# thimabru1010/ResUnet-a_mltsk_keras

Measured on AMD Instinct MI355X. Metric: training patches/sec (256×256, 6-ch, bs=8/GPU) at 1/2/4/8 MI355X, higher is better.
Workload: dtype bf16; 1 GPU; cfg3: ResUnet-a d6 multitask (seg+bound+dist+color) Tanimoto-dual, 256x256x6, 6 classes, Adam, full train step (fwd+loss+bwd+allreduce+update); global_batch=8, per_gpu_batch=8, parallelism=dp1

## Files before the change

include/rua_hip.h:

```cpp
#ifndef RUA_HIP_H
#define RUA_HIP_H
#include <stdint.h>
#ifdef __cplusplus
extern "C" {
#endif

#define RUA_F32 0
#define RUA_BF16 1
#define RUA_MAX_SEG 6
#define RUA_MAX_BRANCH 4
#define RUA_MAX_WGRAD_BATCH 32
#define RUA_MAX_WGRAD_GROUP 8

#define RUA_OK 0
#define RUA_ERR_ARG (-1)
#define RUA_ERR_LAUNCH (-2)

int rua_version(void);
const char* rua_last_error(void);
int rua_device_info(int* cu_count, int* lds_bytes, char* arch, int arch_len);

typedef struct rua_conv_seg {
  const void* x;
  const void* w;
  int32_t C, Hs, Ws;
  int32_t up_shift;
  int32_t dil;
  int32_t taps;
} rua_conv_seg;

typedef struct rua_bn_fold {
  const double* stats;
  int32_t replicas, pad;
  double count, bessel_n;
  float eps, momentum;
  const float* gamma; const float* beta;
  float* moving_mean; float* moving_var;
  float* scale; float* shift; float* mean; float* rstd;
} rua_bn_fold;

typedef struct rua_conv_desc {
  rua_conv_seg seg[RUA_MAX_SEG];
  int32_t nseg;
  int32_t N, H, W, Cout;
  int32_t stride;
  int32_t dtype;
  const float* bias;
  const void* aux;
  int32_t aux_mode;
  const float* mscale;
  const float* mshift;
  int32_t out_relu;
  int32_t accumulate;
  void* y;
  int32_t out_stride, OH, OW;
  double* stats;
  int32_t stats_mode;
  void* workspace;
  int64_t workspace_bytes;
  int32_t stats_replicas;
  const float* bias_more[3];
  const float* in_scale;
  const float* in_shift;
  int32_t in_relu;
  int32_t pad_fold;
  const struct rua_bn_fold* in_fold;
} rua_conv_desc;
int rua_conv_fwd(const rua_conv_desc* d, void* stream);
int rua_conv_fwd_group(const rua_conv_desc* d, int n, void* stream);
int rua_conv_group_last_grids(void);
int rua_conv_group_band_ok(const rua_conv_desc* d, int n);
int rua_conv_group_last_band(void);
int rua_conv_group_last_chain(void);
int rua_conv_fwd_sum(const rua_conv_desc* d, int n, void* stream);
int rua_conv_sum_last_kernel(void);
int rua_conv_sum_kernel(const rua_conv_desc* d, int n);
int rua_conv_smem_bytes(const rua_conv_desc* d);
int64_t rua_conv_workspace_bytes(const rua_conv_desc* d);
void* rua_prof_event_create(void);
int rua_prof_event_record(void* ev, void* hip_stream);
int rua_prof_event_elapsed_us(void* start, void* stop, double* us);
void rua_prof_event_destroy(void* ev);
void rua_profile_mid_event(void* hip_event);
int rua_profile_mid_event_fired(void);
int rua_conv_last_ksplit(void);
int rua_conv_tile_bn(const rua_conv_desc* d);
int rua_conv_kernel_id(const rua_conv_desc* d);
int rua_conv_fused_input_ok(const rua_conv_desc* d);
int rua_conv_tile_bm(const rua_conv_desc* d);
typedef struct rua_conv_launch_info {
  int32_t kernel_id;
  int32_t form;
  int32_t grid_x, grid_y, block, lds_bytes;
  int32_t bm, bn;
  int32_t ksplit;
  int32_t finisher;
  int32_t members;
  int32_t band, chain;
} rua_conv_launch_info;
int rua_conv_plan(const rua_conv_desc* d, rua_conv_launch_info* out);
int rua_conv_group_plan(const rua_conv_desc* d, int n, rua_conv_launch_info* out, int* n_out);

typedef struct rua_wgrad_desc {
  const void* a;  int32_t C, Hs, Ws;
  const void* dy; int32_t Cout, H, W;
  int32_t N, stride, dil, taps, dtype;
  float* dw;
  void* workspace;
  int64_t workspace_bytes;
  const float* in_scale;
  const float* in_shift;
  int32_t in_relu;
  int32_t defer;
  int32_t group_members;
  int32_t batch;
  const int32_t* overwrite_dev;
} rua_wgrad_desc;
typedef struct rua_wgrad_pending {
  int32_t kind;
  int32_t parts;
  int64_t n;
  const float* partials;
  float* dw;
  int32_t CC;
  int32_t blocks;
  int32_t block_begin, pad;
  const int32_t* overwrite_dev;
} rua_wgrad_pending;
int rua_wgrad_plan(const rua_wgrad_desc* d, rua_wgrad_pending* out);
int rua_wgrad_reduce_batch(const rua_wgrad_pending* items_dev, int n_items, int total_blocks, void* stream);
int rua_conv_wgrad(const rua_wgrad_desc* d, void* stream);
int rua_conv_wgrad_group(const rua_wgrad_desc* d, int n, void* stream);
int rua_wgrad_group_last_grids(void);
int rua_wgrad_group_plan(const rua_wgrad_desc* d, int n, rua_wgrad_pending* out);
int64_t rua_wgrad_workspace_bytes(const rua_wgrad_desc* d);
int rua_wgrad_kind(const rua_wgrad_desc* d);
int rua_wgrad_img_kind(const rua_wgrad_desc* d);

typedef struct rua_wprep_item { int64_t src_off, dst_off; int32_t taps, Cout, C, pad; } rua_wprep_item;
int rua_weight_prep(const float* master, void* w_fwd, void* w_dgrad, const rua_wprep_item* items_dev,
                    int n_items, int max_elems, int dtype, void* stream);
int rua_weight_prep_dgrad(const void* w_fwd, void* w_dgrad, const rua_wprep_item* items_dev, int n_items, int max_elems, const int32_t* blockmap_dev,
                          int n_blocks, int dtype, void* stream);
int rua_wprep_blocks(int taps, int Cout, int C);

int rua_stem_fwd(const float* x, const float* w, const float* b, void* y, int64_t M, int Cin, int Cout, int dtype, void* stream);
int rua_stem_fwd_stats(const float* x, const float* w, const float* b, void* y, int64_t M, int Cin, int Cout, int dtype, double* stats, int replicas, void* stream);
int rua_stem_bwd(const float* x, const void* dy, float* dw, float* db, int64_t M, int Cin, int Cout, int dtype, void* stream);
int rua_stem_fwd_pack(const float* x, const float* w, const float* b, void* y, int64_t M, int Cin, int Cout, int dtype, double* stats, int replicas,
                      void* xpack, void* stream);
int rua_stem_bwd_fold(float* tmp, float* dw, float* db, int Cin, int Cout, void* stream);
int rua_head_fwd(const void* x, const float* w, const float* b, float* z, float* p, int64_t M, int Cin, int Cout, int act, int dtype, void* stream);
int rua_head_fwd_loss(const void* x, const float* w, const float* b, float* z, float* p, const float* y, double* tanimoto_sums,
                      double* metrics, int B, int64_t HW, int Cin, int Cout, int act, int dtype, void* stream);
int rua_head_fwd_loss_rep(const void* x, const float* w, const float* b, float* z, float* p, const float* y, double* tanimoto_sums,
                          int sums_replicas, double* metrics, int B, int64_t HW, int Cin, int Cout, int act, int dtype, void* stream);
int rua_head_bwd(const void* x, const float* dz, const float* w, void* dx, int accumulate_dx, float* dw, float* db,
                 float* scratch, int64_t scratch_bytes, int64_t M, int Cin, int Cout, int dtype, int mask_dx, void* stream);
int rua_head_bwd_sums(const void* x, const float* dz, const float* w, void* dx, int accumulate_dx, float* dw, float* db, float* dxsum,
                      float* scratch, int64_t scratch_bytes, int64_t M, int Cin, int Cout, int dtype, int mask_dx, void* stream);

int rua_col_stats(const void* x, int64_t M, int C, double* stats, int replicas, int dtype, void* stream);
int rua_stats_replicas(int64_t blocks);
int rua_col_stats2(const void* g, const void* x, const float* mscale, const float* mshift, int masked,
                   int64_t M, int C, double* stats, int replicas, int dtype, void* stream);
int rua_bn_finalize(const double* stats, int replicas, double count, double bessel_n, const float* gamma, const float* beta,
                    float* moving_mean, float* moving_var, float momentum, float eps, int training,
                    float* scale, float* shift, float* mean, float* rstd, int C, void* stream);
int rua_stats_to_f32(const double* stats, int replicas, int C, float* const* dst, int n, void* stream);
int rua_bn_apply(const void* x, int nb, const float* const* scale, const float* const* shift, int relu,
                 void* const* out, int64_t M, int C, int dtype, void* stream);
int rua_bn_bwd_finalize(const double* stats2, int replicas, double count, const float* gamma, const float* mean, const float* rstd,
                        float* dgamma, float* dbeta, float* coefA, float* coefB, float* coefC, int C, void* stream);
int rua_bn_bwd_apply(int nb, const void* const* g, const float* const* coefA, const float* const* coefB,
                     const float* const* coefC, const float* const* mscale, const float* const* mshift, int masked,
                     const void* x, const void* dskip, void* dx, int accumulate, int64_t M, int C, int dtype, void* stream);

typedef struct rua_bn_branch {
  const float* gamma; const float* beta; float* moving_mean; float* moving_var;
  float* scale; float* shift; float* mean; float* rstd;
  void* out;
  const double* stats; int32_t replicas, pad;
  double* out_stats;
} rua_bn_branch;
typedef struct rua_bn_fwd_desc {
  const void* x; int64_t M; int32_t C, dtype, nb, relu, training, replicas;
  const double* stats;
  double count, bessel_n; float momentum, eps;
  rua_bn_branch br[RUA_MAX_BRANCH];
} rua_bn_fwd_desc;
int rua_bn_fwd(const rua_bn_fwd_desc* d, void* stream);
int rua_bn_fwd_group(const rua_bn_fwd_desc* d, int n, void* stream);
int rua_bn_fwd_group_last_grids(void);
typedef struct rua_bn_bwd_branch {
  const void* g; const double* stats2; int32_t replicas;
  int32_t stats2_out;
  const float* gamma; const float* mean; const float* rstd; const float* scale; const float* shift;
  float* dgamma; float* dbeta;
} rua_bn_bwd_branch;
typedef struct rua_bn_bwd_desc {
  const void* x; const void* dskip; void* dx; int64_t M; int32_t C, dtype, nb, masked, accumulate, pad; double count;
  rua_bn_bwd_branch br[RUA_MAX_BRANCH];
  double* skip_stats;
  int32_t skip_replicas, pad2;
  double* dx_stats;
  int32_t dx_replicas, pad3;
} rua_bn_bwd_desc;
int rua_bn_bwd(const rua_bn_bwd_desc* d, void* stream);
int rua_bn_bwd_group(const rua_bn_bwd_desc* d, int n, void* stream);
int rua_bn_bwd_group_last_grids(void);

int rua_maxpool_fwd(const void* x, void* y, uint8_t* idx, int N, int H, int W, int C, int k, int dtype, void* stream);
int rua_maxpool_bwd(const void* dy, const uint8_t* idx, void* dx, int accumulate, int N, int H, int W, int C, int k, int dtype, void* stream);
int rua_sumpool(const void* x, void* y, int N, int H, int W, int C, int k, int dtype, void* stream);
int rua_maxpool_derive(const void* y_half, const uint8_t* idx_half, void* y, uint8_t* idx, int N, int H_half, int W_half, int C,
                       int k_half, int dtype, void* stream);
int rua_maxpool_bwd_multi(int n, const void* const* dy, const uint8_t* const* idx, const int* ks, void* dx, int accumulate,
                          int N, int H, int W, int C, int dtype, void* stream);
int rua_sumpool_pyramid(const void* x, void* y2, void* y4, void* y8, int N, int H, int W, int C, int dtype, void* stream);
int rua_upsample_nearest(const void* x, void* y, int N, int H, int W, int C, int k, int dtype, void* stream);

int rua_add_n(int n, const void* const* in, void* out, int accumulate, int64_t elems, int dtype, void* stream);
int rua_relu_mask(void* dy, const void* y, int64_t elems, int dtype, void* stream);
int rua_relu(const void* x, void* y, int64_t elems, int dtype, void* stream);
int rua_cast_f32_to(const float* x, void* y, int64_t elems, int dtype, void* stream);
int rua_cast_to_f32(const void* x, float* y, int64_t elems, int dtype, void* stream);
int rua_fill_zero(void* p, int64_t bytes, void* stream);

#define RUA_LOSS_TANIMOTO 0
#define RUA_LOSS_WCE 1
#define RUA_LOSS_CE_LOGITS 2
#define RUA_LOSS_BCE_LOGITS 3
#define RUA_LOSS_MSE 4
#define RUA_ACT_NONE 0
#define RUA_ACT_SOFTMAX 1
#define RUA_ACT_SIGMOID 2
int rua_tanimoto_sums(const float* p, const float* y, int B, int64_t HW, int C, double* sums, void* stream);
int rua_tanimoto_finalize(const double* sums, int B, int64_t HW, int C, float grad_scale, double* loss_out, float* coef,
                          float* per_sample, void* stream);
#define RUA_MAX_HEADS 8
typedef struct rua_tani_head {
  double* sums; int32_t replicas, B, C; float grad_scale; double* loss_out; float* coef; float* per_sample;
} rua_tani_head;
int rua_tanimoto_finalize_multi(const rua_tani_head* heads, int n, void* stream);
typedef struct rua_dz_head {
  int32_t kind, act; const float* p; const float* y; const float* coef; const float* class_w; float grad_scale; int32_t B; int64_t HW; int32_t C, pad; float* dz;
} rua_dz_head;
int rua_head_dz_multi(const rua_dz_head* heads, int n, void* stream);
int rua_tanimoto_finalize_rep(double* sums, int replicas, int B, int64_t HW, int C, float grad_scale, double* loss_out, float* coef,
                              float* per_sample, void* stream);
int rua_tanimoto_ratio(const double* sums, int B, int C, double* mean_out, float* per_sample, void* stream);
int rua_pixel_loss(int kind, const float* p, const float* z, const float* y, const float* class_w,
                   int64_t M, int C, double* loss_out, float* per_pixel, void* stream);
int rua_head_dz(int kind, int act, const float* p, const float* y, const float* coef, const float* class_w,
                float grad_scale, int B, int64_t HW, int C, float* dz, void* stream);
int rua_seg_metrics(const float* p, const float* y, int64_t M, int C, double* out, void* stream);

int rua_tanimoto_sums_void(const float* p, const float* y, const uint8_t* void_mask, int B, int64_t HW, int C, double* sums, void* stream);
int rua_head_fwd_loss_void(const void* x, const float* w, const float* b, float* z, float* p, const float* y, double* tanimoto_sums,
                           int sums_replicas, double* metrics, int B, int64_t HW, int Cin, int Cout, int act, int dtype,
                           const uint8_t* void_mask, void* stream);
int rua_pixel_loss_void(int kind, const float* p, const float* z, const float* y, const float* class_w, const uint8_t* void_mask,
                        int64_t M, int C, double* loss_out, float* per_pixel, void* stream);
int rua_head_dz_void(int kind, int act, const float* p, const float* y, const float* coef, const float* class_w,
                     float grad_scale, int B, int64_t HW, int C, const uint8_t* void_mask, float* dz, void* stream);
int rua_head_dz_multi_void(const rua_dz_head* heads, int n, const uint8_t* void_mask, void* stream);
int rua_seg_metrics_void(const float* p, const float* y, const uint8_t* void_mask, int64_t M, int C, double* out, void* stream);

#define RUA_LOSS_FOCAL_CE 5
#define RUA_LOSS_FOCAL_BCE 6
typedef struct rua_loss_opts { float gamma, label_smoothing, alpha; int32_t class_balance; } rua_loss_opts;
int rua_pixel_loss_opts(int kind, const float* p, const float* z, const float* y, const float* class_w, const uint8_t* void_mask,
                        const rua_loss_opts* opts, int64_t M, int C, double* loss_out, float* per_pixel, void* stream);
int rua_head_dz_opts(int kind, int act, const float* p, const float* y, const float* coef, const float* class_w, float grad_scale,
                     int B, int64_t HW, int C, const uint8_t* void_mask, const rua_loss_opts* opts, float* dz, void* stream);
int rua_head_dz_multi_opts(const rua_dz_head* heads, const rua_loss_opts* opts, int n, const uint8_t* void_mask, void* stream);

typedef struct rua_ohem_opts { int64_t min_kept; int32_t keep_q16, warmup; float thresh; int32_t has_thresh; } rua_ohem_opts;
typedef struct rua_ohem_result { uint32_t tau_key; float tau; int64_t n_valid, n_kept, K; double kept_sum; float scale; int32_t q16_used; } rua_ohem_result;
int64_t rua_ohem_workspace_bytes(int64_t M);
int rua_ohem_select(const float* per_pixel, const uint8_t* void_mask, int64_t M, const rua_ohem_opts* opts, const double* step_state,
                    float loss_weight, void* workspace, int64_t workspace_bytes, uint8_t* drop_mask, double* loss_out,
                    rua_ohem_result* result_dev, void* stream);
typedef struct rua_dz_sel { const uint8_t* drop_mask; const float* scale_dev; } rua_dz_sel;
int rua_head_dz_sel(int kind, int act, const float* p, const float* y, const float* coef, const float* class_w, int B, int64_t HW, int C,
                    const rua_loss_opts* opts, const uint8_t* drop_mask, const float* scale_dev, float* dz, void* stream);
int rua_head_dz_multi_sel(const rua_dz_head* heads, const rua_loss_opts* opts, const rua_dz_sel* sel, int n, const uint8_t* void_mask, void* stream);

int rua_lr_step(double* state, float* lr_out, int adam, double beta1, double beta2, void* stream);
int rua_adam_step(float* theta, float* g, float* m, float* v, int64_t n, float lr_t, const float* lr_t_dev, float beta1, float beta2,
                  float eps, float grad_scale, int zero_grad, void* stream);
int rua_sgd_step(float* theta, float* g, float* vel, int64_t n, float lr, const float* lr_dev, float momentum, float grad_scale,
                 int zero_grad, void* stream);
int rua_adam_step_w(float* theta, float* g, float* m, float* v, int64_t n, float lr_t, const float* lr_t_dev, float beta1, float beta2,
                    float eps, float grad_scale, int zero_grad, void* wcopy_bf16, void* stream);
int rua_sgd_step_w(float* theta, float* g, float* vel, int64_t n, float lr, const float* lr_dev, float momentum, float grad_scale,
                   int zero_grad, void* wcopy_bf16, void* stream);

#define RUA_OPT_CHUNK 8192
typedef struct rua_opt_chunk { int64_t off; int32_t len; int32_t var; } rua_opt_chunk;
typedef struct rua_opt_var { int32_t chunk_begin, chunk_end, decay, pad; } rua_opt_var;
#define RUA_CLIP_NONE 0
#define RUA_CLIP_GLOBAL_NORM 1
#define RUA_CLIP_NORM 2
#define RUA_CLIP_VALUE 3
int rua_grad_sumsq(const float* g, const rua_opt_chunk* chunks, int n_chunks, double* partials, void* stream);
int rua_clip_finish(const double* partials, int n_chunks, const rua_opt_var* vars, int n_vars, int mode, double c, double grad_scale,
                    int skip_nonfinite, double* var_sumsq, float* coef, int32_t* flag, double* report, void* stream);
int rua_adam_step_seg(float* theta, float* g, float* m, float* v, const rua_opt_chunk* chunks, int n_chunks, const rua_opt_var* vars,
                      const float* coef, const int32_t* flag, const float* lr_dev, const double* lr_state, float beta1, float beta2, float eps,
                      float grad_scale, float clipvalue, double weight_decay, int zero_grad, void* wcopy_bf16, void* stream);
int rua_sgd_step_seg(float* theta, float* g, float* vel, const rua_opt_chunk* chunks, int n_chunks, const rua_opt_var* vars,
                     const float* coef, const int32_t* flag, const float* lr_dev, const double* lr_state, float momentum,
                     float grad_scale, float clipvalue, double weight_decay, int zero_grad, void* wcopy_bf16, void* stream);
int rua_state_copy(float* dst, const float* src, int64_t n, const int32_t* flag, void* stream);

#define RUA_SCHED_CONSTANT 0
#define RUA_SCHED_COSINE 1
#define RUA_SCHED_EXPONENTIAL 2
#define RUA_SCHED_POLYNOMIAL 3
#define RUA_SCHED_PIECEWISE 4
#define RUA_SCHED_INVERSE_TIME 5
#define RUA_SCHED_MAX_BOUNDARIES 16
typedef struct rua_lr_schedule {
  int32_t kind, staircase, cycle, warmup, n_boundaries, pad;
  double initial, decay_steps, decay_rate, alpha, end, power, warmup_target, warmup_steps;
  double boundaries[RUA_SCHED_MAX_BOUNDARIES];
  double values[RUA_SCHED_MAX_BOUNDARIES + 1];
} rua_lr_schedule;
int rua_lr_schedule_step(double* state, float* lr_out, rua_lr_schedule sched, int adam, double beta1, double beta2, void* stream);
int rua_ema_step(float* ema, float* theta, void* wcopy_bf16, int64_t n, float momentum, const double* lr_state, int overwrite_every,
                 const int32_t* flag, void* stream);

int rua_accum_gate(int32_t* acc_state, int k, int32_t* hold, void* stream);
int rua_accum_step(float* g, float* a, int64_t n, int k, const int32_t* hold, void* stream);
int rua_lr_step_gated(double* state, float* lr_out, int adam, double beta1, double beta2, const int32_t* hold, void* stream);
int rua_lr_schedule_step_gated(double* state, float* lr_out, rua_lr_schedule sched, int adam, double beta1, double beta2, const int32_t* hold,
                               void* stream);
int rua_grad_sumsq_gated(const float* g, const rua_opt_chunk* chunks, int n_chunks, double* partials, const int32_t* hold, void* stream);
int rua_clip_finish_gated(const double* partials, int n_chunks, const rua_opt_var* vars, int n_vars, int mode, double c, double grad_scale,
                          int skip_nonfinite, double* var_sumsq, float* coef, int32_t* flag2, double* report, const int32_t* hold, void* stream);

int rua_lamb_moments(const float* theta, float* g, float* m, float* v, const rua_opt_chunk* chunks, int n_chunks, const rua_opt_var* vars,
                     const float* coef, const int32_t* flag, const double* lr_state, float beta1, float beta2, float eps, float grad_scale,
                     float clipvalue, double weight_decay, double* pw, double* pu, void* stream);
int rua_lamb_finish(const double* pw, const double* pu, int n_chunks, const rua_opt_var* vars, int n_vars, const int32_t* flag, double* var_wu,
                    float* ratio, double* report, void* stream);
int rua_lamb_apply(float* theta, float* g, const rua_opt_chunk* chunks, int n_chunks, const rua_opt_var* vars, const float* ratio,
                   const int32_t* flag, const float* lr_dev, const double* lr_state, double weight_decay, int zero_grad, void* wcopy_bf16,
                   void* stream);

int64_t rua_targets_scratch_bytes(int N, int num_classes);
int rua_multitask_targets(const uint8_t* img, const uint8_t* cls, int N, int H, int W, int Cin, int num_classes, int norm_type,
                          float* x, float* seg, float* bound, float* dist, float* color, void* scratch, int64_t scratch_bytes, void* stream);
int rua_void_mask(const uint8_t* cls, int N, int H, int W, int num_classes, int margin, uint8_t* mask, void* stream);

int rua_scene_windows(const uint8_t* const* scene_img, const uint8_t* const* scene_cls, const int32_t* scene_h, const int32_t* scene_w,
                      int nscenes, const int32_t* windows, int N, int PH, int PW, int Cin,
                      uint8_t* img_out, uint8_t* cls_out, void* stream);

int rua_scene_windows_affine(const uint8_t* const* scene_img, const uint8_t* const* scene_cls, const int32_t* scene_h, const int32_t* scene_w,
                             int nscenes, const int32_t* windows , int N, int PH, int PW, int Cin,
                             uint8_t* img_out, uint8_t* cls_out, void* stream);

int rua_window_photometric(const uint8_t* img_in, uint8_t* img_out, int N, int PH, int PW, int Cin,
                           const int32_t* photo , void* stream);

int rua_scene_stitch(const float* p, int N, int PH, int PW, int C, const int32_t* windows, const int32_t* own,
                     uint8_t* const* scene_pred, const uint8_t* const* scene_cls, const int32_t* scene_h, const int32_t* scene_w,
                     int nscenes, int64_t* confusion, void* stream);

int rua_scene_stitch_views(const float* p, int G, int K, int PH, int PW, int C, const int32_t* windows ,
                           const int32_t* own , uint8_t* const* scene_pred, const uint8_t* const* scene_cls,
                           const int32_t* scene_h, const int32_t* scene_w, int nscenes, int64_t* confusion, void* stream);

int rua_scene_stitch_maps(const float* p, int G, int K, int PH, int PW, int Ch, const int32_t* windows ,
                          const int32_t* own , uint8_t* const* scene_out, const int32_t* scene_h,
                          const int32_t* scene_w, int nscenes, int mode , void* stream);

int rua_scene_accumulate(const float* p, int G, int K, int PH, int PW, int C, const int32_t* windows7 ,
                         const int32_t* own , int32_t* const* scene_acc, const int32_t* scene_h,
                         const int32_t* scene_w, int nscenes, void* stream);

int rua_scene_accumulate_blend(const float* p, int G, int K, int PH, int PW, int C, const int32_t* windows7 ,
                               const int32_t* foot , int32_t* const* scene_acc, const int32_t* scene_h,
                               const int32_t* scene_w, int nscenes, void* stream);

int rua_scene_argmax(const int32_t* const* scene_acc, uint8_t* const* scene_pred, const uint8_t* const* scene_cls,
                     const int32_t* scene_h, const int32_t* scene_w, int nscenes, int C, int64_t* confusion, void* stream);

int rua_scene_class_counts(const uint8_t* const* scene_cls, const int32_t* scene_h, const int32_t* scene_w, int nscenes,
                           const int32_t* windows, int N, int PH, int PW, int C, int32_t* counts, void* stream);

int rua_scene_erode(const uint8_t* const* scene_cls, const int32_t* scene_h, const int32_t* scene_w, int nscenes, int radius,
                    uint8_t* const* scene_out, const uint8_t* const* scene_pred, int C, int64_t* confusion, void* stream);

int rua_scene_boundary(const uint8_t* const* scene_cls, const uint8_t* const* scene_pred, const int32_t* scene_h, const int32_t* scene_w,
                       int nscenes, int radius, int C, uint8_t* const* bound_cls, uint8_t* const* bound_pred, int64_t* counts,
                       void* stream);

int rua_scene_regions(const uint8_t* const* scene_map, const int32_t* scene_h, const int32_t* scene_w, int nscenes, int connectivity,
                      int32_t* const* labels, int32_t* const* areas, int64_t min_area, int C, int64_t* counts, void* stream);

#define RUA_SIEVE_VOID 0
#define RUA_SIEVE_FILL 1
int rua_scene_sieve(const uint8_t* const* scene_map, const int32_t* scene_h, const int32_t* scene_w, int nscenes, int connectivity,
                    int64_t min_area, int C, uint64_t class_mask, int mode, const int32_t* const* labels, const int32_t* const* areas,
                    uint8_t* const* scene_out, void* work, int64_t work_bytes, int64_t* changed, void* stream);
int64_t rua_scene_sieve_work_bytes(int H, int W, int C);

int rua_scene_area_open(const uint8_t* const* scene_prob, const int32_t* scene_h, const int32_t* scene_w, int nscenes, int pix_stride,
                        const uint8_t* levels, int T, int64_t min_area, int connectivity, uint8_t* const* scene_open,
                        int32_t* const* labels, int32_t* const* areas, void* stream);
int rua_scene_sweep_hist(const uint8_t* const* scene_prob, const uint8_t* const* scene_open, const uint8_t* const* scene_cls,
                         const int32_t* scene_h, const int32_t* scene_w, int nscenes, int pix_stride, int positive, int C,
                         int64_t* hist, void* stream);


int rua_graph_kernel_nodes(void* graph, int* kernels, int* total);

int rua_set_tuning(const char* key, int64_t value);
int rua_get_tuning(const char* key, int64_t* value);
const char* rua_tuning_key(int index);

#ifdef __cplusplus
}
#endif
#endif
```

resunet_a_mltsk_keras_amd/_lib.py:

```python
from __future__ import annotations

import ctypes as C
import os

HERE = os.path.dirname(os.path.abspath(__file__))
LIB_PATH = os.environ.get("RUA_LIB_PATH") or os.path.join(HERE, "librua_hip.so")

RUA_F32, RUA_BF16 = 0, 1
RUA_MAX_SEG, RUA_MAX_BRANCH, RUA_MAX_WGRAD_GROUP, RUA_MAX_WGRAD_BATCH = 6, 4, 8, 32
LOSS_TANIMOTO, LOSS_WCE, LOSS_CE_LOGITS, LOSS_BCE_LOGITS, LOSS_MSE, LOSS_FOCAL_CE, LOSS_FOCAL_BCE = 0, 1, 2, 3, 4, 5, 6
ACT_NONE, ACT_SOFTMAX, ACT_SIGMOID = 0, 1, 2

vp, i32, i64, f32, f64 = C.c_void_p, C.c_int32, C.c_int64, C.c_float, C.c_double


class ConvSeg(C.Structure):
    _fields_ = [("x", vp), ("w", vp), ("C", i32), ("Hs", i32), ("Ws", i32), ("up_shift", i32), ("dil", i32), ("taps", i32)]


class ConvDesc(C.Structure):
    _fields_ = [("seg", ConvSeg * RUA_MAX_SEG), ("nseg", i32), ("N", i32), ("H", i32), ("W", i32), ("Cout", i32),
                ("stride", i32), ("dtype", i32), ("bias", vp), ("aux", vp), ("aux_mode", i32), ("mscale", vp),
                ("mshift", vp), ("out_relu", i32), ("accumulate", i32), ("y", vp), ("out_stride", i32), ("OH", i32),
                ("OW", i32), ("stats", vp), ("stats_mode", i32), ("workspace", vp), ("workspace_bytes", i64), ("stats_replicas", i32),
                ("bias_more", vp * 3), ("in_scale", vp), ("in_shift", vp), ("in_relu", i32), ("pad_fold", i32), ("in_fold", vp)]


class ConvLaunchInfo(C.Structure):
    _fields_ = [(k, i32) for k in ("kernel_id", "form", "grid_x", "grid_y", "block", "lds_bytes", "bm", "bn", "ksplit", "finisher", "members", "band", "chain")]


class BnFold(C.Structure):
    _fields_ = [("stats", vp), ("replicas", i32), ("pad", i32), ("count", f64), ("bessel_n", f64), ("eps", f32), ("momentum", f32),
                ("gamma", vp), ("beta", vp), ("moving_mean", vp), ("moving_var", vp), ("scale", vp), ("shift", vp), ("mean", vp), ("rstd", vp)]


class WgradDesc(C.Structure):
    _fields_ = [("a", vp), ("C", i32), ("Hs", i32), ("Ws", i32), ("dy", vp), ("Cout", i32), ("H", i32), ("W", i32),
                ("N", i32), ("stride", i32), ("dil", i32), ("taps", i32), ("dtype", i32), ("dw", vp), ("workspace", vp), ("workspace_bytes", i64),
                ("in_scale", vp), ("in_shift", vp), ("in_relu", i32), ("defer", i32), ("group_members", i32), ("batch", i32), ("overwrite_dev", vp)]


class WgradPending(C.Structure):
    _fields_ = [("kind", i32), ("parts", i32), ("n", i64), ("partials", vp), ("dw", vp), ("CC", i32), ("blocks", i32),
                ("block_begin", i32), ("pad", i32), ("overwrite_dev", vp)]


class LrSchedule(C.Structure):
    _fields_ = [("kind", i32), ("staircase", i32), ("cycle", i32), ("warmup", i32), ("n_boundaries", i32), ("pad", i32), ("initial", f64),
                ("decay_steps", f64), ("decay_rate", f64), ("alpha", f64), ("end", f64), ("power", f64), ("warmup_target", f64),
                ("warmup_steps", f64), ("boundaries", f64 * 16), ("values", f64 * 17)]


class TaniHead(C.Structure):
    _fields_ = [("sums", vp), ("replicas", i32), ("B", i32), ("C", i32), ("grad_scale", f32), ("loss_out", vp), ("coef", vp), ("per_sample", vp)]


class DzHead(C.Structure):
    _fields_ = [("kind", i32), ("act", i32), ("p", vp), ("y", vp), ("coef", vp), ("class_w", vp), ("grad_scale", f32), ("B", i32), ("HW", i64),
                ("C", i32), ("pad", i32), ("dz", vp)]


class LossOpts(C.Structure):
    _fields_ = [("gamma", f32), ("label_smoothing", f32), ("alpha", f32), ("class_balance", i32)]


class OhemOpts(C.Structure):
    _fields_ = [("min_kept", i64), ("keep_q16", i32), ("warmup", i32), ("thresh", f32), ("has_thresh", i32)]


class OhemResult(C.Structure):
    _fields_ = [("tau_key", C.c_uint32), ("tau", f32), ("n_valid", i64), ("n_kept", i64), ("K", i64), ("kept_sum", f64), ("scale", f32), ("q16_used", i32)]


class DzSel(C.Structure):
    _fields_ = [("drop_mask", vp), ("scale_dev", vp)]


class BnBranch(C.Structure):
    _fields_ = [("gamma", vp), ("beta", vp), ("moving_mean", vp), ("moving_var", vp), ("scale", vp), ("shift", vp),
                ("mean", vp), ("rstd", vp), ("out", vp), ("stats", vp), ("replicas", i32), ("pad", i32), ("out_stats", vp)]


class BnFwdDesc(C.Structure):
    _fields_ = [("x", vp), ("M", i64), ("C", i32), ("dtype", i32), ("nb", i32), ("relu", i32), ("training", i32), ("replicas", i32),
                ("stats", vp), ("count", f64), ("bessel_n", f64), ("momentum", f32), ("eps", f32), ("br", BnBranch * RUA_MAX_BRANCH)]


class BnBwdBranch(C.Structure):
    _fields_ = [("g", vp), ("stats2", vp), ("replicas", i32), ("stats2_out", i32), ("gamma", vp), ("mean", vp), ("rstd", vp),
                ("scale", vp), ("shift", vp), ("dgamma", vp), ("dbeta", vp)]


class BnBwdDesc(C.Structure):
    _fields_ = [("x", vp), ("dskip", vp), ("dx", vp), ("M", i64), ("C", i32), ("dtype", i32), ("nb", i32), ("masked", i32),
                ("accumulate", i32), ("pad", i32), ("count", f64), ("br", BnBwdBranch * RUA_MAX_BRANCH),
                ("skip_stats", vp), ("skip_replicas", i32), ("pad2", i32), ("dx_stats", vp), ("dx_replicas", i32), ("pad3", i32)]


class WprepItem(C.Structure):
    _fields_ = [("src_off", i64), ("dst_off", i64), ("taps", i32), ("Cout", i32), ("C", i32), ("pad", i32)]


PP = C.POINTER(vp)

_SIGS = {
    "rua_version": ([], i32),
    "rua_device_info": ([C.POINTER(i32), C.POINTER(i32), C.c_char_p, i32], i32),
    "rua_conv_fwd": ([C.POINTER(ConvDesc), vp], i32),
    "rua_conv_fwd_group": ([C.POINTER(ConvDesc), i32, vp], i32),
    "rua_conv_smem_bytes": ([C.POINTER(ConvDesc)], i32),
    "rua_conv_tile_bn": ([C.POINTER(ConvDesc)], i32),
    "rua_conv_tile_bm": ([C.POINTER(ConvDesc)], i32),
    "rua_conv_kernel_id": ([C.POINTER(ConvDesc)], i32),
    "rua_conv_fused_input_ok": ([C.POINTER(ConvDesc)], i32),
    "rua_conv_plan": ([C.POINTER(ConvDesc), C.POINTER(ConvLaunchInfo)], i32),
    "rua_conv_group_plan": ([C.POINTER(ConvDesc), i32, C.POINTER(ConvLaunchInfo), C.POINTER(i32)], i32),
    "rua_conv_last_ksplit": ([], i32),
    "rua_conv_group_last_grids": ([], i32),
    "rua_conv_group_band_ok": ([C.POINTER(ConvDesc), i32], i32),
    "rua_conv_group_last_band": ([], i32),
    "rua_conv_group_last_chain": ([], i32),
    "rua_conv_fwd_sum": ([C.POINTER(ConvDesc), i32, vp], i32),
    "rua_conv_sum_last_kernel": ([], i32),
    "rua_conv_sum_kernel": ([C.POINTER(ConvDesc), i32], i32),
    "rua_conv_wgrad_group": ([C.POINTER(WgradDesc), i32, vp], i32),
    "rua_wgrad_group_last_grids": ([], i32),
    "rua_wgrad_group_plan": ([C.POINTER(WgradDesc), i32, C.POINTER(WgradPending)], i32),
    "rua_profile_mid_event": ([vp], None),
    "rua_profile_mid_event_fired": ([], i32),
    "rua_prof_event_create": ([], vp),
    "rua_prof_event_record": ([vp, vp], i32),
    "rua_prof_event_elapsed_us": ([vp, vp, C.POINTER(f64)], i32),
    "rua_prof_event_destroy": ([vp], None),
    "rua_graph_kernel_nodes": ([vp, C.POINTER(i32), C.POINTER(i32)], i32),
    "rua_conv_workspace_bytes": ([C.POINTER(ConvDesc)], i64),
    "rua_conv_wgrad": ([C.POINTER(WgradDesc), vp], i32),
    "rua_wgrad_workspace_bytes": ([C.POINTER(WgradDesc)], i64),
    "rua_wgrad_kind": ([C.POINTER(WgradDesc)], i32),
    "rua_wgrad_img_kind": ([C.POINTER(WgradDesc)], i32),
    "rua_wgrad_plan": ([C.POINTER(WgradDesc), C.POINTER(WgradPending)], i32),
    "rua_wgrad_reduce_batch": ([vp, i32, i32, vp], i32),
    "rua_weight_prep": ([vp, vp, vp, vp, i32, i32, i32, vp], i32),
    "rua_weight_prep_dgrad": ([vp, vp, vp, i32, i32, vp, i32, i32, vp], i32),
    "rua_wprep_blocks": ([i32, i32, i32], i32),
    "rua_stem_fwd": ([vp, vp, vp, vp, i64, i32, i32, i32, vp], i32),
    "rua_stem_fwd_stats": ([vp, vp, vp, vp, i64, i32, i32, i32, vp, i32, vp], i32),
    "rua_stem_bwd": ([vp, vp, vp, vp, i64, i32, i32, i32, vp], i32),
    "rua_stem_fwd_pack": ([vp, vp, vp, vp, i64, i32, i32, i32, vp, i32, vp, vp], i32),
    "rua_stem_bwd_fold": ([vp, vp, vp, i32, i32, vp], i32),
    "rua_head_fwd": ([vp, vp, vp, vp, vp, i64, i32, i32, i32, i32, vp], i32),
    "rua_head_fwd_loss": ([vp, vp, vp, vp, vp, vp, vp, vp, i32, i64, i32, i32, i32, i32, vp], i32),
    "rua_head_fwd_loss_rep": ([vp, vp, vp, vp, vp, vp, vp, i32, vp, i32, i64, i32, i32, i32, i32, vp], i32),
    "rua_head_bwd": ([vp, vp, vp, vp, i32, vp, vp, vp, i64, i64, i32, i32, i32, i32, vp], i32),
    "rua_head_bwd_sums": ([vp, vp, vp, vp, i32, vp, vp, vp, vp, i64, i64, i32, i32, i32, i32, vp], i32),
    "rua_col_stats": ([vp, i64, i32, vp, i32, i32, vp], i32),
    "rua_col_stats2": ([vp, vp, vp, vp, i32, i64, i32, vp, i32, i32, vp], i32),
    "rua_stats_replicas": ([i64], i32),
    "rua_bn_finalize": ([vp, i32, f64, f64, vp, vp, vp, vp, f32, f32, i32, vp, vp, vp, vp, i32, vp], i32),
    "rua_bn_apply": ([vp, i32, PP, PP, i32, PP, i64, i32, i32, vp], i32),
    "rua_bn_bwd_finalize": ([vp, i32, f64, vp, vp, vp, vp, vp, vp, vp, vp, i32, vp], i32),
    "rua_bn_bwd_apply": ([i32, PP, PP, PP, PP, PP, PP, i32, vp, vp, vp, i32, i64, i32, i32, vp], i32),
    "rua_stats_to_f32": ([vp, i32, i32, PP, i32, vp], i32),
    "rua_bn_fwd": ([C.POINTER(BnFwdDesc), vp], i32),
    "rua_bn_fwd_group": ([C.POINTER(BnFwdDesc), i32, vp], i32),
    "rua_bn_fwd_group_last_grids": ([], i32),
    "rua_bn_bwd": ([C.POINTER(BnBwdDesc), vp], i32),
    "rua_bn_bwd_group": ([C.POINTER(BnBwdDesc), i32, vp], i32),
    "rua_bn_bwd_group_last_grids": ([], i32),
    "rua_maxpool_fwd": ([vp, vp, vp, i32, i32, i32, i32, i32, i32, vp], i32),
    "rua_maxpool_bwd": ([vp, vp, vp, i32, i32, i32, i32, i32, i32, i32, vp], i32),
    "rua_sumpool": ([vp, vp, i32, i32, i32, i32, i32, i32, vp], i32),
    "rua_maxpool_derive": ([vp, vp, vp, vp, i32, i32, i32, i32, i32, i32, vp], i32),
    "rua_maxpool_bwd_multi": ([i32, vp, vp, vp, vp, i32, i32, i32, i32, i32, i32, vp], i32),
    "rua_sumpool_pyramid": ([vp, vp, vp, vp, i32, i32, i32, i32, i32, vp], i32),
    "rua_upsample_nearest": ([vp, vp, i32, i32, i32, i32, i32, i32, vp], i32),
    "rua_add_n": ([i32, PP, vp, i32, i64, i32, vp], i32),
    "rua_relu_mask": ([vp, vp, i64, i32, vp], i32),
    "rua_relu": ([vp, vp, i64, i32, vp], i32),
    "rua_cast_f32_to": ([vp, vp, i64, i32, vp], i32),
    "rua_cast_to_f32": ([vp, vp, i64, i32, vp], i32),
    "rua_fill_zero": ([vp, i64, vp], i32),
    "rua_tanimoto_sums": ([vp, vp, i32, i64, i32, vp, vp], i32),
    "rua_tanimoto_finalize": ([vp, i32, i64, i32, f32, vp, vp, vp, vp], i32),
    "rua_tanimoto_finalize_rep": ([vp, i32, i32, i64, i32, f32, vp, vp, vp, vp], i32),
    "rua_tanimoto_finalize_multi": ([vp, i32, vp], i32),
    "rua_head_dz_multi": ([vp, i32, vp], i32),
    "rua_tanimoto_ratio": ([vp, i32, i32, vp, vp, vp], i32),
    "rua_pixel_loss": ([i32, vp, vp, vp, vp, i64, i32, vp, vp, vp], i32),
    "rua_head_dz": ([i32, i32, vp, vp, vp, vp, f32, i32, i64, i32, vp, vp], i32),
    "rua_seg_metrics": ([vp, vp, i64, i32, vp, vp], i32),
    "rua_lr_step": ([vp, vp, i32, f64, f64, vp], i32),
    "rua_adam_step": ([vp, vp, vp, vp, i64, f32, vp, f32, f32, f32, f32, i32, vp], i32),
    "rua_sgd_step": ([vp, vp, vp, i64, f32, vp, f32, f32, i32, vp], i32),
    "rua_adam_step_w": ([vp, vp, vp, vp, i64, f32, vp, f32, f32, f32, f32, i32, vp, vp], i32),
    "rua_sgd_step_w": ([vp, vp, vp, i64, f32, vp, f32, f32, i32, vp, vp], i32),
    "rua_grad_sumsq": ([vp, vp, i32, vp, vp], i32),
    "rua_clip_finish": ([vp, i32, vp, i32, i32, f64, f64, i32, vp, vp, vp, vp, vp], i32),
    "rua_adam_step_seg": ([vp, vp, vp, vp, vp, i32, vp, vp, vp, vp, vp, f32, f32, f32, f32, f32, f64, i32, vp, vp], i32),
    "rua_sgd_step_seg": ([vp, vp, vp, vp, i32, vp, vp, vp, vp, vp, f32, f32, f32, f64, i32, vp, vp], i32),
    "rua_state_copy": ([vp, vp, i64, vp, vp], i32),
    "rua_lr_schedule_step": ([vp, vp, LrSchedule, i32, f64, f64, vp], i32),
    "rua_ema_step": ([vp, vp, vp, i64, f32, vp, i32, vp, vp], i32),
    "rua_accum_gate": ([vp, i32, vp, vp], i32),
    "rua_accum_step": ([vp, vp, i64, i32, vp, vp], i32),
    "rua_lr_step_gated": ([vp, vp, i32, f64, f64, vp, vp], i32),
    "rua_lr_schedule_step_gated": ([vp, vp, LrSchedule, i32, f64, f64, vp, vp], i32),
    "rua_grad_sumsq_gated": ([vp, vp, i32, vp, vp, vp], i32),
    "rua_clip_finish_gated": ([vp, i32, vp, i32, i32, f64, f64, i32, vp, vp, vp, vp, vp, vp], i32),
    "rua_lamb_moments": ([vp, vp, vp, vp, vp, i32, vp, vp, vp, vp, f32, f32, f32, f32, f32, f64, vp, vp, vp], i32),
    "rua_lamb_finish": ([vp, vp, i32, vp, i32, vp, vp, vp, vp, vp], i32),
    "rua_lamb_apply": ([vp, vp, vp, i32, vp, vp, vp, vp, vp, f64, i32, vp, vp], i32),
    "rua_tanimoto_sums_void": ([vp, vp, vp, i32, i64, i32, vp, vp], i32),
    "rua_head_fwd_loss_void": ([vp, vp, vp, vp, vp, vp, vp, i32, vp, i32, i64, i32, i32, i32, i32, vp, vp], i32),
    "rua_pixel_loss_void": ([i32, vp, vp, vp, vp, vp, i64, i32, vp, vp, vp], i32),
    "rua_head_dz_void": ([i32, i32, vp, vp, vp, vp, f32, i32, i64, i32, vp, vp, vp], i32),
    "rua_head_dz_multi_void": ([vp, i32, vp, vp], i32),
    "rua_seg_metrics_void": ([vp, vp, vp, i64, i32, vp, vp], i32),
    "rua_pixel_loss_opts": ([i32, vp, vp, vp, vp, vp, C.POINTER(LossOpts), i64, i32, vp, vp, vp], i32),
    "rua_head_dz_opts": ([i32, i32, vp, vp, vp, vp, f32, i32, i64, i32, vp, C.POINTER(LossOpts), vp, vp], i32),
    "rua_head_dz_multi_opts": ([vp, vp, i32, vp, vp], i32),
    "rua_ohem_workspace_bytes": ([i64], i64),
    "rua_ohem_select": ([vp, vp, i64, C.POINTER(OhemOpts), vp, f32, vp, i64, vp, vp, vp, vp], i32),
    "rua_head_dz_sel": ([i32, i32, vp, vp, vp, vp, i32, i64, i32, C.POINTER(LossOpts), vp, vp, vp, vp], i32),
    "rua_head_dz_multi_sel": ([vp, vp, vp, i32, vp, vp], i32),
    "rua_void_mask": ([vp, i32, i32, i32, i32, i32, vp, vp], i32),
    "rua_targets_scratch_bytes": ([i32, i32], i64),
    "rua_multitask_targets": ([vp, vp, i32, i32, i32, i32, i32, i32, vp, vp, vp, vp, vp, vp, i64, vp], i32),
    "rua_scene_windows": ([vp, vp, vp, vp, i32, vp, i32, i32, i32, i32, vp, vp, vp], i32),
    "rua_scene_windows_affine": ([vp, vp, vp, vp, i32, vp, i32, i32, i32, i32, vp, vp, vp], i32),
    "rua_window_photometric": ([vp, vp, i32, i32, i32, i32, vp, vp], i32),
    "rua_scene_stitch": ([vp, i32, i32, i32, i32, vp, vp, vp, vp, vp, vp, i32, vp, vp], i32),
    "rua_scene_stitch_views": ([vp, i32, i32, i32, i32, i32, vp, vp, vp, vp, vp, vp, i32, vp, vp], i32),
    "rua_scene_stitch_maps": ([vp, i32, i32, i32, i32, i32, vp, vp, vp, vp, vp, i32, i32, vp], i32),
    "rua_scene_accumulate": ([vp, i32, i32, i32, i32, i32, vp, vp, vp, vp, vp, i32, vp], i32),
    "rua_scene_accumulate_blend": ([vp, i32, i32, i32, i32, i32, vp, vp, vp, vp, vp, i32, vp], i32),
    "rua_scene_argmax": ([vp, vp, vp, vp, vp, i32, i32, vp, vp], i32),
    "rua_scene_class_counts": ([vp, vp, vp, i32, vp, i32, i32, i32, i32, vp, vp], i32),
    "rua_scene_erode": ([vp, vp, vp, i32, i32, vp, vp, i32, vp, vp], i32),
    "rua_scene_boundary": ([vp, vp, vp, vp, i32, i32, i32, vp, vp, vp, vp], i32),
    "rua_scene_regions": ([vp, vp, vp, i32, i32, vp, vp, i64, i32, vp, vp], i32),
    "rua_scene_sieve": ([vp, vp, vp, i32, i32, i64, i32, C.c_uint64, i32, vp, vp, vp, vp, i64, vp, vp], i32),
    "rua_scene_sieve_work_bytes": ([i32, i32, i32], i64),
    "rua_scene_area_open": ([vp, vp, vp, i32, i32, vp, i32, i64, i32, vp, vp, vp, vp], i32),
    "rua_scene_sweep_hist": ([vp, vp, vp, vp, vp, i32, i32, i32, i32, vp, vp], i32),
    "rua_set_tuning": ([C.c_char_p, i64], i32),
    "rua_get_tuning": ([C.c_char_p, C.POINTER(i64)], i32),
    "rua_tuning_key": ([i32], C.c_char_p),
}

EXPORTED_SYMBOLS = sorted(list(_SIGS) + ["rua_last_error"])


class RuaError(RuntimeError):
    pass


class _Lib:
    def __init__(self):
        if not os.path.exists(LIB_PATH):
            raise RuaError(
                f"{LIB_PATH} is missing: the HIP extension has not been built. Run "
                "`python -m resunet_a_mltsk_keras_amd.build` (needs hipcc). There is no CPU fallback.")
        self.dll = C.CDLL(LIB_PATH)
        self.dll.rua_last_error.restype = C.c_char_p
        self.dll.rua_last_error.argtypes = []
        for name, (args, res) in _SIGS.items():
            fn = getattr(self.dll, name)
            fn.argtypes = args
            fn.restype = res
            setattr(self, "_" + name, fn)

        i = 0
        while True:
            key = self.dll.rua_tuning_key(i) if hasattr(self.dll, "rua_tuning_key") else None
            if not key:
                break
            v = os.environ.get("RUA_TUNE_" + key.decode().upper())
            if v is not None:
                self.check(self.dll.rua_set_tuning(key, int(v)), "rua_set_tuning")
            i += 1

    def set_tuning(self, **kv):
        for k, v in kv.items():
            self.check(self.dll.rua_set_tuning(k.encode(), int(v)), "rua_set_tuning")

    def get_tuning(self, key: str) -> int:
        v = i64()
        self.check(self.dll.rua_get_tuning(key.encode(), C.byref(v)), "rua_get_tuning")
        return int(v.value)

    def raw(self, name):
        return getattr(self, "_" + name)

    def check(self, rc, name):
        if rc != 0:
            raise RuaError(f"{name} failed ({rc}): {self.dll.rua_last_error().decode()}")

    def call(self, name, *args):
        self.check(getattr(self, "_" + name)(*args), name)


_lib = None


def lib() -> _Lib:
    global _lib
    if _lib is None:
        _lib = _Lib()
    return _lib


def ptr_array(ptrs):
    arr = (vp * len(ptrs))(*[vp(p) for p in ptrs])
    return arr
```

resunet_a_mltsk_keras_amd/csrc/capi.cpp:

```cpp
#include <hip/hip_runtime.h>
#include <stdarg.h>
#include <stdio.h>
#include <string.h>
#include <stdint.h>
#include "common.h"

static thread_local char g_err[512] = "";
RuaTuning g_tune;

void rua_set_error(const char* fmt, ...) {
  va_list ap;
  va_start(ap, fmt);
  vsnprintf(g_err, sizeof(g_err), fmt, ap);
  va_end(ap);
}

extern "C" const char* rua_last_error(void) { return g_err; }
extern "C" int rua_version(void) { return 200; }

extern "C" int rua_device_info(int* cu_count, int* lds_bytes, char* arch, int arch_len) {
  hipDeviceProp_t prop;
  int dev = 0;
  if (hipGetDevice(&dev) != hipSuccess || hipGetDeviceProperties(&prop, dev) != hipSuccess) {
    rua_set_error("rua_device_info: no HIP device");
    return RUA_ERR_LAUNCH;
  }
  if (cu_count) *cu_count = prop.multiProcessorCount;
  if (lds_bytes) *lds_bytes = (int)prop.sharedMemPerBlock;
  if (arch && arch_len > 0) { strncpy(arch, prop.gcnArchName, arch_len - 1); arch[arch_len - 1] = 0; }
  return RUA_OK;
}

extern "C" void* rua_prof_event_create(void) {
  hipEvent_t e = nullptr;
  if (hipEventCreateWithFlags(&e, hipEventDisableSystemFence | hipEventReleaseToDevice) != hipSuccess) {
    (void)hipGetLastError();
    if (hipEventCreate(&e) != hipSuccess) { rua_set_error("rua_prof_event_create: hipEventCreate failed"); return nullptr; }
  }
  return e;
}
extern "C" int rua_prof_event_record(void* ev, void* stream) {
  return hipEventRecord((hipEvent_t)ev, (hipStream_t)stream) == hipSuccess ? RUA_OK : RUA_ERR_LAUNCH;
}
extern "C" int rua_prof_event_elapsed_us(void* start, void* stop, double* us) {
  float ms = 0.f;
  if (hipEventSynchronize((hipEvent_t)stop) != hipSuccess || hipEventElapsedTime(&ms, (hipEvent_t)start, (hipEvent_t)stop) != hipSuccess) {
    rua_set_error("rua_prof_event_elapsed_us: %s", hipGetErrorString(hipGetLastError()));
    return RUA_ERR_LAUNCH;
  }
  *us = 1e3 * (double)ms;
  return RUA_OK;
}
extern "C" void rua_prof_event_destroy(void* ev) { (void)hipEventDestroy((hipEvent_t)ev); }
static thread_local hipEvent_t g_mid_event = nullptr;
static thread_local int g_mid_fired = 0;
extern "C" void rua_profile_mid_event(void* ev) { g_mid_event = (hipEvent_t)ev; if (ev) g_mid_fired = 0; }
extern "C" int rua_profile_mid_event_fired(void) { return g_mid_fired; }
void rua_record_mid_event(hipStream_t st) {
  if (g_mid_event) { (void)hipEventRecord(g_mid_event, st); g_mid_event = nullptr; g_mid_fired = 1; }
}

extern "C" int rua_graph_kernel_nodes(void* graph, int* kernels, int* total) {
  size_t n = 0;
  if (!graph || hipGraphGetNodes((hipGraph_t)graph, nullptr, &n) != hipSuccess) { (void)hipGetLastError(); rua_set_error("rua_graph_kernel_nodes: hipGraphGetNodes failed"); return RUA_ERR_ARG; }
  hipGraphNode_t* nodes = n ? new hipGraphNode_t[n] : nullptr;
  int k = 0;
  if (n && hipGraphGetNodes((hipGraph_t)graph, nodes, &n) == hipSuccess)
    for (size_t i = 0; i < n; ++i) {
      hipGraphNodeType t;
      if (hipGraphNodeGetType(nodes[i], &t) == hipSuccess && t == hipGraphNodeTypeKernel) ++k;
    }
  delete[] nodes;
  if (kernels) *kernels = k;
  if (total) *total = (int)n;
  return RUA_OK;
}

int rua_device_index() {
  int dev = 0;
  if (hipGetDevice(&dev) != hipSuccess || dev < 0) { (void)hipGetLastError(); dev = 0; }
  return dev;
}

int rua_cu_count() {
  static int cached[64] = {0};
  const int dev = rua_device_index();
  if (dev >= 64) return 256;
  if (cached[dev] == 0) {
    int n = 0;
    if (hipDeviceGetAttribute(&n, hipDeviceAttributeMultiprocessorCount, dev) != hipSuccess || n <= 0) { (void)hipGetLastError(); n = 256; }
    cached[dev] = n;
  }
  int n = cached[dev] - (g_tune.cu_reserve > 0 ? g_tune.cu_reserve : 0);
  return n < 16 ? 16 : n;
}

struct TuneKey { const char* name; int* i; long long* ll; };
static const TuneKey* tune_table(int* n) {
  static const TuneKey t[] = {
    {"conv_force_bn", &g_tune.conv_force_bn, nullptr}, {"conv_force_bm", &g_tune.conv_force_bm, nullptr}, {"conv_dma", &g_tune.conv_dma, nullptr},
    {"conv_pw", &g_tune.conv_pw, nullptr}, {"conv_pw_minm", nullptr, &g_tune.conv_pw_minm}, {"conv_pw_blocks", &g_tune.conv_pw_blocks, nullptr},
    {"conv_halo", &g_tune.conv_halo, nullptr}, {"conv_dmap", &g_tune.conv_dmap, nullptr}, {"dmap_target", &g_tune.dmap_target, nullptr},
    {"dmap_fused_finish", &g_tune.dmap_fused_finish, nullptr}, {"dmap_rowb", &g_tune.dmap_rowb, nullptr}, {"dmap_bm64", &g_tune.dmap_bm64, nullptr},
    {"wgrad_pw", &g_tune.wgrad_pw, nullptr}, {"wgpw_blocks", &g_tune.wgpw_blocks, nullptr}, {"wgpw_r", &g_tune.wgpw_r, nullptr},
    {"wgd_blocks", &g_tune.wgd_blocks, nullptr}, {"wgrad_dmap", &g_tune.wgrad_dmap, nullptr}, {"wgd_mintiles", &g_tune.wgd_mintiles, nullptr},
    {"wgrad_blocks", &g_tune.wgrad_blocks, nullptr}, {"bn_grid", &g_tune.bn_grid, nullptr}, {"tani_vec", &g_tune.tani_vec, nullptr},
    {"metrics_blocks", &g_tune.metrics_blocks, nullptr}, {"stem_blocks", &g_tune.stem_blocks, nullptr}, {"head_blocks", &g_tune.head_blocks, nullptr},
    {"conv_img", &g_tune.conv_img, nullptr}, {"conv_strip", &g_tune.conv_strip, nullptr}, {"wgrad_slabs", &g_tune.wgrad_slabs, nullptr},
    {"strip_narrow_maxd", &g_tune.strip_narrow_maxd, nullptr}, {"conv_group", &g_tune.conv_group, nullptr}, {"wgrad_group", &g_tune.wgrad_group, nullptr},
    {"wgrad_batch_blocks", &g_tune.wgrad_batch_blocks, nullptr}, {"wgd_ks_slow", &g_tune.wgd_ks_slow, nullptr}, {"head_fwd2", &g_tune.head_fwd2, nullptr},
    {"head_fwd3", &g_tune.head_fwd3, nullptr}, {"head_fwd3_bpc", &g_tune.head_fwd3_bpc, nullptr}, {"stem_reg", &g_tune.stem_reg, nullptr},
    {"stats_blocks", &g_tune.stats_blocks, nullptr}, {"conv_band", &g_tune.conv_band, nullptr}, {"conv_band64", &g_tune.conv_band64, nullptr},
    {"conv_band64m", &g_tune.conv_band64m, nullptr}, {"strip_group_share", &g_tune.strip_group_share, nullptr}, {"band_dbg", &g_tune.band_dbg, nullptr},
    {"fill_kernel", &g_tune.fill_kernel, nullptr}, {"bn_regs", &g_tune.bn_regs, nullptr}, {"wgrad_taps_share", &g_tune.wgrad_taps_share, nullptr},
    {"dmap_chain", &g_tune.dmap_chain, nullptr}, {"epi_fast", &g_tune.epi_fast, nullptr}, {"dmap_spread", &g_tune.dmap_spread, nullptr},
    {"bn_bwd_group", &g_tune.bn_bwd_group, nullptr}, {"conv_small", &g_tune.conv_small, nullptr}, {"strip_stag", &g_tune.strip_stag, nullptr},
    {"cu_reserve", &g_tune.cu_reserve, nullptr}, {"wgrad_rows", &g_tune.wgrad_rows, nullptr}, {"strip_seglen", &g_tune.strip_seglen, nullptr},
    {"band_stag", &g_tune.band_stag, nullptr}, {"conv_band128m", &g_tune.conv_band128m, nullptr}, {"conv_img2", &g_tune.conv_img2, nullptr},
    {"dbg_ptr", nullptr, &g_tune.dbg_ptr},
  };
  *n = (int)(sizeof(t) / sizeof(t[0]));
  return t;
}
extern "C" int rua_set_tuning(const char* key, int64_t value) {
  int n; const TuneKey* t = tune_table(&n);
  for (int i = 0; key && i < n; ++i)
    if (strcmp(t[i].name, key) == 0) { if (t[i].i) *t[i].i = (int)value; else *t[i].ll = (long long)value; return RUA_OK; }
  rua_set_error("rua_set_tuning: unknown key '%s'", key ? key : "(null)");
  return RUA_ERR_ARG;
}
extern "C" int rua_get_tuning(const char* key, int64_t* value) {
  int n; const TuneKey* t = tune_table(&n);
  for (int i = 0; key && value && i < n; ++i)
    if (strcmp(t[i].name, key) == 0) { *value = t[i].i ? (int64_t)*t[i].i : (int64_t)*t[i].ll; return RUA_OK; }
  rua_set_error("rua_get_tuning: unknown key '%s'", key ? key : "(null)");
  return RUA_ERR_ARG;
}
extern "C" const char* rua_tuning_key(int index) {
  int n; const TuneKey* t = tune_table(&n);
  return (index >= 0 && index < n) ? t[index].name : nullptr;
}
```

resunet_a_mltsk_keras_amd/csrc/common.h:

```cpp
#pragma once
#include <hip/hip_runtime.h>
#include <stdint.h>
#include <stdio.h>
#include <string.h>
#include "../../include/rua_hip.h"

typedef __bf16 bf16_t;
typedef __attribute__((ext_vector_type(16))) float f32x16;
typedef __attribute__((ext_vector_type(4))) float f32x4;
typedef __attribute__((ext_vector_type(8))) __bf16 bf16x8;
typedef __attribute__((ext_vector_type(4))) short s16x4;

void rua_set_error(const char* fmt, ...);
#define RUA_CHECK_ARG(cond, ...) do { if (!(cond)) { rua_set_error(__VA_ARGS__); return RUA_ERR_ARG; } } while (0)
#define RUA_LAUNCH_CHECK(name) do { hipError_t e_ = hipGetLastError(); if (e_ != hipSuccess) { \
    rua_set_error("%s: %s", name, hipGetErrorString(e_)); return RUA_ERR_LAUNCH; } } while (0)

template <typename T> struct ET;
template <> struct ET<float> {
  static constexpr int VEC = 4;
  static __device__ __forceinline__ void unpack(const uint4& v, float* f) {
    f[0] = __uint_as_float(v.x); f[1] = __uint_as_float(v.y); f[2] = __uint_as_float(v.z); f[3] = __uint_as_float(v.w);
  }
  static __device__ __forceinline__ uint4 pack(const float* f) {
    return make_uint4(__float_as_uint(f[0]), __float_as_uint(f[1]), __float_as_uint(f[2]), __float_as_uint(f[3]));
  }
};
template <> struct ET<bf16_t> {
  static constexpr int VEC = 8;
  static __device__ __forceinline__ void unpack(const uint4& v, float* f) {
    f[0] = __uint_as_float(v.x << 16); f[1] = __uint_as_float(v.x & 0xffff0000u);
    f[2] = __uint_as_float(v.y << 16); f[3] = __uint_as_float(v.y & 0xffff0000u);
    f[4] = __uint_as_float(v.z << 16); f[5] = __uint_as_float(v.z & 0xffff0000u);
    f[6] = __uint_as_float(v.w << 16); f[7] = __uint_as_float(v.w & 0xffff0000u);
  }
  static __device__ __forceinline__ uint32_t pk(float a, float b) {
    typedef __attribute__((ext_vector_type(2))) __bf16 bf2;
    bf2 r; r[0] = (__bf16)a; r[1] = (__bf16)b;
    return __builtin_bit_cast(uint32_t, r);
  }
  static __device__ __forceinline__ uint4 pack(const float* f) {
    return make_uint4(pk(f[0], f[1]), pk(f[2], f[3]), pk(f[4], f[5]), pk(f[6], f[7]));
  }
};

__device__ __forceinline__ uint4 ldg16(const void* p) { return *reinterpret_cast<const uint4*>(p); }

typedef __attribute__((ext_vector_type(4))) unsigned int u32x4_t;
#define RUA_OOB 0xFFFFFFF0u
__device__ __forceinline__ __amdgpu_buffer_rsrc_t make_rsrc(const void* p, unsigned bytes) {
  return __builtin_amdgcn_make_buffer_rsrc(const_cast<void*>(p), 0, bytes, 0x00020000);
}
__device__ __forceinline__ uint4 bufload16(__amdgpu_buffer_rsrc_t r, unsigned byte_off) {
  const u32x4_t v = __builtin_amdgcn_raw_buffer_load_b128(r, byte_off, 0, 0);
  return make_uint4(v[0], v[1], v[2], v[3]);
}
__device__ __forceinline__ void stg16(void* p, const uint4& v) { *reinterpret_cast<uint4*>(p) = v; }

__device__ __forceinline__ float wave_sum(float v) {
#pragma unroll
  for (int o = 32; o > 0; o >>= 1) v += __shfl_xor(v, o, 64);
  return v;
}

struct RuaTuning {
  int conv_force_bn = 0, conv_force_bm = 0, conv_dma = -1, conv_pw = 1;
  long long conv_pw_minm = 65536;
  int conv_pw_blocks = 0, conv_halo = 1, conv_dmap = 1, dmap_target = 0, dmap_fused_finish = 0, dmap_rowb = 64, dmap_bm64 = 1;
  int wgrad_pw = 3 , wgpw_blocks = 0, wgpw_r = 0, wgd_blocks = 0, wgrad_dmap = 1, wgd_mintiles = 10 , wgrad_blocks = 0;
  int bn_grid = 0, tani_vec = 1, metrics_blocks = 0, stem_blocks = 0, head_blocks = 0;
  int conv_strip = 1, wgrad_slabs = 1, strip_narrow_maxd = 0, strip_group_share = 1;
  int conv_group = 63;
  int stats_blocks = 0;
  int stem_reg = 1;
  int head_fwd3 = 1;
  int head_fwd3_bpc = 0;
  int head_fwd2 = 1;
  int conv_img2 = 1;
  int conv_img = 0;
  int conv_small = 4096;
  int bn_bwd_group = 1;
  int dmap_spread = 1;
  int epi_fast = 1;
  int dmap_chain = 0;
  int wgrad_taps_share = 1;
  int bn_regs = 1;
  int fill_kernel = 1;
  int band_dbg = 0;
  int conv_band64m = 1;
  int conv_band64 = 1;
  long long dbg_ptr = 0;
  int conv_band128m = 13;
  int conv_band = 1;
  int wgd_ks_slow = 1;
  int wgrad_rows = 127;
  int cu_reserve = 0;
  int strip_seglen = 0;
  int band_stag = 1;
  int strip_stag = 1;
  int wgrad_group = 23;
  int wgrad_batch_blocks = 0;
};
extern RuaTuning g_tune;
int rua_cu_count();
int rua_device_index();
void rua_record_mid_event(hipStream_t st);
struct RuaPerDevFlag { bool f[64] = {}; bool& get() { return f[rua_device_index() & 63]; } };

__device__ __forceinline__ void replica_sum(const double* __restrict__ stats, int R, int C, int c, double& s1, double& s2) {
  double a1 = 0, a2 = 0, b1 = 0, b2 = 0;
  int r = 0;
  for (; r + 8 <= R; r += 8) {
    double x[8], y[8];
#pragma unroll
    for (int u = 0; u < 8; ++u) { x[u] = stats[(size_t)(r + u) * 2 * C + c]; y[u] = stats[(size_t)(r + u) * 2 * C + C + c]; }
    a1 += (x[0] + x[1]) + (x[2] + x[3]); b1 += (x[4] + x[5]) + (x[6] + x[7]);
    a2 += (y[0] + y[1]) + (y[2] + y[3]); b2 += (y[4] + y[5]) + (y[6] + y[7]);
  }
  for (; r + 4 <= R; r += 4) {
    const double x0 = stats[(size_t)(r + 0) * 2 * C + c], y0 = stats[(size_t)(r + 0) * 2 * C + C + c];
    const double x1 = stats[(size_t)(r + 1) * 2 * C + c], y1 = stats[(size_t)(r + 1) * 2 * C + C + c];
    const double x2 = stats[(size_t)(r + 2) * 2 * C + c], y2 = stats[(size_t)(r + 2) * 2 * C + C + c];
    const double x3 = stats[(size_t)(r + 3) * 2 * C + c], y3 = stats[(size_t)(r + 3) * 2 * C + C + c];
    a1 += x0 + x1; b1 += x2 + x3; a2 += y0 + y1; b2 += y2 + y3;
  }
  for (; r < R; ++r) { a1 += stats[(size_t)r * 2 * C + c]; a2 += stats[(size_t)r * 2 * C + C + c]; }
  s1 = a1 + b1; s2 = a2 + b2;
}

__device__ __forceinline__ float ld_f32_or_zero(const float* p, int c, int n) {
  return __builtin_bit_cast(float, __builtin_amdgcn_raw_buffer_load_b32(make_rsrc(p, p ? (unsigned)(n * 4) : 0u), (unsigned)(c * 4), 0, 0));
}

template <int NT, int CH, typename GetF, typename Has, typename Store>
__device__ __forceinline__ void rua_fold_members(GetF&& getf, Has&& has, int nmem, bool publish, double* red, int tid, Store&& store) {
  typedef __attribute__((ext_vector_type(2))) unsigned u32x2_t;
  constexpr int NG = NT / CH, gpm = NG / RUA_MAX_BRANCH;
  static_assert(gpm >= 1, "thread groups per member");
  constexpr int KMAX = (32 + gpm - 1) / gpm;
  constexpr int GPW = 64 / CH;
  static_assert(CH <= 64 && gpm % GPW == 0, "a wave must not straddle two members");
  const int c = tid % CH, grp = tid / CH;
  const int m = __builtin_amdgcn_readfirstlane(tid >> 6) / (gpm / GPW), gi = grp - m * gpm;
  const int mc = m < nmem ? m : 0;
  const bool act = m < nmem && has(mc);
  const rua_bn_fold& f = getf(mc);
  float gam = 0.f, bet = 0.f;
  if (act) {
    const __amdgpu_buffer_rsrc_t rs = make_rsrc(f.stats, (unsigned)(f.replicas * 2 * CH * 8));
    u32x2_t x[KMAX], y[KMAX];
#pragma unroll
    for (int k = 0; k < KMAX; ++k) {
      const unsigned off = (unsigned)(((gi + k * gpm) * 2 * CH + c) * 8);
      x[k] = __builtin_amdgcn_raw_buffer_load_b64(rs, off, 0, 0);
      y[k] = __builtin_amdgcn_raw_buffer_load_b64(rs, off + (unsigned)(CH * 8), 0, 0);
    }
    if (gi == 0) { gam = f.gamma[c]; bet = f.beta[c]; }
    double a1 = 0, a2 = 0;
#pragma unroll
    for (int k = 0; k < KMAX; ++k) { a1 += __builtin_bit_cast(double, x[k]); a2 += __builtin_bit_cast(double, y[k]); }
    for (int r = gi + KMAX * gpm; r < f.replicas; r += gpm) { a1 += f.stats[(size_t)r * 2 * CH + c]; a2 += f.stats[(size_t)r * 2 * CH + CH + c]; }
    red[(grp * 2) * CH + c] = a1; red[(grp * 2 + 1) * CH + c] = a2;
  }
  __syncthreads();
  if (act && gi == 0) {
    double s1 = 0, s2 = 0;
    for (int g = 0; g < gpm; ++g) { s1 += red[((grp + g) * 2) * CH + c]; s2 += red[((grp + g) * 2 + 1) * CH + c]; }
    const double mean = s1 / f.count;
    double v = s2 / f.count - mean * mean;
    if (v < 0) v = 0;
    const double r = 1.0 / sqrt(v + (double)f.eps);
    const double sc = (double)gam * r;
    const float scf = (float)sc, shf = (float)((double)bet - mean * sc);
    store(m, c, scf, shf);
    if (publish) {
      f.scale[c] = scf; f.shift[c] = shf;
      if (f.mean) f.mean[c] = (float)mean;
      if (f.rstd) f.rstd[c] = (float)r;
      if (f.moving_mean) {
        const double unb = f.bessel_n > 1 ? v * (f.bessel_n / (f.bessel_n - 1)) : v;
        f.moving_mean[c] = (float)((double)f.moving_mean[c] * f.momentum + mean * (1.0 - f.momentum));
        f.moving_var[c] = (float)((double)f.moving_var[c] * f.momentum + unb * (1.0 - f.momentum));
      }
    }
  }
  __syncthreads();
}

struct SegK { const unsigned char* x; const unsigned char* w; int C, Hs, Ws, up, dil, taps, nchunk, ubegin; unsigned xbytes, wbytes; };
struct ConvK {
  SegK seg[RUA_MAX_SEG];
  int nseg, nunits;
  int N, H, W, Cout, stride;
  long long M;
  const float* bias; const float* bias_more[3]; const unsigned char* aux; int aux_mode; const float* mscale; const float* mshift;
  int out_relu, accumulate; unsigned char* y; int out_stride, OH, OW; double* stats; int stats_mode; int stats_R;
  int nbn, nbm, ksplit, stages_per_split; float* ws;
  int* cnt;
  const float* in_scale; const float* in_shift; int in_relu;
  int epi_fast;
};
typedef __attribute__((address_space(3))) void* lds_void_p;
struct ConvKG { ConvK k[RUA_MAX_BRANCH]; };
static_assert(sizeof(ConvKG) <= 4096, "grouped launch: kernel arguments are limited to 4 KiB");
struct HaloK {
  ConvK c;
  int d, TH, TW, PT, NS, HPW, HP, nty, ntx, total_sub, rows;
  unsigned mHP, mHPW, mPT, mTW;
};
struct PwStep { const unsigned char* x; const unsigned char* w; unsigned xbytes, wbytes; int C, kofs, up, Hs, Ws, dense; };
template <int KS> struct PwK { ConvK c; PwStep st[KS]; int px_per_wave, wsh, hsh, nblk; };
struct StripK {
  ConvK c;
  const unsigned char* ep;
  unsigned epbytes;
  int d, strips, spc, seglen, njobs, nchains;
  int slot_bytes, SWH;
  int dbg;
  int has_fold; rua_bn_fold f;
};
struct StripKG { StripK k[RUA_MAX_BRANCH]; };
static_assert(sizeof(StripKG) <= 4096, "a grouped launch passes its members by value: HIP kernel arguments are limited to 4 KiB");
struct Img2K {
  const unsigned char* x; const unsigned char* w; float* ws;
  int C, Cout, H, M, ngrp, nco, ksplit, cpb;
  unsigned xbytes, wbytes;
};

enum ConvKernel {
  CK_IGEMM_BF16 = 0,
  CK_IGEMM_F32 = 5,
  CK_DMA = 10,
  CK_DMAP128 = 15, CK_DMAP128_R128, CK_DMAP64, CK_DMAP_S,
  CK_HALO2, CK_HALO3,
  CK_PW2, CK_PW2_DENSE, CK_PW4, CK_PW4_DENSE, CK_PW6, CK_PW6_DENSE,
  CK_SMALL,
  CK_IMG8_24, CK_IMG8_12, CK_IMG16, CK_IMG16_K2,
  CK_MFMA_KERNELS,
  CK_IMG2_8 = CK_MFMA_KERNELS, CK_IMG2_16,
  CK_STRIP,
  CK_STRIPS = CK_STRIP + 4,
  CK_KERNELS = CK_STRIPS + 16
};
enum ConvArgs { CA_CONV, CA_HALO, CA_PW2, CA_PW4, CA_PW6, CA_STRIP, CA_STRIPS, CA_IMG2 };
enum ConvRoute { CONV_LAUNCH = 0, CONV_ROUTE_BAND128_SUM };
struct ConvKernelRow { const char* name; const void* one; const void* many; const void* chain; int args; int lds; int lds_chain; };
#define RUA_KERNEL_FN(...) reinterpret_cast<const void*>(&__VA_ARGS__)
extern const ConvKernelRow RUA_STRIP_ROWS[CK_KERNELS - CK_STRIP];
extern const ConvKernelRow RUA_IMG2_ROWS[2];
struct ConvLaunch {
  int kernel;
  int route;
  int kid;
  unsigned gx, block; int smem;
  int bm, bn;
  int ksplit, finisher;
  bool groupable;
  int per_cu;
  union { ConvK c; HaloK h; PwK<2> p2; PwK<4> p4; PwK<6> p6; StripK s; } a;
  Img2K i2;
};
int rua_plan_conv_strip(const rua_conv_desc* d, int members, bool in_group, ConvLaunch* L);
int rua_strip_s_pack(const ConvLaunch* const* L, int m, void* sg, unsigned* gx, int* smem);
bool rua_band64_ok(const rua_conv_desc* d, int n);
int rua_launch_band64(const rua_conv_desc* d, int n, hipStream_t st);
bool rua_band64m_ok(const rua_conv_desc* d, int n);
int rua_launch_band64m(const rua_conv_desc* d, int n, hipStream_t st);
bool rua_band128m_ok(const rua_conv_desc* d, int n);
int rua_launch_band128m(const rua_conv_desc* d, int n, hipStream_t st);
bool rua_band128_sum_ok(const rua_conv_desc* d);
int rua_launch_band128_sum(const rua_conv_desc* d, hipStream_t st);
int rua_pick_img2(const rua_conv_desc* d, bool in_group);
void rua_plan_conv_img2(const rua_conv_desc* d, int KS, ConvLaunch* L);
bool rua_pick_strip(const rua_conv_desc* d);

static inline int rua_div_up(int64_t a, int64_t b) { return (int)((a + b - 1) / b); }
```

resunet_a_mltsk_keras_amd/csrc/elementwise.hip:

```cpp
#include "common.h"
#include <stdlib.h>

static inline int grid_for(int64_t pieces) {
  int64_t g = (pieces + 255) / 256;
  if (g > 2048) g = 2048;
  if (g < 1) g = 1;
  return (int)g;
}

struct StatsK { const unsigned char* x; const unsigned char* g; const float* ms; const float* mt; int masked;
                long long M; int C, CG, TX, TY, rows_per_block; double* stats; int R; };

template <typename T, int MODE>
__global__ __launch_bounds__(256) void col_stats_kernel(const StatsK p) {
  constexpr int VEC = ET<T>::VEC;
  __shared__ float sred[256 * (2 * VEC + 1)];
  const int tid = threadIdx.x;
  const int CGA = p.CG;
  const int CG = CGA < 256 ? CGA : 256;
  const int cp0 = blockIdx.y * CG;
  const int cp = cp0 + (tid & (CG - 1));
  const int rpb = 256 / CG;
  float s1[VEC], s2[VEC], ms[VEC], mt[VEC];
#pragma unroll
  for (int j = 0; j < VEC; ++j) { s1[j] = 0.f; s2[j] = 0.f; ms[j] = 1.f; mt[j] = 0.f; }
  if (MODE == 2 && p.masked) {
#pragma unroll
    for (int j = 0; j < VEC; ++j) { if (p.ms) ms[j] = p.ms[cp * VEC + j]; if (p.mt) mt[j] = p.mt[cp * VEC + j]; }
  }
  const long long rstep = (long long)gridDim.x * rpb;
  long long r = (long long)blockIdx.x * rpb + tid / CG;
  constexpr int UN = (MODE == 1) ? 8 : 4;
  for (; r + (UN - 1) * rstep < p.M; r += UN * rstep) {
    uint4 q[UN], qg[UN];
#pragma unroll
    for (int u = 0; u < UN; ++u) {
      q[u] = ldg16(p.x + ((size_t)(r + u * rstep) * CGA + cp) * 16);
      if (MODE == 2) qg[u] = ldg16(p.g + ((size_t)(r + u * rstep) * CGA + cp) * 16);
    }
#pragma unroll
    for (int u = 0; u < UN; ++u) {
      float xv[VEC];
      ET<T>::unpack(q[u], xv);
      if (MODE == 1) {
#pragma unroll
        for (int j = 0; j < VEC; ++j) { s1[j] += xv[j]; s2[j] = fmaf(xv[j], xv[j], s2[j]); }
      } else {
        float gv[VEC];
        ET<T>::unpack(qg[u], gv);
#pragma unroll
        for (int j = 0; j < VEC; ++j) {
          const float m = (!p.masked || fmaf(ms[j], xv[j], mt[j]) > 0.f) ? gv[j] : 0.f;
          s1[j] += m; s2[j] = fmaf(m, xv[j], s2[j]);
        }
      }
    }
  }
  for (; r < p.M; r += rstep) {
    float xv[VEC];
    ET<T>::unpack(ldg16(p.x + ((size_t)r * CGA + cp) * 16), xv);
    if (MODE == 1) {
#pragma unroll
      for (int j = 0; j < VEC; ++j) { s1[j] += xv[j]; s2[j] = fmaf(xv[j], xv[j], s2[j]); }
    } else {
      float gv[VEC];
      ET<T>::unpack(ldg16(p.g + ((size_t)r * CGA + cp) * 16), gv);
#pragma unroll
      for (int j = 0; j < VEC; ++j) {
        const float m = (!p.masked || fmaf(ms[j], xv[j], mt[j]) > 0.f) ? gv[j] : 0.f;
        s1[j] += m; s2[j] = fmaf(m, xv[j], s2[j]);
      }
    }
  }
  constexpr int TW = 2 * VEC + 1;
  float* mine = sred + tid * TW;
#pragma unroll
  for (int j = 0; j < VEC; ++j) { mine[j] = s1[j]; mine[VEC + j] = s2[j]; }
  __syncthreads();
  double* st = p.stats + (size_t)(blockIdx.x & (p.R - 1)) * 2 * p.C;
  for (int t = tid; t < CG * 2 * VEC; t += 256) {
    const int cpi = t / (2 * VEC), k = t % (2 * VEC);
    float a0 = 0.f, a1 = 0.f;
    int rr = cpi;
    for (; rr + CG < 256; rr += 2 * CG) { a0 += sred[rr * TW + k]; a1 += sred[(rr + CG) * TW + k]; }
    if (rr < 256) a0 += sred[rr * TW + k];
    unsafeAtomicAdd(&st[(k / VEC) * p.C + (cp0 + cpi) * VEC + (k % VEC)], (double)(a0 + a1));
  }
}

extern "C" int rua_stats_replicas(int64_t blocks) {
  int r = 1;
  while (r < 32 && (int64_t)r * 8 < blocks) r *= 2;
  return r;
}

template <int MODE>
static int launch_stats(const void* g, const void* x, const float* ms, const float* mt, int masked,
                        int64_t M, int C, double* stats, int replicas, int dtype, void* stream, const char* name) {
  RUA_CHECK_ARG(replicas >= 1 && (replicas & (replicas - 1)) == 0, "%s: replicas must be a power of two", name);
  RUA_CHECK_ARG(x && stats && M > 0, "%s: bad arguments", name);
  RUA_CHECK_ARG(dtype == RUA_F32 || dtype == RUA_BF16, "%s: bad dtype", name);
  const int vec = dtype == RUA_BF16 ? 8 : 4;
  RUA_CHECK_ARG(C % vec == 0, "%s: C=%d not a multiple of %d", name, C, vec);
  StatsK k;
  k.x = (const unsigned char*)x; k.g = (const unsigned char*)g; k.ms = ms; k.mt = mt; k.masked = masked;
  k.M = M; k.C = C; k.CG = C / vec;
  RUA_CHECK_ARG((k.CG & (k.CG - 1)) == 0, "%s: C/%d = %d must be a power of two", name, vec, k.CG);
  const int gy = k.CG > 256 ? k.CG / 256 : 1;
  k.TX = k.CG; k.TY = 256 / k.CG; k.rows_per_block = 0;
  k.stats = stats; k.R = replicas;
  const int64_t pieces = M * k.CG;
  int64_t gx = pieces / (256 * 8) / gy;
  const int64_t scap = g_tune.stats_blocks > 0 ? g_tune.stats_blocks : 1024;
  if (gx > scap / gy) gx = scap / gy;
  if (gx < 1) gx = 1;
  hipStream_t st = (hipStream_t)stream;
  if (dtype == RUA_BF16) hipLaunchKernelGGL((col_stats_kernel<bf16_t, MODE>), dim3((unsigned)gx, gy), dim3(256), 0, st, k);
  else hipLaunchKernelGGL((col_stats_kernel<float, MODE>), dim3((unsigned)gx, gy), dim3(256), 0, st, k);
  RUA_LAUNCH_CHECK(name);
  return RUA_OK;
}

extern "C" int rua_col_stats(const void* x, int64_t M, int C, double* stats, int replicas, int dtype, void* stream) {
  return launch_stats<1>(nullptr, x, nullptr, nullptr, 0, M, C, stats, replicas, dtype, stream, "rua_col_stats");
}
extern "C" int rua_col_stats2(const void* g, const void* x, const float* mscale, const float* mshift, int masked,
                              int64_t M, int C, double* stats, int replicas, int dtype, void* stream) {
  RUA_CHECK_ARG(g != nullptr, "rua_col_stats2: null g");
  return launch_stats<2>(g, x, mscale, mshift, masked, M, C, stats, replicas, dtype, stream, "rua_col_stats2");
}


__global__ void bn_finalize_kernel(const double* stats, int R, double count, double bessel_n, const float* gamma, const float* beta,
                                   float* mmean, float* mvar, float momentum, float eps, int training,
                                   float* scale, float* shift, float* mean_o, float* rstd_o, int C) {
  const int c = blockIdx.x * blockDim.x + threadIdx.x;
  if (c >= C) return;
  double mean, var;
  if (training) {
    double s1, s2;
    replica_sum(stats, R, C, c, s1, s2);
    mean = s1 / count;
    var = s2 / count - mean * mean;
    if (var < 0) var = 0;
    if (mmean) {
      const double unb = bessel_n > 1 ? var * (bessel_n / (bessel_n - 1)) : var;
      mmean[c] = (float)((double)mmean[c] * momentum + mean * (1.0 - momentum));
      mvar[c] = (float)((double)mvar[c] * momentum + unb * (1.0 - momentum));
    }
  } else {
    mean = mmean[c]; var = mvar[c];
  }
  const double r = 1.0 / sqrt(var + (double)eps);
  const double s = (double)gamma[c] * r;
  scale[c] = (float)s;
  shift[c] = (float)((double)beta[c] - mean * s);
  if (mean_o) mean_o[c] = (float)mean;
  if (rstd_o) rstd_o[c] = (float)r;
}

extern "C" int rua_bn_finalize(const double* stats, int replicas, double count, double bessel_n, const float* gamma, const float* beta,
                               float* moving_mean, float* moving_var, float momentum, float eps, int training,
                               float* scale, float* shift, float* mean, float* rstd, int C, void* stream) {
  RUA_CHECK_ARG(gamma && beta && scale && shift && C > 0, "rua_bn_finalize: bad arguments");
  RUA_CHECK_ARG(training ? (stats != nullptr && count > 0) : (moving_mean && moving_var), "rua_bn_finalize: missing statistics");
  hipLaunchKernelGGL(bn_finalize_kernel, dim3(rua_div_up(C, 64)), dim3(64), 0, (hipStream_t)stream,
                     stats, replicas < 1 ? 1 : replicas, count, bessel_n, gamma, beta, moving_mean, moving_var, momentum, eps, training, scale, shift, mean, rstd, C);
  RUA_LAUNCH_CHECK("rua_bn_finalize");
  return RUA_OK;
}

__global__ void bn_bwd_finalize_kernel(const double* st2, int R, double count, const float* gamma, const float* mean, const float* rstd,
                                       float* dgamma, float* dbeta, float* cA, float* cB, float* cC, int C) {
  const int c = blockIdx.x * blockDim.x + threadIdx.x;
  if (c >= C) return;
  double sg, sgx;
  replica_sum(st2, R, C, c, sg, sgx);
  const double mu = mean[c], r = rstd[c], gm = gamma[c];
  const double dbe = sg;
  const double dga = r * (sgx - mu * sg);
  const double s = gm * r;
  if (dgamma) dgamma[c] += (float)dga;
  if (dbeta) dbeta[c] += (float)dbe;
  cA[c] = (float)s;
  cB[c] = (float)(-s * r * dga / count);
  cC[c] = (float)(-s * dbe / count + s * r * mu * dga / count);
}

extern "C" int rua_bn_bwd_finalize(const double* stats2, int replicas, double count, const float* gamma, const float* mean, const float* rstd,
                                   float* dgamma, float* dbeta, float* coefA, float* coefB, float* coefC, int C, void* stream) {
  RUA_CHECK_ARG(stats2 && gamma && mean && rstd && coefA && coefB && coefC && C > 0 && count > 0, "rua_bn_bwd_finalize: bad arguments");
  hipLaunchKernelGGL(bn_bwd_finalize_kernel, dim3(rua_div_up(C, 64)), dim3(64), 0, (hipStream_t)stream,
                     stats2, replicas < 1 ? 1 : replicas, count, gamma, mean, rstd, dgamma, dbeta, coefA, coefB, coefC, C);
  RUA_LAUNCH_CHECK("rua_bn_bwd_finalize");
  return RUA_OK;
}

__global__ void stats_to_f32_kernel(const double* stats, int R, int C, float* d0, float* d1, float* d2, float* d3, int n) {
  const int c = blockIdx.x * blockDim.x + threadIdx.x;
  if (c >= C) return;
  double a, unused;
  replica_sum(stats, R, C, c, a, unused);
  const float v = (float)a;
  d0[c] += v; if (n > 1) d1[c] += v; if (n > 2) d2[c] += v; if (n > 3) d3[c] += v;
}
extern "C" int rua_stats_to_f32(const double* stats, int replicas, int C, float* const* dst, int n, void* stream) {
  RUA_CHECK_ARG(stats && dst && n >= 1 && n <= 4 && C > 0, "rua_stats_to_f32: bad arguments");
  for (int i = 0; i < n; ++i) RUA_CHECK_ARG(dst[i], "rua_stats_to_f32: null destination");
  hipLaunchKernelGGL(stats_to_f32_kernel, dim3(rua_div_up(C, 64)), dim3(64), 0, (hipStream_t)stream, stats, replicas < 1 ? 1 : replicas, C,
                     dst[0], n > 1 ? dst[1] : nullptr, n > 2 ? dst[2] : nullptr, n > 3 ? dst[3] : nullptr, n);
  RUA_LAUNCH_CHECK("rua_stats_to_f32");
  return RUA_OK;
}

struct ApplyK { const unsigned char* x; int nb; const float* scale[RUA_MAX_BRANCH]; const float* shift[RUA_MAX_BRANCH];
                unsigned char* out[RUA_MAX_BRANCH]; int relu; long long pieces; int C, CG; };

template <typename T>
__global__ __launch_bounds__(256) void bn_apply_kernel(const ApplyK p) {
  constexpr int VEC = ET<T>::VEC;
  extern __shared__ float tab[];
  for (int i = threadIdx.x; i < p.nb * p.C; i += 256) {
    const int b = i / p.C, c = i - b * p.C;
    tab[(b * 2) * p.C + c] = p.scale[b][c];
    tab[(b * 2 + 1) * p.C + c] = p.shift[b][c];
  }
  __syncthreads();
  const long long stride = (long long)gridDim.x * 256;
  for (long long i = (long long)blockIdx.x * 256 + threadIdx.x; i < p.pieces; i += stride) {
    const int c = (int)(i % p.CG) * VEC;
    float xv[VEC];
    ET<T>::unpack(ldg16(p.x + i * 16), xv);
    for (int b = 0; b < p.nb; ++b) {
      float o[VEC];
#pragma unroll
      for (int j = 0; j < VEC; ++j) {
        o[j] = fmaf(tab[(b * 2) * p.C + c + j], xv[j], tab[(b * 2 + 1) * p.C + c + j]);
        if (p.relu) o[j] = fmaxf(o[j], 0.f);
      }
      stg16(p.out[b] + i * 16, ET<T>::pack(o));
    }
  }
}

extern "C" int rua_bn_apply(const void* x, int nb, const float* const* scale, const float* const* shift, int relu,
                            void* const* out, int64_t M, int C, int dtype, void* stream) {
  RUA_CHECK_ARG(x && scale && shift && out && nb >= 1 && nb <= RUA_MAX_BRANCH && M > 0, "rua_bn_apply: bad arguments");
  RUA_CHECK_ARG(dtype == RUA_F32 || dtype == RUA_BF16, "rua_bn_apply: bad dtype");
  const int vec = dtype == RUA_BF16 ? 8 : 4;
  RUA_CHECK_ARG(C % vec == 0, "rua_bn_apply: C=%d not a multiple of %d", C, vec);
  ApplyK k;
  k.x = (const unsigned char*)x; k.nb = nb; k.relu = relu; k.C = C; k.CG = C / vec; k.pieces = M * k.CG;
  for (int b = 0; b < nb; ++b) { k.scale[b] = scale[b]; k.shift[b] = shift[b]; k.out[b] = (unsigned char*)out[b];
    RUA_CHECK_ARG(scale[b] && shift[b] && out[b], "rua_bn_apply: null branch pointer"); }
  const size_t smem = (size_t)nb * 2 * C * 4;
  RUA_CHECK_ARG(smem <= 64 * 1024, "rua_bn_apply: coefficient table too large");
  hipStream_t st = (hipStream_t)stream;
  if (dtype == RUA_BF16) hipLaunchKernelGGL((bn_apply_kernel<bf16_t>), dim3(grid_for(k.pieces)), dim3(256), smem, st, k);
  else hipLaunchKernelGGL((bn_apply_kernel<float>), dim3(grid_for(k.pieces)), dim3(256), smem, st, k);
  RUA_LAUNCH_CHECK("rua_bn_apply");
  return RUA_OK;
}

struct BwdApplyK { int nb; const unsigned char* g[RUA_MAX_BRANCH]; const float* cA[RUA_MAX_BRANCH]; const float* cB[RUA_MAX_BRANCH];
                   const float* cC[RUA_MAX_BRANCH]; const float* ms[RUA_MAX_BRANCH]; const float* mt[RUA_MAX_BRANCH]; int masked;
                   const unsigned char* x; const unsigned char* dskip; unsigned char* dx; int accumulate; long long pieces; int C, CG; };

template <typename T>
__global__ __launch_bounds__(256) void bn_bwd_apply_kernel(const BwdApplyK p) {
  constexpr int VEC = ET<T>::VEC;
  extern __shared__ float tab[];
  float* tB = tab + p.nb * 3 * p.C;
  for (int c = threadIdx.x; c < p.C; c += 256) {
    float sb = 0.f, sc = 0.f;
    for (int b = 0; b < p.nb; ++b) {
      tab[(b * 3) * p.C + c] = p.cA[b][c];
      tab[(b * 3 + 1) * p.C + c] = (p.masked && p.ms[b]) ? p.ms[b][c] : 1.f;
      tab[(b * 3 + 2) * p.C + c] = (p.masked && p.mt[b]) ? p.mt[b][c] : 0.f;
      sb += p.cB[b][c]; sc += p.cC[b][c];
    }
    tB[c] = sb; tB[p.C + c] = sc;
  }
  __syncthreads();
  const long long stride = (long long)gridDim.x * 256;
  for (long long i = (long long)blockIdx.x * 256 + threadIdx.x; i < p.pieces; i += stride) {
    const int c = (int)(i % p.CG) * VEC;
    float xv[VEC], acc[VEC];
    ET<T>::unpack(ldg16(p.x + i * 16), xv);
#pragma unroll
    for (int j = 0; j < VEC; ++j) acc[j] = fmaf(tB[c + j], xv[j], tB[p.C + c + j]);
    if (p.dskip) {
      float d[VEC];
      ET<T>::unpack(ldg16(p.dskip + i * 16), d);
#pragma unroll
      for (int j = 0; j < VEC; ++j) acc[j] += d[j];
    }
    if (p.accumulate) {
      float d[VEC];
      ET<T>::unpack(ldg16(p.dx + i * 16), d);
#pragma unroll
      for (int j = 0; j < VEC; ++j) acc[j] += d[j];
    }
    for (int b = 0; b < p.nb; ++b) {
      float gv[VEC];
      ET<T>::unpack(ldg16(p.g[b] + i * 16), gv);
#pragma unroll
      for (int j = 0; j < VEC; ++j) {
        const bool on = !p.masked || fmaf(tab[(b * 3 + 1) * p.C + c + j], xv[j], tab[(b * 3 + 2) * p.C + c + j]) > 0.f;
        acc[j] = fmaf(tab[(b * 3) * p.C + c + j], on ? gv[j] : 0.f, acc[j]);
      }
    }
    stg16(p.dx + i * 16, ET<T>::pack(acc));
  }
}

extern "C" int rua_bn_bwd_apply(int nb, const void* const* g, const float* const* coefA, const float* const* coefB,
                                const float* const* coefC, const float* const* mscale, const float* const* mshift, int masked,
                                const void* x, const void* dskip, void* dx, int accumulate, int64_t M, int C, int dtype, void* stream) {
  RUA_CHECK_ARG(nb >= 1 && nb <= RUA_MAX_BRANCH && g && coefA && coefB && coefC && x && dx && M > 0, "rua_bn_bwd_apply: bad arguments");
  RUA_CHECK_ARG(dtype == RUA_F32 || dtype == RUA_BF16, "rua_bn_bwd_apply: bad dtype");
  const int vec = dtype == RUA_BF16 ? 8 : 4;
  RUA_CHECK_ARG(C % vec == 0, "rua_bn_bwd_apply: C=%d not a multiple of %d", C, vec);
  BwdApplyK k;
  k.nb = nb; k.masked = masked; k.x = (const unsigned char*)x; k.dskip = (const unsigned char*)dskip; k.dx = (unsigned char*)dx;
  k.accumulate = accumulate; k.C = C; k.CG = C / vec; k.pieces = M * k.CG;
  for (int b = 0; b < nb; ++b) {
    RUA_CHECK_ARG(g[b] && coefA[b] && coefB[b] && coefC[b], "rua_bn_bwd_apply: null branch pointer");
    k.g[b] = (const unsigned char*)g[b]; k.cA[b] = coefA[b]; k.cB[b] = coefB[b]; k.cC[b] = coefC[b];
    k.ms[b] = mscale ? mscale[b] : nullptr; k.mt[b] = mshift ? mshift[b] : nullptr;
  }
  const size_t smem = (size_t)(nb * 3 + 2) * C * 4;
  RUA_CHECK_ARG(smem <= 64 * 1024, "rua_bn_bwd_apply: coefficient table too large");
  hipStream_t st = (hipStream_t)stream;
  if (dtype == RUA_BF16) hipLaunchKernelGGL((bn_bwd_apply_kernel<bf16_t>), dim3(grid_for(k.pieces)), dim3(256), smem, st, k);
  else hipLaunchKernelGGL((bn_bwd_apply_kernel<float>), dim3(grid_for(k.pieces)), dim3(256), smem, st, k);
  RUA_LAUNCH_CHECK("rua_bn_bwd_apply");
  return RUA_OK;
}

template <typename T, int NB>
__device__ __forceinline__ void bn_fwd_body(const rua_bn_fwd_desc& p, long long pieces, int CG) {
  constexpr int VEC = ET<T>::VEC;
  extern __shared__ float tab[];
  const int C = p.C;
  float* mr = tab + p.nb * 2 * C;
  for (int c = threadIdx.x; c < C; c += 256) {
    double mean, var;
    if (p.training && p.stats) {
      double s1, s2;
      replica_sum(p.stats, p.replicas, C, c, s1, s2);
      mean = s1 / p.count;
      var = s2 / p.count - mean * mean;
      if (var < 0) var = 0;
    } else { mean = 0; var = 1; }
    for (int b = 0; b < p.nb; ++b) {
      const rua_bn_branch& br = p.br[b];
      double m = mean, v = var;
      if (p.training && br.stats) {
        double s1, s2;
        replica_sum(br.stats, br.replicas, C, c, s1, s2);
        m = s1 / p.count;
        v = s2 / p.count - m * m;
        if (v < 0) v = 0;
      }
      if (!p.training) { m = br.moving_mean[c]; v = br.moving_var[c]; }
      const double r = 1.0 / sqrt(v + (double)p.eps);
      const double sc = (double)br.gamma[c] * r;
      tab[(b * 2) * C + c] = (float)sc;
      tab[(b * 2 + 1) * C + c] = (float)((double)br.beta[c] - m * sc);
      if (blockIdx.x == 0) {
        br.scale[c] = (float)sc; br.shift[c] = (float)((double)br.beta[c] - m * sc);
        if (br.mean) br.mean[c] = (float)m;
        if (br.rstd) br.rstd[c] = (float)r;
        if (p.training && br.out_stats) {
          const double be = (double)br.beta[c];
          br.out_stats[c] = p.count * be;
          br.out_stats[C + c] = p.count * (be * be + sc * sc * v);
        }
        if (p.training && br.moving_mean) {
          const double unb = p.bessel_n > 1 ? v * (p.bessel_n / (p.bessel_n - 1)) : v;
          br.moving_mean[c] = (float)((double)br.moving_mean[c] * p.momentum + m * (1.0 - p.momentum));
          br.moving_var[c] = (float)((double)br.moving_var[c] * p.momentum + unb * (1.0 - p.momentum));
        }
      }
    }
    (void)mr;
  }
  __syncthreads();
  if (p.br[0].out == nullptr) return;
  const unsigned char* x = (const unsigned char*)p.x;
  const long long stride = (long long)gridDim.x * 256;
  if constexpr (NB > 0) {
    const int c = (int)(threadIdx.x % CG) * VEC;
    float sc[NB][VEC], sh[NB][VEC];
#pragma unroll
    for (int b = 0; b < NB; ++b)
#pragma unroll
      for (int j = 0; j < VEC; ++j) { sc[b][j] = tab[(b * 2) * C + c + j]; sh[b][j] = tab[(b * 2 + 1) * C + c + j]; }
    unsigned char* outs[NB];
#pragma unroll
    for (int b = 0; b < NB; ++b) outs[b] = (unsigned char*)p.br[b].out;
    const bool relu = p.relu != 0;
    for (long long i = (long long)blockIdx.x * 256 + threadIdx.x; i < pieces; i += stride) {
      float xv[VEC];
      ET<T>::unpack(ldg16(x + i * 16), xv);
#pragma unroll
      for (int b = 0; b < NB; ++b) {
        float o[VEC];
#pragma unroll
        for (int j = 0; j < VEC; ++j) {
          o[j] = fmaf(sc[b][j], xv[j], sh[b][j]);
          if (relu) o[j] = fmaxf(o[j], 0.f);
        }
        stg16(outs[b] + i * 16, ET<T>::pack(o));
      }
    }
  } else {
    for (long long i = (long long)blockIdx.x * 256 + threadIdx.x; i < pieces; i += stride) {
      const int c = (int)(i % CG) * VEC;
      float xv[VEC];
      ET<T>::unpack(ldg16(x + i * 16), xv);
      for (int b = 0; b < p.nb; ++b) {
        float o[VEC];
#pragma unroll
        for (int j = 0; j < VEC; ++j) {
          o[j] = fmaf(tab[(b * 2) * C + c + j], xv[j], tab[(b * 2 + 1) * C + c + j]);
          if (p.relu) o[j] = fmaxf(o[j], 0.f);
        }
        stg16((unsigned char*)p.br[b].out + i * 16, ET<T>::pack(o));
      }
    }
  }
}

template <typename T, int NB>
__global__ __launch_bounds__(256) void bn_fwd_kernel(const rua_bn_fwd_desc p, long long pieces, int CG) { bn_fwd_body<T, NB>(p, pieces, CG); }
struct BnFwdG { rua_bn_fwd_desc k[RUA_MAX_BRANCH]; long long pieces[RUA_MAX_BRANCH]; };
static_assert(sizeof(BnFwdG) <= 4096, "grouped launch: kernel arguments are limited to 4 KiB");
template <typename T>
__global__ __launch_bounds__(256) void bn_fwd_kernel_g(const BnFwdG g, int CG) { bn_fwd_body<T, 1>(g.k[blockIdx.y], g.pieces[blockIdx.y], CG); }

extern "C" int rua_bn_fwd(const rua_bn_fwd_desc* d, void* stream);
static thread_local int g_bn_fwd_group_last = 0;
extern "C" int rua_bn_fwd_group_last_grids(void) { return g_bn_fwd_group_last; }
extern "C" int rua_bn_fwd_group(const rua_bn_fwd_desc* d, int n, void* stream) {
  RUA_CHECK_ARG(d && n >= 1 && n <= RUA_MAX_BRANCH, "rua_bn_fwd_group: 1..%d members", RUA_MAX_BRANCH);
  const int vec = d[0].dtype == RUA_BF16 ? 8 : 4;
  bool one = n > 1 && g_tune.bn_bwd_group && d[0].C % vec == 0 && d[0].C / vec <= 256 && 256 % (d[0].C / vec) == 0 && g_tune.bn_regs &&
             (d[0].dtype == RUA_F32 || d[0].dtype == RUA_BF16) && (size_t)4 * d[0].C * 4 <= 64 * 1024;
  for (int i = 0; i < n && one; ++i) {
    const rua_bn_fwd_desc& m = d[i];
    const rua_bn_branch& br = m.br[0];
    one = m.x && m.nb == 1 && m.M > 0 && m.C == d[0].C && m.dtype == d[0].dtype && m.training == d[0].training && m.relu == d[0].relu && br.out &&
          br.gamma && br.beta && br.scale && br.shift && (!m.training || (m.count > 0 && (br.stats ? br.replicas >= 1 : (m.stats && m.replicas >= 1)))) &&
          (m.training || (br.moving_mean && br.moving_var)) && (br.out_stats == nullptr || (m.relu == 0 && m.training));
  }
  g_bn_fwd_group_last = n;
  if (!one) {
    for (int i = 0; i < n; ++i) { const int rc = rua_bn_fwd(d + i, stream); if (rc != RUA_OK) return rc; }
    return RUA_OK;
  }
  const int CG = d[0].C / vec;
  const size_t smem = (size_t)(1 * 2 + 2) * d[0].C * 4;
  BnFwdG a;
  long long pieces = 0;
  for (int i = 0; i < n; ++i) { a.k[i] = d[i]; a.pieces[i] = d[i].M * CG; if (a.pieces[i] > pieces) pieces = a.pieces[i]; }
  int g = grid_for(pieces);
  const int cap = 2 * rua_cu_count() / (n > 2 ? 2 : 1);
  if (g > cap) g = cap;
  hipStream_t st = (hipStream_t)stream;
  if (d[0].dtype == RUA_BF16) hipLaunchKernelGGL((bn_fwd_kernel_g<bf16_t>), dim3(g, n), dim3(256), smem, st, a, CG);
  else hipLaunchKernelGGL((bn_fwd_kernel_g<float>), dim3(g, n), dim3(256), smem, st, a, CG);
  RUA_LAUNCH_CHECK("rua_bn_fwd_group");
  g_bn_fwd_group_last = 1;
  return RUA_OK;
}

extern "C" int rua_bn_fwd(const rua_bn_fwd_desc* d, void* stream) {
  RUA_CHECK_ARG(d && d->nb >= 1 && d->nb <= RUA_MAX_BRANCH && d->M > 0 && d->C > 0, "rua_bn_fwd: bad arguments");
  const bool coef_only = d->br[0].out == nullptr;
  RUA_CHECK_ARG(coef_only || d->x, "rua_bn_fwd: null input");
  RUA_CHECK_ARG(d->dtype == RUA_F32 || d->dtype == RUA_BF16, "rua_bn_fwd: bad dtype");
  const int vec = d->dtype == RUA_BF16 ? 8 : 4;
  RUA_CHECK_ARG(d->C % vec == 0, "rua_bn_fwd: C=%d not a multiple of %d", d->C, vec);
  RUA_CHECK_ARG(!d->training || d->count > 0, "rua_bn_fwd: training needs the element count");
  for (int b = 0; b < d->nb; ++b) {
    const rua_bn_branch& br = d->br[b];
    RUA_CHECK_ARG(br.gamma && br.beta && br.scale && br.shift, "rua_bn_fwd: null branch pointer");
    RUA_CHECK_ARG((br.out == nullptr) == coef_only, "rua_bn_fwd: either every branch has an output or none (coefficients only)");
    RUA_CHECK_ARG(!d->training || (br.stats ? br.replicas >= 1 : (d->stats && d->replicas >= 1)), "rua_bn_fwd: training needs statistics");
    RUA_CHECK_ARG(d->training || (br.moving_mean && br.moving_var), "rua_bn_fwd: inference needs moving statistics");
    RUA_CHECK_ARG(br.out_stats == nullptr || (d->relu == 0 && d->training), "rua_bn_fwd: out_stats is the statistics of a training-mode BatchNorm WITHOUT ReLU");
  }
  const size_t smem = (size_t)(d->nb * 2 + 2) * d->C * 4;
  RUA_CHECK_ARG(smem <= 64 * 1024, "rua_bn_fwd: coefficient table too large");
  const int CG = d->C / vec;
  const long long pieces = d->M * CG;
  int g = grid_for(pieces);
  const int cap = g_tune.bn_grid > 0 ? g_tune.bn_grid : 2 * rua_cu_count();
  if ((long long)d->replicas * d->C >= 512 && g > cap) g = cap;
  if (coef_only) g = 1;
  hipStream_t st = (hipStream_t)stream;
  const int nbk = (!coef_only && CG <= 256 && 256 % CG == 0 && g_tune.bn_regs) ? d->nb : 0;
#define RUA_BN_FWD_GO(T_, NB_) hipLaunchKernelGGL((bn_fwd_kernel<T_, NB_>), dim3(g), dim3(256), smem, st, *d, pieces, CG)
  if (d->dtype == RUA_BF16) {
    switch (nbk) { case 1: RUA_BN_FWD_GO(bf16_t, 1); break; case 2: RUA_BN_FWD_GO(bf16_t, 2); break; case 3: RUA_BN_FWD_GO(bf16_t, 3); break;
                   case 4: RUA_BN_FWD_GO(bf16_t, 4); break; default: RUA_BN_FWD_GO(bf16_t, 0); }
  } else {
    switch (nbk) { case 1: RUA_BN_FWD_GO(float, 1); break; case 2: RUA_BN_FWD_GO(float, 2); break; case 3: RUA_BN_FWD_GO(float, 3); break;
                   case 4: RUA_BN_FWD_GO(float, 4); break; default: RUA_BN_FWD_GO(float, 0); }
  }
#undef RUA_BN_FWD_GO
  RUA_LAUNCH_CHECK("rua_bn_fwd");
  return RUA_OK;
}

template <typename T, int NB, bool MASKED, bool DXS = false>
__device__ __forceinline__ void bn_bwd_body(const rua_bn_bwd_desc& p, long long pieces, int CG) {
  constexpr int VEC = ET<T>::VEC;
  extern __shared__ float tab[];
  const int C = p.C;
  float* tB = tab + p.nb * 3 * C;
  float* tT = tB + 2 * C;
  for (int it = threadIdx.x; it < p.nb * C; it += 256) {
    const int b = it / C, c = it - b * C;
    const rua_bn_bwd_branch& br = p.br[b];
    double sg, sgx;
    replica_sum(br.stats2, br.replicas, C, c, sg, sgx);
    const double mu = br.mean[c], r = br.rstd[c], gm = br.gamma[c];
    if (br.stats2_out) {
      const double sc = br.scale[c], sh = br.shift[c];
      sgx = sc != 0.0 ? (sgx - sh * sg) / sc : mu * sg;
    }
    const double dga = r * (sgx - mu * sg);
    const double s = gm * r;
    tab[(b * 3) * C + c] = (float)s;
    tab[(b * 3 + 1) * C + c] = (p.masked && br.scale) ? br.scale[c] : 1.f;
    tab[(b * 3 + 2) * C + c] = (p.masked && br.shift) ? br.shift[c] : 0.f;
    tT[(b * 2) * C + c] = (float)(-s * r * dga / p.count);
    tT[(b * 2 + 1) * C + c] = (float)(-s * sg / p.count + s * r * mu * dga / p.count);
    if (blockIdx.x == 0) {
      if (br.dgamma) br.dgamma[c] += (float)dga;
      if (br.dbeta) br.dbeta[c] += (float)sg;
    }
  }
  __syncthreads();
  for (int c = threadIdx.x; c < C; c += 256) {
    float sb = 0.f, sc_ = 0.f;
    for (int b = 0; b < p.nb; ++b) { sb += tT[(b * 2) * C + c]; sc_ += tT[(b * 2 + 1) * C + c]; }
    tB[c] = sb; tB[C + c] = sc_;
  }
  __syncthreads();
  const unsigned char* x = (const unsigned char*)p.x;
  const unsigned char* dskip = (const unsigned char*)p.dskip;
  unsigned char* dx = (unsigned char*)p.dx;
  const long long stride = (long long)gridDim.x * 256;
  float sk[VEC], so[VEC], so2[VEC];
#pragma unroll
  for (int j = 0; j < VEC; ++j) { sk[j] = 0.f; so[j] = 0.f; so2[j] = 0.f; }
  if constexpr (NB > 0) {
    const int c = (int)(threadIdx.x % CG) * VEC;
    float cA[NB][VEC], cS[MASKED ? NB : 1][VEC], cT[MASKED ? NB : 1][VEC], cB[VEC], cC[VEC];
#pragma unroll
    for (int j = 0; j < VEC; ++j) { cB[j] = tB[c + j]; cC[j] = tB[C + c + j]; }
#pragma unroll
    for (int b = 0; b < NB; ++b)
#pragma unroll
      for (int j = 0; j < VEC; ++j) {
        cA[b][j] = tab[(b * 3) * C + c + j];
        if constexpr (MASKED) { cS[b][j] = tab[(b * 3 + 1) * C + c + j]; cT[b][j] = tab[(b * 3 + 2) * C + c + j]; }
      }
    const unsigned char* gp[NB];
#pragma unroll
    for (int b = 0; b < NB; ++b) gp[b] = (const unsigned char*)p.br[b].g;
    const bool accum = p.accumulate != 0;
    for (long long i = (long long)blockIdx.x * 256 + threadIdx.x; i < pieces; i += stride) {
      const uint4 xr = ldg16(x + i * 16);
      uint4 gr[NB];
#pragma unroll
      for (int b = 0; b < NB; ++b) gr[b] = ldg16(gp[b] + i * 16);
      uint4 dr = make_uint4(0, 0, 0, 0), ar = make_uint4(0, 0, 0, 0);
      if (dskip) dr = ldg16(dskip + i * 16);
      if (accum) ar = ldg16(dx + i * 16);
      float xv[VEC], acc[VEC];
      ET<T>::unpack(xr, xv);
#pragma unroll
      for (int j = 0; j < VEC; ++j) acc[j] = fmaf(cB[j], xv[j], cC[j]);
      if (dskip) {
        float dd[VEC];
        ET<T>::unpack(dr, dd);
#pragma unroll
        for (int j = 0; j < VEC; ++j) { acc[j] += dd[j]; sk[j] += dd[j]; }
      }
      if (accum) {
        float dd[VEC];
        ET<T>::unpack(ar, dd);
#pragma unroll
        for (int j = 0; j < VEC; ++j) acc[j] += dd[j];
      }
#pragma unroll
      for (int b = 0; b < NB; ++b) {
        float gv[VEC];
        ET<T>::unpack(gr[b], gv);
#pragma unroll
        for (int j = 0; j < VEC; ++j) {
          bool on = true;
          if constexpr (MASKED) on = fmaf(cS[b][j], xv[j], cT[b][j]) > 0.f;
          acc[j] = fmaf(cA[b][j], on ? gv[j] : 0.f, acc[j]);
        }
      }
#pragma unroll
      for (int j = 0; j < VEC; ++j) if constexpr (DXS) { so[j] += acc[j]; so2[j] = fmaf(acc[j], xv[j], so2[j]); }
      stg16(dx + i * 16, ET<T>::pack(acc));
    }
  } else {
  for (long long i = (long long)blockIdx.x * 256 + threadIdx.x; i < pieces; i += stride) {
    const int c = (int)(i % CG) * VEC;
    float xv[VEC], acc[VEC];
    ET<T>::unpack(ldg16(x + i * 16), xv);
#pragma unroll
    for (int j = 0; j < VEC; ++j) acc[j] = fmaf(tB[c + j], xv[j], tB[C + c + j]);
    if (dskip) {
      float dd[VEC];
      ET<T>::unpack(ldg16(dskip + i * 16), dd);
#pragma unroll
      for (int j = 0; j < VEC; ++j) { acc[j] += dd[j]; sk[j] += dd[j]; }
    }
    if (p.accumulate) {
      float dd[VEC];
      ET<T>::unpack(ldg16(dx + i * 16), dd);
#pragma unroll
      for (int j = 0; j < VEC; ++j) acc[j] += dd[j];
    }
    for (int b = 0; b < p.nb; ++b) {
      float gv[VEC];
      ET<T>::unpack(ldg16((const unsigned char*)p.br[b].g + i * 16), gv);
#pragma unroll
      for (int j = 0; j < VEC; ++j) {
        const bool on = !p.masked || fmaf(tab[(b * 3 + 1) * C + c + j], xv[j], tab[(b * 3 + 2) * C + c + j]) > 0.f;
        acc[j] = fmaf(tab[(b * 3) * C + c + j], on ? gv[j] : 0.f, acc[j]);
      }
    }
#pragma unroll
    for (int j = 0; j < VEC; ++j) if constexpr (DXS) { so[j] += acc[j]; so2[j] = fmaf(acc[j], xv[j], so2[j]); }
    stg16(dx + i * 16, ET<T>::pack(acc));
  }
  }
  auto fold = [&](float* v, double* dst, int replicas, int slot) {
    float* red = tab;
    __syncthreads();
    if (CG <= 32) {
#pragma unroll
      for (int j = 0; j < VEC; ++j)
        for (int o = CG; o < 64; o <<= 1) v[j] += __shfl_xor(v[j], o, 64);
      const int lane = threadIdx.x & 63, wv = threadIdx.x >> 6;
      if (lane < CG) {
#pragma unroll
        for (int j = 0; j < VEC; ++j) red[(wv * CG + lane) * VEC + j] = v[j];
      }
      __syncthreads();
      for (int ch = threadIdx.x; ch < C; ch += 256) {
        const float t = (red[ch] + red[C + ch]) + (red[2 * C + ch] + red[3 * C + ch]);
        unsafeAtomicAdd(&dst[(size_t)(blockIdx.x & (replicas - 1)) * 2 * C + slot * C + ch], (double)t);
      }
    } else {
#pragma unroll
      for (int j = 0; j < VEC; ++j) red[threadIdx.x * VEC + j] = v[j];
      __syncthreads();
      const int per = 256 / CG;
      for (int ch = threadIdx.x; ch < C; ch += 256) {
        const int cg = ch / VEC, j = ch - cg * VEC;
        float t = 0.f;
        for (int k = 0; k < per; ++k) t += red[(k * CG + cg) * VEC + j];
        unsafeAtomicAdd(&dst[(size_t)(blockIdx.x & (replicas - 1)) * 2 * C + slot * C + ch], (double)t);
      }
    }
  };
  if (p.skip_stats && dskip) fold(sk, p.skip_stats, p.skip_replicas, 0);
  if constexpr (DXS) { fold(so, p.dx_stats, p.dx_replicas, 0); fold(so2, p.dx_stats, p.dx_replicas, 1); }
}

template <typename T, int NB, bool MASKED, bool DXS = false>
__global__ __launch_bounds__(256) void bn_bwd_kernel(const rua_bn_bwd_desc p, long long pieces, int CG) { bn_bwd_body<T, NB, MASKED, DXS>(p, pieces, CG); }
struct BnBwdG { rua_bn_bwd_desc k[RUA_MAX_BRANCH]; long long pieces[RUA_MAX_BRANCH]; };
static_assert(sizeof(BnBwdG) <= 4096, "grouped launch: kernel arguments are limited to 4 KiB");
template <typename T, bool MASKED>
__global__ __launch_bounds__(256) void bn_bwd_kernel_g(const BnBwdG g, int CG) { bn_bwd_body<T, 1, MASKED>(g.k[blockIdx.y], g.pieces[blockIdx.y], CG); }

extern "C" int rua_bn_bwd(const rua_bn_bwd_desc* d, void* stream);
static thread_local int g_bn_bwd_group_last = 0;
extern "C" int rua_bn_bwd_group_last_grids(void) { return g_bn_bwd_group_last; }
extern "C" int rua_bn_bwd_group(const rua_bn_bwd_desc* d, int n, void* stream) {
  RUA_CHECK_ARG(d && n >= 1 && n <= RUA_MAX_BRANCH, "rua_bn_bwd_group: 1..%d members", RUA_MAX_BRANCH);
  const int vec = d[0].dtype == RUA_BF16 ? 8 : 4;
  bool one = n > 1 && g_tune.bn_bwd_group && d[0].C % vec == 0 && d[0].C / vec <= 256 && 256 % (d[0].C / vec) == 0 && g_tune.bn_regs;
  for (int i = 0; i < n && one; ++i) {
    const rua_bn_bwd_desc& m = d[i];
    one = m.x && m.dx && m.nb == 1 && m.M > 0 && m.C == d[0].C && m.dtype == d[0].dtype && m.masked == d[0].masked && !m.skip_stats && !m.dx_stats && m.count > 0 &&
          m.br[0].g && m.br[0].stats2 && m.br[0].replicas >= 1 && m.br[0].gamma && m.br[0].mean && m.br[0].rstd &&
          (d[0].dtype == RUA_F32 || d[0].dtype == RUA_BF16);
  }
  g_bn_bwd_group_last = n;
  if (!one) {
    for (int i = 0; i < n; ++i) { const int rc = rua_bn_bwd(d + i, stream); if (rc != RUA_OK) return rc; }
    return RUA_OK;
  }
  const int CG = d[0].C / vec;
  const size_t smem = (size_t)(1 * 5 + 2) * d[0].C * 4;
  BnBwdG a;
  long long pieces = 0;
  for (int i = 0; i < n; ++i) { a.k[i] = d[i]; a.pieces[i] = d[i].M * CG; if (a.pieces[i] > pieces) pieces = a.pieces[i]; }
  int g = grid_for(pieces);
  const int cap = (pieces >= (1ll << 20) ? 4 : 2) * rua_cu_count() / (n > 2 ? 2 : 1);
  if (g > cap) g = cap;
  hipStream_t st = (hipStream_t)stream;
  const bool mk = d[0].masked != 0;
  if (d[0].dtype == RUA_BF16) {
    if (mk) hipLaunchKernelGGL((bn_bwd_kernel_g<bf16_t, true>), dim3(g, n), dim3(256), smem, st, a, CG);
    else hipLaunchKernelGGL((bn_bwd_kernel_g<bf16_t, false>), dim3(g, n), dim3(256), smem, st, a, CG);
  } else {
    if (mk) hipLaunchKernelGGL((bn_bwd_kernel_g<float, true>), dim3(g, n), dim3(256), smem, st, a, CG);
    else hipLaunchKernelGGL((bn_bwd_kernel_g<float, false>), dim3(g, n), dim3(256), smem, st, a, CG);
  }
  RUA_LAUNCH_CHECK("rua_bn_bwd_group");
  g_bn_bwd_group_last = 1;
  return RUA_OK;
}

extern "C" int rua_bn_bwd(const rua_bn_bwd_desc* d, void* stream) {
  RUA_CHECK_ARG(d && d->x && d->dx && d->nb >= 1 && d->nb <= RUA_MAX_BRANCH && d->M > 0 && d->C > 0 && d->count > 0, "rua_bn_bwd: bad arguments");
  RUA_CHECK_ARG(d->dtype == RUA_F32 || d->dtype == RUA_BF16, "rua_bn_bwd: bad dtype");
  const int vec = d->dtype == RUA_BF16 ? 8 : 4;
  RUA_CHECK_ARG(d->C % vec == 0, "rua_bn_bwd: C=%d not a multiple of %d", d->C, vec);
  int rmax = 1;
  for (int b = 0; b < d->nb; ++b) {
    const rua_bn_bwd_branch& br = d->br[b];
    RUA_CHECK_ARG(br.g && br.stats2 && br.replicas >= 1 && br.gamma && br.mean && br.rstd, "rua_bn_bwd: null branch pointer");
    if (br.replicas > rmax) rmax = br.replicas;
  }
  size_t smem = (size_t)(d->nb * 5 + 2) * d->C * 4;
  RUA_CHECK_ARG(smem <= 160 * 1024, "rua_bn_bwd: coefficient table too large");
  const int CG = d->C / vec;
  if (d->skip_stats) {
    RUA_CHECK_ARG(d->dskip && d->skip_replicas >= 1 && (d->skip_replicas & (d->skip_replicas - 1)) == 0 && CG <= 256 && 256 % CG == 0,
                  "rua_bn_bwd: skip_stats needs dskip, a power-of-two replica count and C / %d dividing 256", vec);
    if (smem < (size_t)256 * vec * 4) smem = (size_t)256 * vec * 4;
  }
  if (d->dx_stats) {
    RUA_CHECK_ARG(d->dx_replicas >= 1 && (d->dx_replicas & (d->dx_replicas - 1)) == 0 && CG <= 256 && 256 % CG == 0,
                  "rua_bn_bwd: dx_stats needs a power-of-two replica count and C / %d dividing 256", vec);
    if (smem < (size_t)256 * vec * 4) smem = (size_t)256 * vec * 4;
  }
  const long long pieces = d->M * CG;
  int g = grid_for(pieces);
  const int cap_env = g_tune.bn_grid;
  const int cap = cap_env > 0 ? cap_env : (pieces >= (1ll << 20) ? 4 : 2) * rua_cu_count();
  if ((long long)rmax * d->C * d->nb >= 512 && g > cap) g = cap;
  hipStream_t st = (hipStream_t)stream;
  const int nbk = (CG <= 256 && 256 % CG == 0 && g_tune.bn_regs) ? d->nb : 0;
  const bool mk = d->masked != 0;
#define RUA_BN_BWD_GO1(T_, NB_, MK_, DX_) do { if (smem > 64 * 1024) (void)hipFuncSetAttribute((const void*)bn_bwd_kernel<T_, NB_, MK_, DX_>, hipFuncAttributeMaxDynamicSharedMemorySize, (int)smem); \
                                               hipLaunchKernelGGL((bn_bwd_kernel<T_, NB_, MK_, DX_>), dim3(g), dim3(256), smem, st, *d, pieces, CG); } while (0)
#define RUA_BN_BWD_GO(T_, NB_, MK_) do { if (d->dx_stats) RUA_BN_BWD_GO1(T_, NB_, MK_, true); else RUA_BN_BWD_GO1(T_, NB_, MK_, false); } while (0)
#define RUA_BN_BWD_SW(T_) switch (nbk * 2 + (mk ? 1 : 0)) { \
    case 2: RUA_BN_BWD_GO(T_, 1, false); break; case 3: RUA_BN_BWD_GO(T_, 1, true); break; \
    case 4: RUA_BN_BWD_GO(T_, 2, false); break; case 5: RUA_BN_BWD_GO(T_, 2, true); break; \
    case 6: RUA_BN_BWD_GO(T_, 3, false); break; case 7: RUA_BN_BWD_GO(T_, 3, true); break; \
    case 8: RUA_BN_BWD_GO(T_, 4, false); break; case 9: RUA_BN_BWD_GO(T_, 4, true); break; \
    default: RUA_BN_BWD_GO(T_, 0, false); }
  if (d->dtype == RUA_BF16) { RUA_BN_BWD_SW(bf16_t) } else { RUA_BN_BWD_SW(float) }
#undef RUA_BN_BWD_SW
#undef RUA_BN_BWD_GO
#undef RUA_BN_BWD_GO1
  RUA_LAUNCH_CHECK("rua_bn_bwd");
  return RUA_OK;
}

template <int VEC> __device__ __forceinline__ void idx_load(const uint8_t* p, int* out) {
  if constexpr (VEC == 8) { const uint2 q = *reinterpret_cast<const uint2*>(p);
#pragma unroll
    for (int j = 0; j < 4; ++j) { out[j] = (q.x >> (8 * j)) & 255; out[4 + j] = (q.y >> (8 * j)) & 255; } }
  else { const unsigned q = *reinterpret_cast<const unsigned*>(p);
#pragma unroll
    for (int j = 0; j < 4; ++j) out[j] = (q >> (8 * j)) & 255; }
}
template <int VEC> __device__ __forceinline__ void idx_store(uint8_t* p, const int* v) {
  if constexpr (VEC == 8) { uint2 q; q.x = (unsigned)v[0] | ((unsigned)v[1] << 8) | ((unsigned)v[2] << 16) | ((unsigned)v[3] << 24);
    q.y = (unsigned)v[4] | ((unsigned)v[5] << 8) | ((unsigned)v[6] << 16) | ((unsigned)v[7] << 24);
    *reinterpret_cast<uint2*>(p) = q; }
  else *reinterpret_cast<unsigned*>(p) = (unsigned)v[0] | ((unsigned)v[1] << 8) | ((unsigned)v[2] << 16) | ((unsigned)v[3] << 24);
}

template <typename T, int K>
__global__ void maxpool_fwd_kernel(const unsigned char* x, unsigned char* y, uint8_t* idx, int N, int H, int W, int CG, int k_rt) {
  constexpr int VEC = ET<T>::VEC;
  const int k = K > 0 ? K : k_rt;
  const int Ho = H / k, Wo = W / k;
  const long long total = (long long)N * Ho * Wo * CG;
  for (long long i = (long long)blockIdx.x * blockDim.x + threadIdx.x; i < total; i += (long long)gridDim.x * blockDim.x) {
    const int cp = (int)(i % CG); long long r = i / CG;
    const int wo = (int)(r % Wo); r /= Wo;
    const int ho = (int)(r % Ho); const int n = (int)(r / Ho);
    float best[VEC]; int bi[VEC];
#pragma unroll
    for (int j = 0; j < VEC; ++j) { best[j] = -INFINITY; bi[j] = 0; }
    if constexpr (K > 0) {
      for (int a = 0; a < K; ++a) {
        uint4 q[K];
#pragma unroll
        for (int b = 0; b < K; ++b) q[b] = ldg16(x + ((((size_t)n * H + ho * K + a) * W + wo * K + b) * CG + cp) * 16);
#pragma unroll
        for (int b = 0; b < K; ++b) {
          float v[VEC];
          ET<T>::unpack(q[b], v);
#pragma unroll
          for (int j = 0; j < VEC; ++j) if (v[j] > best[j]) { best[j] = v[j]; bi[j] = a * K + b; }
        }
      }
    } else {
      for (int a = 0; a < k; ++a)
        for (int b = 0; b < k; ++b) {
          float v[VEC];
          ET<T>::unpack(ldg16(x + ((((size_t)n * H + ho * k + a) * W + wo * k + b) * CG + cp) * 16), v);
#pragma unroll
          for (int j = 0; j < VEC; ++j) if (v[j] > best[j]) { best[j] = v[j]; bi[j] = a * k + b; }
        }
    }
    stg16(y + i * 16, ET<T>::pack(best));
    idx_store<VEC>(idx + i * VEC, bi);
  }
}

template <typename T>
__global__ void maxpool_bwd_kernel(const unsigned char* dy, const uint8_t* idx, unsigned char* dx, int accumulate,
                                   int N, int H, int W, int CG, int k) {
  constexpr int VEC = ET<T>::VEC;
  const int Ho = H / k, Wo = W / k;
  const long long total = (long long)N * H * W * CG;
  for (long long i = (long long)blockIdx.x * blockDim.x + threadIdx.x; i < total; i += (long long)gridDim.x * blockDim.x) {
    const int cp = (int)(i % CG); long long r = i / CG;
    const int w = (int)(r % W); r /= W;
    const int h = (int)(r % H); const int n = (int)(r / H);
    float o[VEC];
#pragma unroll
    for (int j = 0; j < VEC; ++j) o[j] = 0.f;
    if (accumulate) ET<T>::unpack(ldg16(dx + i * 16), o);
    if (h / k < Ho && w / k < Wo) {
      const size_t pi = (((size_t)n * Ho + h / k) * Wo + w / k) * CG + cp;
      float g[VEC];
      ET<T>::unpack(ldg16(dy + pi * 16), g);
      const int pos = (h % k) * k + (w % k);
      int ib[VEC];
      idx_load<VEC>(idx + pi * VEC, ib);
#pragma unroll
      for (int j = 0; j < VEC; ++j) if (ib[j] == pos) o[j] += g[j];
    }
    stg16(dx + i * 16, ET<T>::pack(o));
  }
}

template <typename T, int K>
__global__ void sumpool_kernel(const unsigned char* x, unsigned char* y, int N, int H, int W, int CG, int k_rt) {
  constexpr int VEC = ET<T>::VEC;
  const int k = K > 0 ? K : k_rt;
  const int Ho = H / k, Wo = W / k;
  const long long total = (long long)N * Ho * Wo * CG;
  for (long long i = (long long)blockIdx.x * blockDim.x + threadIdx.x; i < total; i += (long long)gridDim.x * blockDim.x) {
    const int cp = (int)(i % CG); long long r = i / CG;
    const int wo = (int)(r % Wo); r /= Wo;
    const int ho = (int)(r % Ho); const int n = (int)(r / Ho);
    float s[VEC];
#pragma unroll
    for (int j = 0; j < VEC; ++j) s[j] = 0.f;
    if constexpr (K > 0) {
      for (int a = 0; a < K; ++a) {
        uint4 q[K];
#pragma unroll
        for (int b = 0; b < K; ++b) q[b] = ldg16(x + ((((size_t)n * H + ho * K + a) * W + wo * K + b) * CG + cp) * 16);
#pragma unroll
        for (int b = 0; b < K; ++b) {
          float v[VEC];
          ET<T>::unpack(q[b], v);
#pragma unroll
          for (int j = 0; j < VEC; ++j) s[j] += v[j];
        }
      }
    } else {
      for (int a = 0; a < k; ++a)
        for (int b = 0; b < k; ++b) {
          float v[VEC];
          ET<T>::unpack(ldg16(x + ((((size_t)n * H + ho * k + a) * W + wo * k + b) * CG + cp) * 16), v);
#pragma unroll
          for (int j = 0; j < VEC; ++j) s[j] += v[j];
        }
    }
    stg16(y + i * 16, ET<T>::pack(s));
  }
}

template <typename T>
__global__ void upsample_kernel(const unsigned char* x, unsigned char* y, int N, int H, int W, int CG, int k) {
  const int Ho = H * k, Wo = W * k;
  const long long total = (long long)N * Ho * Wo * CG;
  for (long long i = (long long)blockIdx.x * blockDim.x + threadIdx.x; i < total; i += (long long)gridDim.x * blockDim.x) {
    const int cp = (int)(i % CG); long long r = i / CG;
    const int wo = (int)(r % Wo); r /= Wo;
    const int ho = (int)(r % Ho); const int n = (int)(r / Ho);
    stg16(y + i * 16, ldg16(x + ((((size_t)n * H + ho / k) * W + wo / k) * CG + cp) * 16));
  }
}

template <typename T>
__global__ __launch_bounds__(256) void maxpool_derive_kernel(const unsigned char* yp, const uint8_t* ip, unsigned char* y, uint8_t* idx,
                                                             int N, int Hp, int Wp, int CG, int kp) {
  constexpr int VEC = ET<T>::VEC;
  const int Ho = Hp / 2, Wo = Wp / 2, k = 2 * kp;
  const long long total = (long long)N * Ho * Wo * CG;
  for (long long i = (long long)blockIdx.x * blockDim.x + threadIdx.x; i < total; i += (long long)gridDim.x * blockDim.x) {
    const int cp = (int)(i % CG); long long r = i / CG;
    const int wo = (int)(r % Wo); r /= Wo;
    const int ho = (int)(r % Ho); const int n = (int)(r / Ho);
    uint4 q[4]; size_t o[4];
#pragma unroll
    for (int u = 0; u < 4; ++u) {
      o[u] = (((size_t)n * Hp + ho * 2 + (u >> 1)) * Wp + wo * 2 + (u & 1)) * CG + cp;
      q[u] = ldg16(yp + o[u] * 16);
    }
    float best[VEC]; int bi[VEC];
#pragma unroll
    for (int j = 0; j < VEC; ++j) { best[j] = -INFINITY; bi[j] = k * k; }
#pragma unroll
    for (int u = 0; u < 4; ++u) {
      float v[VEC];
      ET<T>::unpack(q[u], v);
      int ib[VEC];
      idx_load<VEC>(ip + o[u] * VEC, ib);
#pragma unroll
      for (int j = 0; j < VEC; ++j) {
        const int pp = ib[j];
        const int pos = ((u >> 1) * kp + pp / kp) * k + (u & 1) * kp + pp % kp;
        if (v[j] > best[j] || (v[j] == best[j] && pos < bi[j])) { best[j] = v[j]; bi[j] = pos; }
      }
    }
    stg16(y + i * 16, ET<T>::pack(best));
    idx_store<VEC>(idx + i * VEC, bi);
  }
}

struct PoolPyr { const unsigned char* dy[3]; const uint8_t* idx[3]; int k[3]; int n; };
template <typename T, bool POW2>
__global__ __launch_bounds__(256) void maxpool_bwd_multi_kernel(const PoolPyr q, unsigned char* dx, int accumulate, int N, int H, int W, int CG, int cgs, int ws, int hs) {
  constexpr int VEC = ET<T>::VEC;
  const long long total = (long long)N * H * W * CG;
  for (long long i = (long long)blockIdx.x * blockDim.x + threadIdx.x; i < total; i += (long long)gridDim.x * blockDim.x) {
    int cp, w, h, n;
    if constexpr (POW2) {
      const unsigned ii = (unsigned)i;
      cp = (int)(ii & (unsigned)(CG - 1)); const unsigned r = ii >> cgs;
      w = (int)(r & (unsigned)(W - 1)); h = (int)((r >> ws) & (unsigned)(H - 1)); n = (int)(r >> (ws + hs));
    } else {
      cp = (int)(i % CG); long long r = i / CG;
      w = (int)(r % W); r /= W;
      h = (int)(r % H); n = (int)(r / H);
    }
    float o[VEC];
#pragma unroll
    for (int j = 0; j < VEC; ++j) o[j] = 0.f;
    if (accumulate) ET<T>::unpack(ldg16(dx + i * 16), o);
#pragma unroll
    for (int u = 0; u < 3; ++u) {
      if (u >= q.n) break;
      const int k = q.k[u];
      size_t pi; int pos;
      if constexpr (POW2) {
        const int ks = 31 - __clz(k);
        pi = ((((size_t)n << (hs - ks)) + (h >> ks)) << (ws - ks)) + (w >> ks); pi = (pi << cgs) + cp;
        pos = ((h & (k - 1)) << ks) + (w & (k - 1));
      } else {
        const int Ho = H / k, Wo = W / k;
        pi = (((size_t)n * Ho + h / k) * Wo + w / k) * CG + cp;
        pos = (h % k) * k + (w % k);
      }
      float g[VEC];
      ET<T>::unpack(ldg16(q.dy[u] + pi * 16), g);
      int ib[VEC];
      idx_load<VEC>(q.idx[u] + pi * VEC, ib);
#pragma unroll
      for (int j = 0; j < VEC; ++j) if (ib[j] == pos) o[j] += g[j];
    }
    stg16(dx + i * 16, ET<T>::pack(o));
  }
}

template <typename T>
__global__ __launch_bounds__(256) void sumpool_pyramid_kernel(const unsigned char* x, unsigned char* y2, unsigned char* y4, unsigned char* y8,
                                                              int N, int H, int W, int CG) {
  constexpr int VEC = ET<T>::VEC;
  const int H8 = H / 8, W8 = W / 8;
  const long long total = (long long)N * H8 * W8 * CG;
  for (long long i = (long long)blockIdx.x * blockDim.x + threadIdx.x; i < total; i += (long long)gridDim.x * blockDim.x) {
    const int cp = (int)(i % CG); long long r = i / CG;
    const int w8 = (int)(r % W8); r /= W8;
    const int h8 = (int)(r % H8); const int n = (int)(r / H8);
    float s8[VEC], s4[2][VEC], s2[4][VEC];
#pragma unroll
    for (int j = 0; j < VEC; ++j) s8[j] = 0.f;
#pragma unroll
    for (int a = 0; a < 8; ++a) {
      uint4 q[8];
#pragma unroll
      for (int b = 0; b < 8; ++b) q[b] = ldg16(x + ((((size_t)n * H + h8 * 8 + a) * W + w8 * 8 + b) * CG + cp) * 16);
      if ((a & 1) == 0) {
#pragma unroll
        for (int u = 0; u < 4; ++u)
#pragma unroll
          for (int j = 0; j < VEC; ++j) s2[u][j] = 0.f;
      }
      if ((a & 3) == 0) {
#pragma unroll
        for (int u = 0; u < 2; ++u)
#pragma unroll
          for (int j = 0; j < VEC; ++j) s4[u][j] = 0.f;
      }
#pragma unroll
      for (int b = 0; b < 8; ++b) {
        float v[VEC];
        ET<T>::unpack(q[b], v);
#pragma unroll
        for (int j = 0; j < VEC; ++j) s2[b >> 1][j] += v[j];
      }
      if (a & 1) {
#pragma unroll
        for (int u = 0; u < 4; ++u) {
          const size_t o = (((size_t)n * (H / 2) + h8 * 4 + (a >> 1)) * (W / 2) + w8 * 4 + u) * CG + cp;
          stg16(y2 + o * 16, ET<T>::pack(s2[u]));
#pragma unroll
          for (int j = 0; j < VEC; ++j) s4[u >> 1][j] += s2[u][j];
        }
      }
      if ((a & 3) == 3) {
#pragma unroll
        for (int u = 0; u < 2; ++u) {
          const size_t o = (((size_t)n * (H / 4) + h8 * 2 + (a >> 2)) * (W / 4) + w8 * 2 + u) * CG + cp;
          stg16(y4 + o * 16, ET<T>::pack(s4[u]));
#pragma unroll
          for (int j = 0; j < VEC; ++j) s8[j] += s4[u][j];
        }
      }
    }
    stg16(y8 + i * 16, ET<T>::pack(s8));
  }
}

#define POOL_ARGS_CHECK(name) \
  RUA_CHECK_ARG(x && y && N > 0 && H > 0 && W > 0 && k >= 1, name ": bad arguments"); \
  RUA_CHECK_ARG(dtype == RUA_F32 || dtype == RUA_BF16, name ": bad dtype"); \
  const int vec = dtype == RUA_BF16 ? 8 : 4; \
  RUA_CHECK_ARG(C % vec == 0, name ": C=%d not a multiple of %d", C, vec); \
  const int CG = C / vec; hipStream_t st = (hipStream_t)stream;

extern "C" int rua_maxpool_fwd(const void* x, void* y, uint8_t* idx, int N, int H, int W, int C, int k, int dtype, void* stream) {
  POOL_ARGS_CHECK("rua_maxpool_fwd");
  RUA_CHECK_ARG(idx && H % k == 0 && W % k == 0 && k * k <= 256, "rua_maxpool_fwd: H,W must be divisible by k");
  RUA_CHECK_ARG(((size_t)idx & 7) == 0, "rua_maxpool_fwd: idx must be 8-byte aligned");
  const int g = grid_for((int64_t)N * (H / k) * (W / k) * CG);
#define RUA_MAXPOOL(TT, KK) hipLaunchKernelGGL((maxpool_fwd_kernel<TT, KK>), dim3(g), dim3(256), 0, st, (const unsigned char*)x, (unsigned char*)y, idx, N, H, W, CG, k)
  if (dtype == RUA_BF16) { if (k == 2) RUA_MAXPOOL(bf16_t, 2); else if (k == 4) RUA_MAXPOOL(bf16_t, 4); else if (k == 8) RUA_MAXPOOL(bf16_t, 8); else RUA_MAXPOOL(bf16_t, 0); }
  else { if (k == 2) RUA_MAXPOOL(float, 2); else if (k == 4) RUA_MAXPOOL(float, 4); else if (k == 8) RUA_MAXPOOL(float, 8); else RUA_MAXPOOL(float, 0); }
#undef RUA_MAXPOOL
  RUA_LAUNCH_CHECK("rua_maxpool_fwd");
  return RUA_OK;
}
extern "C" int rua_maxpool_bwd(const void* x, const uint8_t* idx, void* y, int accumulate, int N, int H, int W, int C, int k, int dtype, void* stream) {
  POOL_ARGS_CHECK("rua_maxpool_bwd");
  RUA_CHECK_ARG(idx && H % k == 0 && W % k == 0, "rua_maxpool_bwd: H,W must be divisible by k");
  RUA_CHECK_ARG(((size_t)idx & 7) == 0, "rua_maxpool_bwd: idx must be 8-byte aligned");
  const int g = grid_for((int64_t)N * H * W * CG);
  if (dtype == RUA_BF16) hipLaunchKernelGGL((maxpool_bwd_kernel<bf16_t>), dim3(g), dim3(256), 0, st, (const unsigned char*)x, idx, (unsigned char*)y, accumulate, N, H, W, CG, k);
  else hipLaunchKernelGGL((maxpool_bwd_kernel<float>), dim3(g), dim3(256), 0, st, (const unsigned char*)x, idx, (unsigned char*)y, accumulate, N, H, W, CG, k);
  RUA_LAUNCH_CHECK("rua_maxpool_bwd");
  return RUA_OK;
}
extern "C" int rua_sumpool(const void* x, void* y, int N, int H, int W, int C, int k, int dtype, void* stream) {
  POOL_ARGS_CHECK("rua_sumpool");
  RUA_CHECK_ARG(H % k == 0 && W % k == 0, "rua_sumpool: H,W must be divisible by k");
  const int g = grid_for((int64_t)N * (H / k) * (W / k) * CG);
#define RUA_SUMPOOL(TT, KK) hipLaunchKernelGGL((sumpool_kernel<TT, KK>), dim3(g), dim3(256), 0, st, (const unsigned char*)x, (unsigned char*)y, N, H, W, CG, k)
  if (dtype == RUA_BF16) { if (k == 2) RUA_SUMPOOL(bf16_t, 2); else if (k == 4) RUA_SUMPOOL(bf16_t, 4); else if (k == 8) RUA_SUMPOOL(bf16_t, 8); else RUA_SUMPOOL(bf16_t, 0); }
  else { if (k == 2) RUA_SUMPOOL(float, 2); else if (k == 4) RUA_SUMPOOL(float, 4); else if (k == 8) RUA_SUMPOOL(float, 8); else RUA_SUMPOOL(float, 0); }
#undef RUA_SUMPOOL
  RUA_LAUNCH_CHECK("rua_sumpool");
  return RUA_OK;
}

extern "C" int rua_maxpool_derive(const void* y_half, const uint8_t* idx_half, void* y, uint8_t* idx, int N, int H_half, int W_half, int C,
                                  int k_half, int dtype, void* stream) {
  const void* x = y_half; const int H = H_half, W = W_half, k = k_half;
  POOL_ARGS_CHECK("rua_maxpool_derive");
  RUA_CHECK_ARG(idx_half && idx && H % 2 == 0 && W % 2 == 0 && 4 * k * k <= 256, "rua_maxpool_derive: even input grid, window 2k with 4 k^2 <= 256");
  RUA_CHECK_ARG((((size_t)idx | (size_t)idx_half) & 7) == 0, "rua_maxpool_derive: idx buffers must be 8-byte aligned");
  const int g = grid_for((long long)N * (H / 2) * (W / 2) * CG);
  if (dtype == RUA_BF16) hipLaunchKernelGGL((maxpool_derive_kernel<bf16_t>), dim3(g), dim3(256), 0, st, (const unsigned char*)y_half, idx_half, (unsigned char*)y, idx, N, H, W, CG, k);
  else hipLaunchKernelGGL((maxpool_derive_kernel<float>), dim3(g), dim3(256), 0, st, (const unsigned char*)y_half, idx_half, (unsigned char*)y, idx, N, H, W, CG, k);
  RUA_LAUNCH_CHECK("rua_maxpool_derive");
  return RUA_OK;
}

extern "C" int rua_maxpool_bwd_multi(int n, const void* const* dy, const uint8_t* const* idx, const int* ks, void* dx, int accumulate,
                                     int N, int H, int W, int C, int dtype, void* stream) {
  const void* x = dx; const void* y = dx; const int k = 1;
  POOL_ARGS_CHECK("rua_maxpool_bwd_multi");
  RUA_CHECK_ARG(n >= 1 && n <= 3 && dy && idx && ks, "rua_maxpool_bwd_multi: 1..3 pooled gradients");
  PoolPyr q;
  q.n = n;
  for (int u = 0; u < 3; ++u) {
    q.dy[u] = u < n ? (const unsigned char*)dy[u] : nullptr; q.idx[u] = u < n ? idx[u] : nullptr; q.k[u] = u < n ? ks[u] : 1;
    if (u < n) RUA_CHECK_ARG(dy[u] && idx[u] && ((size_t)idx[u] & 7) == 0 && ks[u] >= 1 && H % ks[u] == 0 && W % ks[u] == 0, "rua_maxpool_bwd_multi: member %d: H, W must be divisible by k, idx 8-byte aligned", u);
  }
  const int g = grid_for((long long)N * H * W * CG);
  auto lg2 = [](int v) { int s_ = 0; while ((1 << s_) < v) ++s_; return (1 << s_) == v ? s_ : -1; };
  const int cgs = lg2(CG), ws = lg2(W), hs = lg2(H);
  bool p2 = cgs >= 0 && ws >= 0 && hs >= 0 && (long long)N * H * W * CG < (1ll << 31);
  for (int u = 0; u < n; ++u) p2 = p2 && lg2(ks[u]) >= 0;
  if (p2) {
    if (dtype == RUA_BF16) hipLaunchKernelGGL((maxpool_bwd_multi_kernel<bf16_t, true>), dim3(g), dim3(256), 0, st, q, (unsigned char*)dx, accumulate, N, H, W, CG, cgs, ws, hs);
    else hipLaunchKernelGGL((maxpool_bwd_multi_kernel<float, true>), dim3(g), dim3(256), 0, st, q, (unsigned char*)dx, accumulate, N, H, W, CG, cgs, ws, hs);
  } else {
    if (dtype == RUA_BF16) hipLaunchKernelGGL((maxpool_bwd_multi_kernel<bf16_t, false>), dim3(g), dim3(256), 0, st, q, (unsigned char*)dx, accumulate, N, H, W, CG, 0, 0, 0);
    else hipLaunchKernelGGL((maxpool_bwd_multi_kernel<float, false>), dim3(g), dim3(256), 0, st, q, (unsigned char*)dx, accumulate, N, H, W, CG, 0, 0, 0);
  }
  RUA_LAUNCH_CHECK("rua_maxpool_bwd_multi");
  return RUA_OK;
}

extern "C" int rua_sumpool_pyramid(const void* x, void* y2, void* y4, void* y8, int N, int H, int W, int C, int dtype, void* stream) {
  const void* y = y2; const int k = 8;
  POOL_ARGS_CHECK("rua_sumpool_pyramid");
  RUA_CHECK_ARG(y4 && y8 && H % 8 == 0 && W % 8 == 0, "rua_sumpool_pyramid: H, W must be multiples of 8, every output given");
  const int g = grid_for((long long)N * (H / 8) * (W / 8) * CG);
  if (dtype == RUA_BF16) hipLaunchKernelGGL((sumpool_pyramid_kernel<bf16_t>), dim3(g), dim3(256), 0, st, (const unsigned char*)x, (unsigned char*)y2, (unsigned char*)y4, (unsigned char*)y8, N, H, W, CG);
  else hipLaunchKernelGGL((sumpool_pyramid_kernel<float>), dim3(g), dim3(256), 0, st, (const unsigned char*)x, (unsigned char*)y2, (unsigned char*)y4, (unsigned char*)y8, N, H, W, CG);
  RUA_LAUNCH_CHECK("rua_sumpool_pyramid");
  return RUA_OK;
}
extern "C" int rua_upsample_nearest(const void* x, void* y, int N, int H, int W, int C, int k, int dtype, void* stream) {
  POOL_ARGS_CHECK("rua_upsample_nearest");
  const int g = grid_for((int64_t)N * H * k * W * k * CG);
  if (dtype == RUA_BF16) hipLaunchKernelGGL((upsample_kernel<bf16_t>), dim3(g), dim3(256), 0, st, (const unsigned char*)x, (unsigned char*)y, N, H, W, CG, k);
  else hipLaunchKernelGGL((upsample_kernel<float>), dim3(g), dim3(256), 0, st, (const unsigned char*)x, (unsigned char*)y, N, H, W, CG, k);
  RUA_LAUNCH_CHECK("rua_upsample_nearest");
  return RUA_OK;
}

struct AddK { int n; const unsigned char* in[8]; unsigned char* out; int accumulate; long long pieces; };
template <typename T>
__global__ void add_n_kernel(const AddK p) {
  constexpr int VEC = ET<T>::VEC;
  for (long long i = (long long)blockIdx.x * blockDim.x + threadIdx.x; i < p.pieces; i += (long long)gridDim.x * blockDim.x) {
    float s[VEC];
#pragma unroll
    for (int j = 0; j < VEC; ++j) s[j] = 0.f;
    if (p.accumulate) ET<T>::unpack(ldg16(p.out + i * 16), s);
    for (int b = 0; b < p.n; ++b) {
      float v[VEC];
      ET<T>::unpack(ldg16(p.in[b] + i * 16), v);
#pragma unroll
      for (int j = 0; j < VEC; ++j) s[j] += v[j];
    }
    stg16(p.out + i * 16, ET<T>::pack(s));
  }
}
extern "C" int rua_add_n(int n, const void* const* in, void* out, int accumulate, int64_t elems, int dtype, void* stream) {
  RUA_CHECK_ARG(n >= 1 && n <= 8 && in && out && elems > 0, "rua_add_n: bad arguments");
  const int vec = dtype == RUA_BF16 ? 8 : 4;
  RUA_CHECK_ARG(elems % vec == 0, "rua_add_n: element count must be a multiple of %d", vec);
  AddK k; k.n = n; k.out = (unsigned char*)out; k.accumulate = accumulate; k.pieces = elems / vec;
  for (int b = 0; b < n; ++b) { RUA_CHECK_ARG(in[b], "rua_add_n: null input"); k.in[b] = (const unsigned char*)in[b]; }
  hipStream_t st = (hipStream_t)stream;
  if (dtype == RUA_BF16) hipLaunchKernelGGL((add_n_kernel<bf16_t>), dim3(grid_for(k.pieces)), dim3(256), 0, st, k);
  else hipLaunchKernelGGL((add_n_kernel<float>), dim3(grid_for(k.pieces)), dim3(256), 0, st, k);
  RUA_LAUNCH_CHECK("rua_add_n");
  return RUA_OK;
}

template <typename T, int MODE>
__global__ void relu_kernel(unsigned char* a, const unsigned char* b, long long pieces) {
  constexpr int VEC = ET<T>::VEC;
  for (long long i = (long long)blockIdx.x * blockDim.x + threadIdx.x; i < pieces; i += (long long)gridDim.x * blockDim.x) {
    float u[VEC], v[VEC];
    ET<T>::unpack(ldg16(b + i * 16), v);
    if (MODE == 0) {
      ET<T>::unpack(ldg16(a + i * 16), u);
#pragma unroll
      for (int j = 0; j < VEC; ++j) u[j] = v[j] > 0.f ? u[j] : 0.f;
    } else {
#pragma unroll
      for (int j = 0; j < VEC; ++j) u[j] = fmaxf(v[j], 0.f);
    }
    stg16(a + i * 16, ET<T>::pack(u));
  }
}
extern "C" int rua_relu_mask(void* dy, const void* y, int64_t elems, int dtype, void* stream) {
  RUA_CHECK_ARG(dy && y && elems > 0, "rua_relu_mask: bad arguments");
  const int vec = dtype == RUA_BF16 ? 8 : 4;
  RUA_CHECK_ARG(elems % vec == 0, "rua_relu_mask: element count must be a multiple of %d", vec);
  hipStream_t st = (hipStream_t)stream;
  if (dtype == RUA_BF16) hipLaunchKernelGGL((relu_kernel<bf16_t, 0>), dim3(grid_for(elems / vec)), dim3(256), 0, st, (unsigned char*)dy, (const unsigned char*)y, (long long)(elems / vec));
  else hipLaunchKernelGGL((relu_kernel<float, 0>), dim3(grid_for(elems / vec)), dim3(256), 0, st, (unsigned char*)dy, (const unsigned char*)y, (long long)(elems / vec));
  RUA_LAUNCH_CHECK("rua_relu_mask");
  return RUA_OK;
}
extern "C" int rua_relu(const void* x, void* y, int64_t elems, int dtype, void* stream) {
  RUA_CHECK_ARG(x && y && elems > 0, "rua_relu: bad arguments");
  const int vec = dtype == RUA_BF16 ? 8 : 4;
  RUA_CHECK_ARG(elems % vec == 0, "rua_relu: element count must be a multiple of %d", vec);
  hipStream_t st = (hipStream_t)stream;
  if (dtype == RUA_BF16) hipLaunchKernelGGL((relu_kernel<bf16_t, 1>), dim3(grid_for(elems / vec)), dim3(256), 0, st, (unsigned char*)y, (const unsigned char*)x, (long long)(elems / vec));
  else hipLaunchKernelGGL((relu_kernel<float, 1>), dim3(grid_for(elems / vec)), dim3(256), 0, st, (unsigned char*)y, (const unsigned char*)x, (long long)(elems / vec));
  RUA_LAUNCH_CHECK("rua_relu");
  return RUA_OK;
}

__global__ void cast_to_bf16_kernel(const float* __restrict__ x, bf16_t* __restrict__ y, long long n) {
  for (long long i = (long long)blockIdx.x * blockDim.x + threadIdx.x; i < n; i += (long long)gridDim.x * blockDim.x) y[i] = (bf16_t)x[i];
}
__global__ void cast_from_bf16_kernel(const bf16_t* __restrict__ x, float* __restrict__ y, long long n) {
  for (long long i = (long long)blockIdx.x * blockDim.x + threadIdx.x; i < n; i += (long long)gridDim.x * blockDim.x) y[i] = (float)x[i];
}
extern "C" int rua_cast_f32_to(const float* x, void* y, int64_t elems, int dtype, void* stream) {
  RUA_CHECK_ARG(x && y && elems > 0, "rua_cast_f32_to: bad arguments");
  hipStream_t st = (hipStream_t)stream;
  if (dtype == RUA_BF16) {
    hipLaunchKernelGGL(cast_to_bf16_kernel, dim3(grid_for(elems)), dim3(256), 0, st, x, (bf16_t*)y, (long long)elems);
    RUA_LAUNCH_CHECK("rua_cast_f32_to");
    return RUA_OK;
  }
  hipError_t e = hipMemcpyAsync(y, x, elems * 4, hipMemcpyDeviceToDevice, st);
  if (e != hipSuccess) { rua_set_error("rua_cast_f32_to: %s", hipGetErrorString(e)); return RUA_ERR_LAUNCH; }
  return RUA_OK;
}
extern "C" int rua_cast_to_f32(const void* x, float* y, int64_t elems, int dtype, void* stream) {
  RUA_CHECK_ARG(x && y && elems > 0, "rua_cast_to_f32: bad arguments");
  hipStream_t st = (hipStream_t)stream;
  if (dtype == RUA_BF16) {
    hipLaunchKernelGGL(cast_from_bf16_kernel, dim3(grid_for(elems)), dim3(256), 0, st, (const bf16_t*)x, y, (long long)elems);
    RUA_LAUNCH_CHECK("rua_cast_to_f32");
    return RUA_OK;
  }
  hipError_t e = hipMemcpyAsync(y, x, elems * 4, hipMemcpyDeviceToDevice, st);
  if (e != hipSuccess) { rua_set_error("rua_cast_to_f32: %s", hipGetErrorString(e)); return RUA_ERR_LAUNCH; }
  return RUA_OK;
}
__global__ __launch_bounds__(256) void fill_zero_kernel(unsigned char* p, long long bytes) {
  const long long head = ((16 - ((size_t)p & 15)) & 15) < bytes ? ((16 - ((size_t)p & 15)) & 15) : bytes;
  const long long n16 = (bytes - head) / 16;
  uint4* q = reinterpret_cast<uint4*>(p + head);
  const uint4 z = make_uint4(0, 0, 0, 0);
  for (long long i = blockIdx.x * (long long)blockDim.x + threadIdx.x; i < n16; i += (long long)gridDim.x * blockDim.x) q[i] = z;
  if (blockIdx.x == 0) {
    for (long long i = threadIdx.x; i < head; i += blockDim.x) p[i] = 0;
    for (long long i = head + n16 * 16 + threadIdx.x; i < bytes; i += blockDim.x) p[i] = 0;
  }
}
extern "C" int rua_fill_zero(void* p, int64_t bytes, void* stream) {
  RUA_CHECK_ARG(p && bytes >= 0, "rua_fill_zero: bad arguments");
  if (bytes == 0) return RUA_OK;
  if (g_tune.fill_kernel) {
    long long blocks = (bytes / 16 + 255) / 256;
    if (blocks < 1) blocks = 1;
    if (blocks > 4 * rua_cu_count()) blocks = 4 * rua_cu_count();
    hipLaunchKernelGGL(fill_zero_kernel, dim3((unsigned)blocks), dim3(256), 0, (hipStream_t)stream, (unsigned char*)p, (long long)bytes);
    RUA_LAUNCH_CHECK("rua_fill_zero");
    return RUA_OK;
  }
  hipError_t e = hipMemsetAsync(p, 0, bytes, (hipStream_t)stream);
  if (e != hipSuccess) { rua_set_error("rua_fill_zero: %s", hipGetErrorString(e)); return RUA_ERR_LAUNCH; }
  return RUA_OK;
}
```

Measured before the change: 1382 patches/s.

## Add channel-sliced BatchNorm fwd/bwd kernels for small activations

Adds a sliced BatchNorm path where each block owns a slice of S channel groups and a contiguous range of rows. Per-block coefficients are computed only for that slice, which shrinks the shared coefficient table, and reductions are folded per slice with atomics into replicated stats. The path is used by default for small tensors (up to 262144 vector pieces) in both single and grouped launches. The aim is to cut per-block setup cost and raise parallelism on the many small low-resolution BN layers, at the cost of more kernel variants and atomic traffic.

```diff
diff --git a/include/rua_hip.h b/include/rua_hip.h
--- a/include/rua_hip.h
+++ b/include/rua_hip.h
@@ -209,6 +209,9 @@
 int rua_bn_bwd(const rua_bn_bwd_desc* d, void* stream);
 int rua_bn_bwd_group(const rua_bn_bwd_desc* d, int n, void* stream);
 int rua_bn_bwd_group_last_grids(void);
+int rua_bn_fwd_route(const rua_bn_fwd_desc* d);
+int rua_bn_bwd_route(const rua_bn_bwd_desc* d);
+int rua_bn_part_range(int64_t M, int P, int part, int64_t* begin, int64_t* end);
 
 int rua_maxpool_fwd(const void* x, void* y, uint8_t* idx, int N, int H, int W, int C, int k, int dtype, void* stream);
 int rua_maxpool_bwd(const void* dy, const uint8_t* idx, void* dx, int accumulate, int N, int H, int W, int C, int k, int dtype, void* stream);
diff --git a/resunet_a_mltsk_keras_amd/_lib.py b/resunet_a_mltsk_keras_amd/_lib.py
--- a/resunet_a_mltsk_keras_amd/_lib.py
+++ b/resunet_a_mltsk_keras_amd/_lib.py
@@ -168,6 +168,9 @@
     "rua_bn_bwd": ([C.POINTER(BnBwdDesc), vp], i32),
     "rua_bn_bwd_group": ([C.POINTER(BnBwdDesc), i32, vp], i32),
     "rua_bn_bwd_group_last_grids": ([], i32),
+    "rua_bn_fwd_route": ([C.POINTER(BnFwdDesc)], i32),
+    "rua_bn_bwd_route": ([C.POINTER(BnBwdDesc)], i32),
+    "rua_bn_part_range": ([i64, i32, i32, C.POINTER(i64), C.POINTER(i64)], i32),
     "rua_maxpool_fwd": ([vp, vp, vp, i32, i32, i32, i32, i32, i32, vp], i32),
     "rua_maxpool_bwd": ([vp, vp, vp, i32, i32, i32, i32, i32, i32, i32, vp], i32),
     "rua_sumpool": ([vp, vp, i32, i32, i32, i32, i32, i32, vp], i32),
diff --git a/resunet_a_mltsk_keras_amd/csrc/capi.cpp b/resunet_a_mltsk_keras_amd/csrc/capi.cpp
--- a/resunet_a_mltsk_keras_amd/csrc/capi.cpp
+++ b/resunet_a_mltsk_keras_amd/csrc/capi.cpp
@@ -117,6 +117,7 @@
     {"bn_bwd_group", &g_tune.bn_bwd_group, nullptr}, {"conv_small", &g_tune.conv_small, nullptr}, {"strip_stag", &g_tune.strip_stag, nullptr},
     {"cu_reserve", &g_tune.cu_reserve, nullptr}, {"wgrad_rows", &g_tune.wgrad_rows, nullptr}, {"strip_seglen", &g_tune.strip_seglen, nullptr},
     {"band_stag", &g_tune.band_stag, nullptr}, {"conv_band128m", &g_tune.conv_band128m, nullptr}, {"conv_img2", &g_tune.conv_img2, nullptr},
+    {"bn_sliced", &g_tune.bn_sliced, nullptr}, {"bn_sliced_parts", &g_tune.bn_sliced_parts, nullptr}, {"bn_sliced_s", &g_tune.bn_sliced_s, nullptr},
     {"dbg_ptr", nullptr, &g_tune.dbg_ptr},
   };
   *n = (int)(sizeof(t) / sizeof(t[0]));
diff --git a/resunet_a_mltsk_keras_amd/csrc/common.h b/resunet_a_mltsk_keras_amd/csrc/common.h
--- a/resunet_a_mltsk_keras_amd/csrc/common.h
+++ b/resunet_a_mltsk_keras_amd/csrc/common.h
@@ -84,6 +84,8 @@
   int epi_fast = 1;
   int dmap_chain = 0;
   int wgrad_taps_share = 1;
+  int bn_sliced = 1;
+  int bn_sliced_parts = 0, bn_sliced_s = 0;
   int bn_regs = 1;
   int fill_kernel = 1;
   int band_dbg = 0;
diff --git a/resunet_a_mltsk_keras_amd/csrc/elementwise.hip b/resunet_a_mltsk_keras_amd/csrc/elementwise.hip
--- a/resunet_a_mltsk_keras_amd/csrc/elementwise.hip
+++ b/resunet_a_mltsk_keras_amd/csrc/elementwise.hip
@@ -338,53 +338,76 @@
   return RUA_OK;
 }
 
+
+__device__ __forceinline__ void bn_fwd_moments(const rua_bn_fwd_desc& p, int c, double& mean, double& var) {
+  if (p.training && p.stats) {
+    double s1, s2;
+    replica_sum(p.stats, p.replicas, p.C, c, s1, s2);
+    mean = s1 / p.count;
+    var = s2 / p.count - mean * mean;
+    if (var < 0) var = 0;
+  } else { mean = 0; var = 1; }
+}
+__device__ __forceinline__ void bn_fwd_coef(const rua_bn_fwd_desc& p, const rua_bn_branch& br, int c, double mean, double var, bool publish,
+                                            float& scale, float& shift) {
+  const int C = p.C;
+  double m = mean, v = var;
+  if (p.training && br.stats) {
+    double s1, s2;
+    replica_sum(br.stats, br.replicas, C, c, s1, s2);
+    m = s1 / p.count;
+    v = s2 / p.count - m * m;
+    if (v < 0) v = 0;
+  }
+  if (!p.training) { m = br.moving_mean[c]; v = br.moving_var[c]; }
+  const double r = 1.0 / sqrt(v + (double)p.eps);
+  const double sc = (double)br.gamma[c] * r;
+  scale = (float)sc;
+  shift = (float)((double)br.beta[c] - m * sc);
+  if (publish) {
+    br.scale[c] = (float)sc; br.shift[c] = (float)((double)br.beta[c] - m * sc);
+    if (br.mean) br.mean[c] = (float)m;
+    if (br.rstd) br.rstd[c] = (float)r;
+    if (p.training && br.out_stats) {
+      const double be = (double)br.beta[c];
+      br.out_stats[c] = p.count * be;
+      br.out_stats[C + c] = p.count * (be * be + sc * sc * v);
+    }
+    if (p.training && br.moving_mean) {
+      const double unb = p.bessel_n > 1 ? v * (p.bessel_n / (p.bessel_n - 1)) : v;
+      br.moving_mean[c] = (float)((double)br.moving_mean[c] * p.momentum + m * (1.0 - p.momentum));
+      br.moving_var[c] = (float)((double)br.moving_var[c] * p.momentum + unb * (1.0 - p.momentum));
+    }
+  }
+}
+template <typename T, int NB>
+__device__ __forceinline__ void bn_fwd_piece(const unsigned char* x, unsigned char* const (&outs)[NB], long long i,
+                                             const float (&sc)[NB][ET<T>::VEC], const float (&sh)[NB][ET<T>::VEC], bool relu) {
+  constexpr int VEC = ET<T>::VEC;
+  float xv[VEC];
+  ET<T>::unpack(ldg16(x + i * 16), xv);
+#pragma unroll
+  for (int b = 0; b < NB; ++b) {
+    float o[VEC];
+#pragma unroll
+    for (int j = 0; j < VEC; ++j) {
+      o[j] = fmaf(sc[b][j], xv[j], sh[b][j]);
+      if (relu) o[j] = fmaxf(o[j], 0.f);
+    }
+    stg16(outs[b] + i * 16, ET<T>::pack(o));
+  }
+}
+
 template <typename T, int NB>
 __device__ __forceinline__ void bn_fwd_body(const rua_bn_fwd_desc& p, long long pieces, int CG) {
   constexpr int VEC = ET<T>::VEC;
   extern __shared__ float tab[];
   const int C = p.C;
-  float* mr = tab + p.nb * 2 * C;
   for (int c = threadIdx.x; c < C; c += 256) {
     double mean, var;
-    if (p.training && p.stats) {
-      double s1, s2;
-      replica_sum(p.stats, p.replicas, C, c, s1, s2);
-      mean = s1 / p.count;
-      var = s2 / p.count - mean * mean;
-      if (var < 0) var = 0;
-    } else { mean = 0; var = 1; }
-    for (int b = 0; b < p.nb; ++b) {
-      const rua_bn_branch& br = p.br[b];
-      double m = mean, v = var;
-      if (p.training && br.stats) {
-        double s1, s2;
-        replica_sum(br.stats, br.replicas, C, c, s1, s2);
-        m = s1 / p.count;
-        v = s2 / p.count - m * m;
-        if (v < 0) v = 0;
-      }
-      if (!p.training) { m = br.moving_mean[c]; v = br.moving_var[c]; }
-      const double r = 1.0 / sqrt(v + (double)p.eps);
-      const double sc = (double)br.gamma[c] * r;
-      tab[(b * 2) * C + c] = (float)sc;
-      tab[(b * 2 + 1) * C + c] = (float)((double)br.beta[c] - m * sc);
-      if (blockIdx.x == 0) {
-        br.scale[c] = (float)sc; br.shift[c] = (float)((double)br.beta[c] - m * sc);
-        if (br.mean) br.mean[c] = (float)m;
-        if (br.rstd) br.rstd[c] = (float)r;
-        if (p.training && br.out_stats) {
-          const double be = (double)br.beta[c];
-          br.out_stats[c] = p.count * be;
-          br.out_stats[C + c] = p.count * (be * be + sc * sc * v);
-        }
-        if (p.training && br.moving_mean) {
-          const double unb = p.bessel_n > 1 ? v * (p.bessel_n / (p.bessel_n - 1)) : v;
-          br.moving_mean[c] = (float)((double)br.moving_mean[c] * p.momentum + m * (1.0 - p.momentum));
-          br.moving_var[c] = (float)((double)br.moving_var[c] * p.momentum + unb * (1.0 - p.momentum));
-        }
-      }
-    }
-    (void)mr;
+    bn_fwd_moments(p, c, mean, var);
+    for (int b = 0; b < p.nb; ++b)
+      bn_fwd_coef(p, p.br[b], c, mean, var, blockIdx.x == 0, tab[(b * 2) * C + c], tab[(b * 2 + 1) * C + c]);
   }
   __syncthreads();
   if (p.br[0].out == nullptr) return;
@@ -401,20 +424,7 @@
 #pragma unroll
     for (int b = 0; b < NB; ++b) outs[b] = (unsigned char*)p.br[b].out;
     const bool relu = p.relu != 0;
-    for (long long i = (long long)blockIdx.x * 256 + threadIdx.x; i < pieces; i += stride) {
-      float xv[VEC];
-      ET<T>::unpack(ldg16(x + i * 16), xv);
-#pragma unroll
-      for (int b = 0; b < NB; ++b) {
-        float o[VEC];
-#pragma unroll
-        for (int j = 0; j < VEC; ++j) {
-          o[j] = fmaf(sc[b][j], xv[j], sh[b][j]);
-          if (relu) o[j] = fmaxf(o[j], 0.f);
-        }
-        stg16(outs[b] + i * 16, ET<T>::pack(o));
-      }
-    }
+    for (long long i = (long long)blockIdx.x * 256 + threadIdx.x; i < pieces; i += stride) bn_fwd_piece<T, NB>(x, outs, i, sc, sh, relu);
   } else {
     for (long long i = (long long)blockIdx.x * 256 + threadIdx.x; i < pieces; i += stride) {
       const int c = (int)(i % CG) * VEC;
@@ -440,20 +450,132 @@
 template <typename T>
 __global__ __launch_bounds__(256) void bn_fwd_kernel_g(const BnFwdG g, int CG) { bn_fwd_body<T, 1>(g.k[blockIdx.y], g.pieces[blockIdx.y], CG); }
 
+__host__ __device__ __forceinline__ long long bn_part_begin(long long M, int P, int part) { return M * part / P; }
+extern "C" int rua_bn_part_range(int64_t M, int P, int part, int64_t* begin, int64_t* end) {
+  RUA_CHECK_ARG(M > 0 && P >= 1 && P <= M && part >= 0 && part < P && begin && end, "rua_bn_part_range: bad arguments");
+  *begin = bn_part_begin(M, P, part); *end = bn_part_begin(M, P, part + 1);
+  return RUA_OK;
+}
+
+template <typename T, int NB, int S>
+__device__ __forceinline__ void bn_fwd_sliced_body(const rua_bn_fwd_desc& p, int P, int bx) {
+  constexpr int VEC = ET<T>::VEC, SV = S * VEC;
+  __shared__ float tab[NB * 2 * SV];
+  const int CG = p.C / VEC, slices = CG / S;
+  const int slice = bx % slices, part = bx / slices;
+  if (part >= P) return;
+  for (int it = threadIdx.x; it < NB * SV; it += 256) {
+    const int b = it / SV, cl = it - b * SV, c = slice * SV + cl;
+    double mean, var;
+    bn_fwd_moments(p, c, mean, var);
+    bn_fwd_coef(p, p.br[b], c, mean, var, part == 0, tab[(b * 2) * SV + cl], tab[(b * 2 + 1) * SV + cl]);
+  }
+  __syncthreads();
+  const int q = (int)(threadIdx.x % S);
+  float sc[NB][VEC], sh[NB][VEC];
+#pragma unroll
+  for (int b = 0; b < NB; ++b)
+#pragma unroll
+    for (int j = 0; j < VEC; ++j) { sc[b][j] = tab[(b * 2) * SV + q * VEC + j]; sh[b][j] = tab[(b * 2 + 1) * SV + q * VEC + j]; }
+  unsigned char* outs[NB];
+#pragma unroll
+  for (int b = 0; b < NB; ++b) outs[b] = (unsigned char*)p.br[b].out;
+  const unsigned char* x = (const unsigned char*)p.x;
+  const bool relu = p.relu != 0;
+  const long long m1 = bn_part_begin(p.M, P, part + 1);
+  for (long long m = bn_part_begin(p.M, P, part) + threadIdx.x / S; m < m1; m += 256 / S)
+    bn_fwd_piece<T, NB>(x, outs, m * CG + slice * S + q, sc, sh, relu);
+}
+template <typename T, int NB, int S>
+__global__ __launch_bounds__(256) void bn_fwd_sliced_kernel(const rua_bn_fwd_desc p, int P) { bn_fwd_sliced_body<T, NB, S>(p, P, blockIdx.x); }
+struct BnFwdGS { rua_bn_fwd_desc k[RUA_MAX_BRANCH]; int P[RUA_MAX_BRANCH]; };
+static_assert(sizeof(BnFwdGS) <= 4096, "grouped launch: kernel arguments are limited to 4 KiB");
+template <typename T, int S>
+__global__ __launch_bounds__(256) void bn_fwd_sliced_kernel_g(const BnFwdGS g) { bn_fwd_sliced_body<T, 1, S>(g.k[blockIdx.y], g.P[blockIdx.y], blockIdx.x); }
+
+struct BnRoute { int S, P; };
+constexpr long long RUA_BN_SLICED_BLOCKS = 512;
+constexpr long long RUA_BN_SLICED_MAX_PIECES = 262144;
+constexpr long long RUA_BN_SLICED_MAX_STEPS = 8;
+static BnRoute bn_route(long long M, int C, int dtype, int nb, int r_in, int r_out) {
+  BnRoute none = {0, 0};
+  if (g_tune.bn_sliced == 0 || M <= 0 || C <= 0 || nb < 1 || nb > RUA_MAX_BRANCH) return none;
+  const int vec = dtype == RUA_BF16 ? 8 : 4;
+  int S = C % (8 * vec) == 0 ? 8 : C % (4 * vec) == 0 ? 4 : 0;
+  if (g_tune.bn_sliced_s == 4 && C % (4 * vec) == 0) S = 4;
+  if (S == 0) return none;
+  const long long slices = C / (S * vec), steps = (M + 256 / S - 1) / (256 / S);
+  long long P = (RUA_BN_SLICED_BLOCKS + slices - 1) / slices;
+  if (P > steps) P = steps;
+  if (r_out > 0 && P > r_out) P = r_out;
+  if (g_tune.bn_sliced_parts > 0) P = g_tune.bn_sliced_parts < M ? g_tune.bn_sliced_parts : M;
+  if (P > 65535) P = 65535;
+  (void)r_in;
+  if (g_tune.bn_sliced != 2 && (M * (C / vec) > RUA_BN_SLICED_MAX_PIECES || steps > RUA_BN_SLICED_MAX_STEPS * P)) return none;
+  BnRoute r = {S, (int)P};
+  return r;
+}
+static BnRoute bn_fwd_route_of(const rua_bn_fwd_desc& d) {
+  BnRoute none = {0, 0};
+  if (d.nb < 1 || d.nb > RUA_MAX_BRANCH || d.br[0].out == nullptr || (d.dtype != RUA_F32 && d.dtype != RUA_BF16)) return none;
+  int r_in = 0;
+  if (d.training) {
+    if (d.stats) r_in = d.replicas;
+    for (int b = 0; b < d.nb; ++b) if (d.br[b].stats && d.br[b].replicas > r_in) r_in = d.br[b].replicas;
+  }
+  return bn_route(d.M, d.C, d.dtype, d.nb, r_in, 0);
+}
+extern "C" int rua_bn_fwd_route(const rua_bn_fwd_desc* d) {
+  if (!d) return 0;
+  const BnRoute r = bn_fwd_route_of(*d);
+  return r.S ? (r.S | r.P << 8) : 0;
+}
+template <typename T, int S>
+static void bn_fwd_sliced_launch(const rua_bn_fwd_desc& d, int P, hipStream_t st) {
+  const dim3 g((unsigned)(d.C / (S * ET<T>::VEC) * P));
+  switch (d.nb) {
+    case 1: hipLaunchKernelGGL((bn_fwd_sliced_kernel<T, 1, S>), g, dim3(256), 0, st, d, P); break;
+    case 2: hipLaunchKernelGGL((bn_fwd_sliced_kernel<T, 2, S>), g, dim3(256), 0, st, d, P); break;
+    case 3: hipLaunchKernelGGL((bn_fwd_sliced_kernel<T, 3, S>), g, dim3(256), 0, st, d, P); break;
+    default: hipLaunchKernelGGL((bn_fwd_sliced_kernel<T, 4, S>), g, dim3(256), 0, st, d, P); break;
+  }
+}
+
 extern "C" int rua_bn_fwd(const rua_bn_fwd_desc* d, void* stream);
 static thread_local int g_bn_fwd_group_last = 0;
 extern "C" int rua_bn_fwd_group_last_grids(void) { return g_bn_fwd_group_last; }
 extern "C" int rua_bn_fwd_group(const rua_bn_fwd_desc* d, int n, void* stream) {
   RUA_CHECK_ARG(d && n >= 1 && n <= RUA_MAX_BRANCH, "rua_bn_fwd_group: 1..%d members", RUA_MAX_BRANCH);
   const int vec = d[0].dtype == RUA_BF16 ? 8 : 4;
-  bool one = n > 1 && g_tune.bn_bwd_group && d[0].C % vec == 0 && d[0].C / vec <= 256 && 256 % (d[0].C / vec) == 0 && g_tune.bn_regs &&
-             (d[0].dtype == RUA_F32 || d[0].dtype == RUA_BF16) && (size_t)4 * d[0].C * 4 <= 64 * 1024;
-  for (int i = 0; i < n && one; ++i) {
+  bool same = n > 1 && g_tune.bn_bwd_group && d[0].C > 0 && d[0].C % vec == 0 && (d[0].dtype == RUA_F32 || d[0].dtype == RUA_BF16);
+  for (int i = 0; i < n && same; ++i) {
     const rua_bn_fwd_desc& m = d[i];
     const rua_bn_branch& br = m.br[0];
-    one = m.x && m.nb == 1 && m.M > 0 && m.C == d[0].C && m.dtype == d[0].dtype && m.training == d[0].training && m.relu == d[0].relu && br.out &&
-          br.gamma && br.beta && br.scale && br.shift && (!m.training || (m.count > 0 && (br.stats ? br.replicas >= 1 : (m.stats && m.replicas >= 1)))) &&
-          (m.training || (br.moving_mean && br.moving_var)) && (br.out_stats == nullptr || (m.relu == 0 && m.training));
+    same = m.x && m.nb == 1 && m.M > 0 && m.C == d[0].C && m.dtype == d[0].dtype && m.training == d[0].training && m.relu == d[0].relu && br.out &&
+           br.gamma && br.beta && br.scale && br.shift && (!m.training || (m.count > 0 && (br.stats ? br.replicas >= 1 : (m.stats && m.replicas >= 1)))) &&
+           (m.training || (br.moving_mean && br.moving_var)) && (br.out_stats == nullptr || (m.relu == 0 && m.training));
+  }
+  const bool one = same && d[0].C / vec <= 256 && 256 % (d[0].C / vec) == 0 && g_tune.bn_regs && (size_t)4 * d[0].C * 4 <= 64 * 1024;
+  if (same) {
+    BnFwdGS a;
+    int S = 0, pmax = 0;
+    bool sliced = true;
+    for (int i = 0; i < n && sliced; ++i) {
+      const BnRoute r = bn_fwd_route_of(d[i]);
+      sliced = r.S != 0 && (i == 0 || r.S == S);
+      S = r.S; a.k[i] = d[i]; a.P[i] = r.P; if (r.P > pmax) pmax = r.P;
+    }
+    if (sliced) {
+      const dim3 g((unsigned)(d[0].C / (S * vec) * pmax), n);
+      hipStream_t st = (hipStream_t)stream;
+      if (d[0].dtype == RUA_BF16) { if (S == 8) hipLaunchKernelGGL((bn_fwd_sliced_kernel_g<bf16_t, 8>), g, dim3(256), 0, st, a);
+                                    else hipLaunchKernelGGL((bn_fwd_sliced_kernel_g<bf16_t, 4>), g, dim3(256), 0, st, a); }
+      else { if (S == 8) hipLaunchKernelGGL((bn_fwd_sliced_kernel_g<float, 8>), g, dim3(256), 0, st, a);
+             else hipLaunchKernelGGL((bn_fwd_sliced_kernel_g<float, 4>), g, dim3(256), 0, st, a); }
+      RUA_LAUNCH_CHECK("rua_bn_fwd_group");
+      g_bn_fwd_group_last = 1;
+      return RUA_OK;
+    }
   }
   g_bn_fwd_group_last = n;
   if (!one) {
@@ -492,6 +614,13 @@
     RUA_CHECK_ARG(d->training || (br.moving_mean && br.moving_var), "rua_bn_fwd: inference needs moving statistics");
     RUA_CHECK_ARG(br.out_stats == nullptr || (d->relu == 0 && d->training), "rua_bn_fwd: out_stats is the statistics of a training-mode BatchNorm WITHOUT ReLU");
   }
+  hipStream_t st = (hipStream_t)stream;
+  if (const BnRoute rt = bn_fwd_route_of(*d); rt.S) {
+    if (d->dtype == RUA_BF16) { if (rt.S == 8) bn_fwd_sliced_launch<bf16_t, 8>(*d, rt.P, st); else bn_fwd_sliced_launch<bf16_t, 4>(*d, rt.P, st); }
+    else { if (rt.S == 8) bn_fwd_sliced_launch<float, 8>(*d, rt.P, st); else bn_fwd_sliced_launch<float, 4>(*d, rt.P, st); }
+    RUA_LAUNCH_CHECK("rua_bn_fwd");
+    return RUA_OK;
+  }
   const size_t smem = (size_t)(d->nb * 2 + 2) * d->C * 4;
   RUA_CHECK_ARG(smem <= 64 * 1024, "rua_bn_fwd: coefficient table too large");
   const int CG = d->C / vec;
@@ -500,7 +629,6 @@
   const int cap = g_tune.bn_grid > 0 ? g_tune.bn_grid : 2 * rua_cu_count();
   if ((long long)d->replicas * d->C >= 512 && g > cap) g = cap;
   if (coef_only) g = 1;
-  hipStream_t st = (hipStream_t)stream;
   const int nbk = (!coef_only && CG <= 256 && 256 % CG == 0 && g_tune.bn_regs) ? d->nb : 0;
 #define RUA_BN_FWD_GO(T_, NB_) hipLaunchKernelGGL((bn_fwd_kernel<T_, NB_>), dim3(g), dim3(256), smem, st, *d, pieces, CG)
   if (d->dtype == RUA_BF16) {
@@ -514,6 +642,61 @@
   RUA_LAUNCH_CHECK("rua_bn_fwd");
   return RUA_OK;
 }
+
+__device__ __forceinline__ void bn_bwd_coef(const rua_bn_bwd_desc& p, const rua_bn_bwd_branch& br, int c, bool publish,
+                                            float& A, float& ms, float& mt, float& tb, float& tc) {
+  double sg, sgx;
+  replica_sum(br.stats2, br.replicas, p.C, c, sg, sgx);
+  const double mu = br.mean[c], r = br.rstd[c], gm = br.gamma[c];
+  if (br.stats2_out) {
+    const double sc = br.scale[c], sh = br.shift[c];
+    sgx = sc != 0.0 ? (sgx - sh * sg) / sc : mu * sg;
+  }
+  const double dga = r * (sgx - mu * sg);
+  const double s = gm * r;
+  A = (float)s;
+  ms = (p.masked && br.scale) ? br.scale[c] : 1.f;
+  mt = (p.masked && br.shift) ? br.shift[c] : 0.f;
+  tb = (float)(-s * r * dga / p.count);
+  tc = (float)(-s * sg / p.count + s * r * mu * dga / p.count);
+  if (publish) {
+    if (br.dgamma) br.dgamma[c] += (float)dga;
+    if (br.dbeta) br.dbeta[c] += (float)sg;
+  }
+}
+#define RUA_BN_BWD_PIECE(i_) do { \
+  const long long pi_ = (i_); \
+  const uint4 xr = ldg16(x + pi_ * 16); \
+  uint4 gr[NB]; \
+  _Pragma("unroll") for (int b = 0; b < NB; ++b) gr[b] = ldg16(gp[b] + pi_ * 16); \
+  uint4 dr = make_uint4(0, 0, 0, 0), ar = make_uint4(0, 0, 0, 0); \
+  if (dskip) dr = ldg16(dskip + pi_ * 16); \
+  if (accum) ar = ldg16(dx + pi_ * 16); \
+  float xv[VEC], acc[VEC]; \
+  ET<T>::unpack(xr, xv); \
+  _Pragma("unroll") for (int j = 0; j < VEC; ++j) acc[j] = fmaf(cB[j], xv[j], cC[j]); \
+  if (dskip) { \
+    float dd[VEC]; \
+    ET<T>::unpack(dr, dd); \
+    _Pragma("unroll") for (int j = 0; j < VEC; ++j) { acc[j] += dd[j]; sk[j] += dd[j]; } \
+  } \
+  if (accum) { \
+    float dd[VEC]; \
+    ET<T>::unpack(ar, dd); \
+    _Pragma("unroll") for (int j = 0; j < VEC; ++j) acc[j] += dd[j]; \
+  } \
+  _Pragma("unroll") for (int b = 0; b < NB; ++b) { \
+    float gv[VEC]; \
+    ET<T>::unpack(gr[b], gv); \
+    _Pragma("unroll") for (int j = 0; j < VEC; ++j) { \
+      bool on = true; \
+      if constexpr (MASKED) on = fmaf(cS[b][j], xv[j], cT[b][j]) > 0.f; \
+      acc[j] = fmaf(cA[b][j], on ? gv[j] : 0.f, acc[j]); \
+    } \
+  } \
+  _Pragma("unroll") for (int j = 0; j < VEC; ++j) if constexpr (DXS) { so[j] += acc[j]; so2[j] = fmaf(acc[j], xv[j], so2[j]); } \
+  stg16(dx + pi_ * 16, ET<T>::pack(acc)); \
+} while (0)
 
 template <typename T, int NB, bool MASKED, bool DXS = false>
 __device__ __forceinline__ void bn_bwd_body(const rua_bn_bwd_desc& p, long long pieces, int CG) {
@@ -524,25 +707,8 @@
   float* tT = tB + 2 * C;
   for (int it = threadIdx.x; it < p.nb * C; it += 256) {
     const int b = it / C, c = it - b * C;
-    const rua_bn_bwd_branch& br = p.br[b];
-    double sg, sgx;
-    replica_sum(br.stats2, br.replicas, C, c, sg, sgx);
-    const double mu = br.mean[c], r = br.rstd[c], gm = br.gamma[c];
-    if (br.stats2_out) {
-      const double sc = br.scale[c], sh = br.shift[c];
-      sgx = sc != 0.0 ? (sgx - sh * sg) / sc : mu * sg;
-    }
-    const double dga = r * (sgx - mu * sg);
-    const double s = gm * r;
-    tab[(b * 3) * C + c] = (float)s;
-    tab[(b * 3 + 1) * C + c] = (p.masked && br.scale) ? br.scale[c] : 1.f;
-    tab[(b * 3 + 2) * C + c] = (p.masked && br.shift) ? br.shift[c] : 0.f;
-    tT[(b * 2) * C + c] = (float)(-s * r * dga / p.count);
-    tT[(b * 2 + 1) * C + c] = (float)(-s * sg / p.count + s * r * mu * dga / p.count);
-    if (blockIdx.x == 0) {
-      if (br.dgamma) br.dgamma[c] += (float)dga;
-      if (br.dbeta) br.dbeta[c] += (float)sg;
-    }
+    bn_bwd_coef(p, p.br[b], c, blockIdx.x == 0, tab[(b * 3) * C + c], tab[(b * 3 + 1) * C + c], tab[(b * 3 + 2) * C + c],
+                tT[(b * 2) * C + c], tT[(b * 2 + 1) * C + c]);
   }
   __syncthreads();
   for (int c = threadIdx.x; c < C; c += 256) {
@@ -574,45 +740,7 @@
 #pragma unroll
     for (int b = 0; b < NB; ++b) gp[b] = (const unsigned char*)p.br[b].g;
     const bool accum = p.accumulate != 0;
-    for (long long i = (long long)blockIdx.x * 256 + threadIdx.x; i < pieces; i += stride) {
-      const uint4 xr = ldg16(x + i * 16);
-      uint4 gr[NB];
-#pragma unroll
-      for (int b = 0; b < NB; ++b) gr[b] = ldg16(gp[b] + i * 16);
-      uint4 dr = make_uint4(0, 0, 0, 0), ar = make_uint4(0, 0, 0, 0);
-      if (dskip) dr = ldg16(dskip + i * 16);
-      if (accum) ar = ldg16(dx + i * 16);
-      float xv[VEC], acc[VEC];
-      ET<T>::unpack(xr, xv);
-#pragma unroll
-      for (int j = 0; j < VEC; ++j) acc[j] = fmaf(cB[j], xv[j], cC[j]);
-      if (dskip) {
-        float dd[VEC];
-        ET<T>::unpack(dr, dd);
-#pragma unroll
-        for (int j = 0; j < VEC; ++j) { acc[j] += dd[j]; sk[j] += dd[j]; }
-      }
-      if (accum) {
-        float dd[VEC];
-        ET<T>::unpack(ar, dd);
-#pragma unroll
-        for (int j = 0; j < VEC; ++j) acc[j] += dd[j];
-      }
-#pragma unroll
-      for (int b = 0; b < NB; ++b) {
-        float gv[VEC];
-        ET<T>::unpack(gr[b], gv);
-#pragma unroll
-        for (int j = 0; j < VEC; ++j) {
-          bool on = true;
-          if constexpr (MASKED) on = fmaf(cS[b][j], xv[j], cT[b][j]) > 0.f;
-          acc[j] = fmaf(cA[b][j], on ? gv[j] : 0.f, acc[j]);
-        }
-      }
-#pragma unroll
-      for (int j = 0; j < VEC; ++j) if constexpr (DXS) { so[j] += acc[j]; so2[j] = fmaf(acc[j], xv[j], so2[j]); }
-      stg16(dx + i * 16, ET<T>::pack(acc));
-    }
+    for (long long i = (long long)blockIdx.x * 256 + threadIdx.x; i < pieces; i += stride) RUA_BN_BWD_PIECE(i);
   } else {
   for (long long i = (long long)blockIdx.x * 256 + threadIdx.x; i < pieces; i += stride) {
     const int c = (int)(i % CG) * VEC;
@@ -687,18 +815,153 @@
 template <typename T, bool MASKED>
 __global__ __launch_bounds__(256) void bn_bwd_kernel_g(const BnBwdG g, int CG) { bn_bwd_body<T, 1, MASKED>(g.k[blockIdx.y], g.pieces[blockIdx.y], CG); }
 
+template <typename T, int NB, bool MASKED, bool DXS, int S>
+__device__ __forceinline__ void bn_bwd_sliced_body(const rua_bn_bwd_desc& p, int P, int bx) {
+  constexpr int VEC = ET<T>::VEC, SV = S * VEC;
+  __shared__ float tab[(NB * 5 + 2) * SV];
+  static_assert((NB * 5 + 2) >= 4, "the folds reuse the table as [4][SV]");
+  float* tB = tab + NB * 3 * SV;
+  float* tT = tB + 2 * SV;
+  const int C = p.C, CG = C / VEC, slices = CG / S;
+  const int slice = bx % slices, part = bx / slices;
+  if (part >= P) return;
+  for (int it = threadIdx.x; it < NB * SV; it += 256) {
+    const int b = it / SV, cl = it - b * SV;
+    bn_bwd_coef(p, p.br[b], slice * SV + cl, part == 0, tab[(b * 3) * SV + cl], tab[(b * 3 + 1) * SV + cl], tab[(b * 3 + 2) * SV + cl],
+                tT[(b * 2) * SV + cl], tT[(b * 2 + 1) * SV + cl]);
+  }
+  __syncthreads();
+  if (threadIdx.x < SV) {
+    const int cl = threadIdx.x;
+    float sb = 0.f, sc_ = 0.f;
+    for (int b = 0; b < NB; ++b) { sb += tT[(b * 2) * SV + cl]; sc_ += tT[(b * 2 + 1) * SV + cl]; }
+    tB[cl] = sb; tB[SV + cl] = sc_;
+  }
+  __syncthreads();
+  const int q = (int)(threadIdx.x % S);
+  float sk[VEC], so[VEC], so2[VEC];
+#pragma unroll
+  for (int j = 0; j < VEC; ++j) { sk[j] = 0.f; so[j] = 0.f; so2[j] = 0.f; }
+  float cA[NB][VEC], cS[MASKED ? NB : 1][VEC], cT[MASKED ? NB : 1][VEC], cB[VEC], cC[VEC];
+#pragma unroll
+  for (int j = 0; j < VEC; ++j) { cB[j] = tB[q * VEC + j]; cC[j] = tB[SV + q * VEC + j]; }
+#pragma unroll
+  for (int b = 0; b < NB; ++b)
+#pragma unroll
+    for (int j = 0; j < VEC; ++j) {
+      cA[b][j] = tab[(b * 3) * SV + q * VEC + j];
+      if constexpr (MASKED) { cS[b][j] = tab[(b * 3 + 1) * SV + q * VEC + j]; cT[b][j] = tab[(b * 3 + 2) * SV + q * VEC + j]; }
+    }
+  const unsigned char* gp[NB];
+#pragma unroll
+  for (int b = 0; b < NB; ++b) gp[b] = (const unsigned char*)p.br[b].g;
+  const unsigned char* x = (const unsigned char*)p.x;
+  const unsigned char* dskip = (const unsigned char*)p.dskip;
+  unsigned char* dx = (unsigned char*)p.dx;
+  const bool accum = p.accumulate != 0;
+  const long long m1 = bn_part_begin(p.M, P, part + 1);
+  for (long long m = bn_part_begin(p.M, P, part) + threadIdx.x / S; m < m1; m += 256 / S)
+    RUA_BN_BWD_PIECE(m * CG + slice * S + q);
+  auto fold = [&](float* v, double* dst, int replicas, int slot) {
+    float* red = tab;
+    __syncthreads();
+#pragma unroll
+    for (int j = 0; j < VEC; ++j)
+#pragma unroll
+      for (int o = S; o < 64; o <<= 1) v[j] += __shfl_xor(v[j], o, 64);
+    const int lane = threadIdx.x & 63, wv = threadIdx.x >> 6;
+    if (lane < S) {
+#pragma unroll
+      for (int j = 0; j < VEC; ++j) red[wv * SV + lane * VEC + j] = v[j];
+    }
+    __syncthreads();
+    if (threadIdx.x < SV) {
+      const int cl = threadIdx.x;
+      const float t = (red[cl] + red[SV + cl]) + (red[2 * SV + cl] + red[3 * SV + cl]);
+      unsafeAtomicAdd(&dst[(size_t)(part & (replicas - 1)) * 2 * C + slot * C + slice * SV + cl], (double)t);
+    }
+  };
+  if (p.skip_stats && dskip) fold(sk, p.skip_stats, p.skip_replicas, 0);
+  if constexpr (DXS) { fold(so, p.dx_stats, p.dx_replicas, 0); fold(so2, p.dx_stats, p.dx_replicas, 1); }
+}
+#undef RUA_BN_BWD_PIECE
+template <typename T, int NB, bool MASKED, bool DXS, int S>
+__global__ __launch_bounds__(256) void bn_bwd_sliced_kernel(const rua_bn_bwd_desc p, int P) { bn_bwd_sliced_body<T, NB, MASKED, DXS, S>(p, P, blockIdx.x); }
+struct BnBwdGS { rua_bn_bwd_desc k[RUA_MAX_BRANCH]; int P[RUA_MAX_BRANCH]; };
+static_assert(sizeof(BnBwdGS) <= 4096, "grouped launch: kernel arguments are limited to 4 KiB");
+template <typename T, bool MASKED, int S>
+__global__ __launch_bounds__(256) void bn_bwd_sliced_kernel_g(const BnBwdGS g) { bn_bwd_sliced_body<T, 1, MASKED, false, S>(g.k[blockIdx.y], g.P[blockIdx.y], blockIdx.x); }
+
+static BnRoute bn_bwd_route_of(const rua_bn_bwd_desc& d) {
+  BnRoute none = {0, 0};
+  if (d.nb < 1 || d.nb > RUA_MAX_BRANCH || (d.dtype != RUA_F32 && d.dtype != RUA_BF16)) return none;
+  int r_in = 1, r_out = 0;
+  for (int b = 0; b < d.nb; ++b) if (d.br[b].replicas > r_in) r_in = d.br[b].replicas;
+  if (d.skip_stats) r_out = d.skip_replicas;
+  if (d.dx_stats && (r_out == 0 || d.dx_replicas < r_out)) r_out = d.dx_replicas;
+  return bn_route(d.M, d.C, d.dtype, d.nb, r_in, r_out);
+}
+extern "C" int rua_bn_bwd_route(const rua_bn_bwd_desc* d) {
+  if (!d) return 0;
+  const BnRoute r = bn_bwd_route_of(*d);
+  return r.S ? (r.S | r.P << 8) : 0;
+}
+template <typename T, int NB, int S>
+static void bn_bwd_sliced_launch_nb(const rua_bn_bwd_desc& d, int P, hipStream_t st) {
+  const dim3 g((unsigned)(d.C / (S * ET<T>::VEC) * P));
+  switch ((d.masked ? 2 : 0) + (d.dx_stats ? 1 : 0)) {
+    case 0: hipLaunchKernelGGL((bn_bwd_sliced_kernel<T, NB, false, false, S>), g, dim3(256), 0, st, d, P); break;
+    case 1: hipLaunchKernelGGL((bn_bwd_sliced_kernel<T, NB, false, true, S>), g, dim3(256), 0, st, d, P); break;
+    case 2: hipLaunchKernelGGL((bn_bwd_sliced_kernel<T, NB, true, false, S>), g, dim3(256), 0, st, d, P); break;
+    default: hipLaunchKernelGGL((bn_bwd_sliced_kernel<T, NB, true, true, S>), g, dim3(256), 0, st, d, P); break;
+  }
+}
+template <typename T, int S>
+static void bn_bwd_sliced_launch(const rua_bn_bwd_desc& d, int P, hipStream_t st) {
+  switch (d.nb) {
+    case 1: bn_bwd_sliced_launch_nb<T, 1, S>(d, P, st); break;
+    case 2: bn_bwd_sliced_launch_nb<T, 2, S>(d, P, st); break;
+    case 3: bn_bwd_sliced_launch_nb<T, 3, S>(d, P, st); break;
+    default: bn_bwd_sliced_launch_nb<T, 4, S>(d, P, st); break;
+  }
+}
+
 extern "C" int rua_bn_bwd(const rua_bn_bwd_desc* d, void* stream);
 static thread_local int g_bn_bwd_group_last = 0;
 extern "C" int rua_bn_bwd_group_last_grids(void) { return g_bn_bwd_group_last; }
 extern "C" int rua_bn_bwd_group(const rua_bn_bwd_desc* d, int n, void* stream) {
   RUA_CHECK_ARG(d && n >= 1 && n <= RUA_MAX_BRANCH, "rua_bn_bwd_group: 1..%d members", RUA_MAX_BRANCH);
   const int vec = d[0].dtype == RUA_BF16 ? 8 : 4;
-  bool one = n > 1 && g_tune.bn_bwd_group && d[0].C % vec == 0 && d[0].C / vec <= 256 && 256 % (d[0].C / vec) == 0 && g_tune.bn_regs;
-  for (int i = 0; i < n && one; ++i) {
+  bool same = n > 1 && g_tune.bn_bwd_group && d[0].C > 0 && d[0].C % vec == 0;
+  for (int i = 0; i < n && same; ++i) {
     const rua_bn_bwd_desc& m = d[i];
-    one = m.x && m.dx && m.nb == 1 && m.M > 0 && m.C == d[0].C && m.dtype == d[0].dtype && m.masked == d[0].masked && !m.skip_stats && !m.dx_stats && m.count > 0 &&
-          m.br[0].g && m.br[0].stats2 && m.br[0].replicas >= 1 && m.br[0].gamma && m.br[0].mean && m.br[0].rstd &&
-          (d[0].dtype == RUA_F32 || d[0].dtype == RUA_BF16);
+    same = m.x && m.dx && m.nb == 1 && m.M > 0 && m.C == d[0].C && m.dtype == d[0].dtype && m.masked == d[0].masked && !m.skip_stats && !m.dx_stats && m.count > 0 &&
+           m.br[0].g && m.br[0].stats2 && m.br[0].replicas >= 1 && m.br[0].gamma && m.br[0].mean && m.br[0].rstd &&
+           (d[0].dtype == RUA_F32 || d[0].dtype == RUA_BF16);
+  }
+  const bool one = same && d[0].C / vec <= 256 && 256 % (d[0].C / vec) == 0 && g_tune.bn_regs;
+  if (same) {
+    BnBwdGS a;
+    int S = 0, pmax = 0;
+    bool sliced = true;
+    for (int i = 0; i < n && sliced; ++i) {
+      const BnRoute r = bn_bwd_route_of(d[i]);
+      sliced = r.S != 0 && (i == 0 || r.S == S);
+      S = r.S; a.k[i] = d[i]; a.P[i] = r.P; if (r.P > pmax) pmax = r.P;
+    }
+    if (sliced) {
+      const dim3 g((unsigned)(d[0].C / (S * vec) * pmax), n);
+      hipStream_t st = (hipStream_t)stream;
+      const bool mk = d[0].masked != 0;
+#define RUA_BN_BWD_GS(T_, MK_) do { if (S == 8) hipLaunchKernelGGL((bn_bwd_sliced_kernel_g<T_, MK_, 8>), g, dim3(256), 0, st, a); \
+                                    else hipLaunchKernelGGL((bn_bwd_sliced_kernel_g<T_, MK_, 4>), g, dim3(256), 0, st, a); } while (0)
+      if (d[0].dtype == RUA_BF16) { if (mk) RUA_BN_BWD_GS(bf16_t, true); else RUA_BN_BWD_GS(bf16_t, false); }
+      else { if (mk) RUA_BN_BWD_GS(float, true); else RUA_BN_BWD_GS(float, false); }
+#undef RUA_BN_BWD_GS
+      RUA_LAUNCH_CHECK("rua_bn_bwd_group");
+      g_bn_bwd_group_last = 1;
+      return RUA_OK;
+    }
   }
   g_bn_bwd_group_last = n;
   if (!one) {
@@ -739,7 +1002,6 @@
     if (br.replicas > rmax) rmax = br.replicas;
   }
   size_t smem = (size_t)(d->nb * 5 + 2) * d->C * 4;
-  RUA_CHECK_ARG(smem <= 160 * 1024, "rua_bn_bwd: coefficient table too large");
   const int CG = d->C / vec;
   if (d->skip_stats) {
     RUA_CHECK_ARG(d->dskip && d->skip_replicas >= 1 && (d->skip_replicas & (d->skip_replicas - 1)) == 0 && CG <= 256 && 256 % CG == 0,
@@ -751,12 +1013,19 @@
                   "rua_bn_bwd: dx_stats needs a power-of-two replica count and C / %d dividing 256", vec);
     if (smem < (size_t)256 * vec * 4) smem = (size_t)256 * vec * 4;
   }
+  hipStream_t st = (hipStream_t)stream;
+  if (const BnRoute rt = bn_bwd_route_of(*d); rt.S) {
+    if (d->dtype == RUA_BF16) { if (rt.S == 8) bn_bwd_sliced_launch<bf16_t, 8>(*d, rt.P, st); else bn_bwd_sliced_launch<bf16_t, 4>(*d, rt.P, st); }
+    else { if (rt.S == 8) bn_bwd_sliced_launch<float, 8>(*d, rt.P, st); else bn_bwd_sliced_launch<float, 4>(*d, rt.P, st); }
+    RUA_LAUNCH_CHECK("rua_bn_bwd");
+    return RUA_OK;
+  }
+  RUA_CHECK_ARG(smem <= 160 * 1024, "rua_bn_bwd: coefficient table too large");
   const long long pieces = d->M * CG;
   int g = grid_for(pieces);
   const int cap_env = g_tune.bn_grid;
   const int cap = cap_env > 0 ? cap_env : (pieces >= (1ll << 20) ? 4 : 2) * rua_cu_count();
   if ((long long)rmax * d->C * d->nb >= 512 && g > cap) g = cap;
-  hipStream_t st = (hipStream_t)stream;
   const int nbk = (CG <= 256 && 256 % CG == 0 && g_tune.bn_regs) ? d->nb : 0;
   const bool mk = d->masked != 0;
 #define RUA_BN_BWD_GO1(T_, NB_, MK_, DX_) do { if (smem > 64 * 1024) (void)hipFuncSetAttribute((const void*)bn_bwd_kernel<T_, NB_, MK_, DX_>, hipFuncAttributeMaxDynamicSharedMemorySize, (int)smem); \
```

New measurement: 1407 patches/s (median of 6 runs). 1.02x the previous value.
